# AIDynamicAction/rcognita

Measured on AMD Instinct MI355X. Metric: env-control-steps/sec (whole node), 3wrobot Nactor=10, higher is better.
Workload: dtype f64

## Files before the change

### include/rcg.h

```cpp
#ifndef RCG_H
#define RCG_H

#include <stdint.h>

#ifdef __cplusplus
extern "C" {
#endif

#define RCG_VERSION 122

#define RCG_MAX_DS 5
#define RCG_MAX_DU 2
#define RCG_MAX_CHI 7
#define RCG_MAX_PARS 5
#define RCG_MAX_DC 35
#define RCG_MAX_ROW 64
#define RCG_MAX_NACTOR 4096

typedef enum rcg_status {
  RCG_OK = 0,
  RCG_ERR_BAD_ARG = -1,
  RCG_ERR_HIP = -2,
  RCG_ERR_NO_DEVICE = -3,
  RCG_ERR_UNSUPPORTED = -4,
  RCG_ERR_NONFINITE = -5
} rcg_status;

typedef enum rcg_system { RCG_SYS_3WROBOT = 0, RCG_SYS_3WROBOT_NI = 1, RCG_SYS_2TANK = 2 } rcg_system;
#define RCG_SYS_USER_BASE 16
typedef enum rcg_mode { RCG_MODE_MPC = 0, RCG_MODE_RQL = 1, RCG_MODE_SQL = 2 } rcg_mode;
typedef enum rcg_stage { RCG_STAGE_QUADRATIC = 0, RCG_STAGE_BIQUADRATIC = 1 } rcg_stage;
typedef enum rcg_critic_struct {
  RCG_CRITIC_QUAD_LIN = 0,
  RCG_CRITIC_QUADRATIC = 1,
  RCG_CRITIC_QUAD_NOMIX = 2,
  RCG_CRITIC_QUAD_MIX = 3
} rcg_critic_struct;
typedef enum rcg_dtype { RCG_F32 = 0, RCG_F64 = 1 } rcg_dtype;
typedef enum rcg_where { RCG_HOST = 0, RCG_DEVICE = 1 } rcg_where;

#define RCG_FLAG_HAS_TARGET 0x1
#define RCG_FLAG_PER_ENV_PARS 0x2
#define RCG_FLAG_REF_LAG 0x4
#define RCG_FLAG_ACCUM_EVERY_SUBSTEP 0x8
#define RCG_FLAG_NO_CLIP 0x10
#define RCG_FLAG_DISTURB 0x20

typedef enum rcg_field {
  RCG_FIELD_STATE = 0,
  RCG_FIELD_ACTION = 1,
  RCG_FIELD_ACCUM = 2,
  RCG_FIELD_STEP_IDX = 3,
  RCG_FIELD_EPISODE_IDX = 4,
  RCG_FIELD_STATUS = 5,
  RCG_FIELD_PARS = 6,
  RCG_FIELD_STATE_INIT = 7,
  RCG_FIELD_STATE_PREV = 8,
  RCG_FIELD_BEST_J = 9,
  RCG_FIELD_BEST_IDX = 10,
  RCG_FIELD_W_CRITIC = 11,
  RCG_FIELD_W_PREV = 12,
  RCG_FIELD_OBS_BUF = 13,
  RCG_FIELD_ACT_BUF = 14,
  RCG_FIELD_RETURNS = 15,
  RCG_FIELD_ACTION_SQN = 16,
  RCG_FIELD_DISTURB = 17,
  RCG_FIELD_SUBSTEP_IDX = 18,
  RCG_FIELD_COUNT_ = 19
} rcg_field;

typedef struct rcg_cfg {
  int32_t struct_size;
  int32_t sys_id;
  int32_t batch;
  int32_t dtype;
  int32_t device;
  int32_t n_actor;
  int32_t mode;
  int32_t stage_obj_struct;
  int32_t critic_struct;
  int32_t n_critic;
  int32_t buffer_size;
  int32_t substeps_per_tick;
  int32_t flags;
  int32_t critic_every_ticks;
  double dt_sim;
  double sampling_time;
  double pred_step_size;
  double gamma;
  double pars[8];
  double ctrl_bnds[4];
  double R1[49];
  double R2[49];
  double target[8];
  double action_init[4];
  double w_init[40];
  double w_min[40];
  double w_max[40];
  double pars_disturb[6];
  double disturb_init[2];
  uint64_t seed;
  int64_t env_id_base;
} rcg_cfg;

typedef struct rcg_summary {
  double count;
  double sum;
  double sumsq;
  double min;
  double max;
  double n_failed;
} rcg_summary;

typedef struct rcg_handle rcg_handle;

int rcg_version(void);
const char* rcg_last_error(const rcg_handle* h);
int rcg_device_count(void);

int rcg_register_system(const char* name, const char* policy_src, int32_t ds, int32_t du, int32_t np, int32_t* sys_id);
int rcg_rtc_version(int32_t* major, int32_t* minor);
int rcg_system_info(int32_t sys_id, int32_t* ds, int32_t* du, int32_t* np, int32_t* has_jac);
int rcg_system_output_info(int32_t sys_id, int32_t* dy, int32_t* has_out, int32_t* has_out_jac);
int rcg_system_has_critic(int32_t sys_id, int32_t* has_critic);
int rcg_system_programs(int32_t sys_id, char* buf, int64_t cap, int64_t* need);

int rcg_create(const rcg_cfg* cfg, rcg_handle** out);
int rcg_destroy(rcg_handle* h);
int rcg_set_stream(rcg_handle* h, void* hip_stream);
int rcg_use_own_stream(rcg_handle* h);
int rcg_wait_stream(rcg_handle* h, void* producer_stream);
int rcg_release_stream(rcg_handle* h, void* consumer_stream);
int rcg_synchronize(rcg_handle* h);

int rcg_dev_alloc(rcg_handle* h, uint64_t bytes, void** dev_out);
int rcg_dev_free(rcg_handle* h, void* dev);
int rcg_memcpy_h2d(rcg_handle* h, void* dev_dst, const void* host_src, uint64_t bytes);
int rcg_memcpy_d2h(rcg_handle* h, void* host_dst, const void* dev_src, uint64_t bytes);

int rcg_set_field(rcg_handle* h, int field, const void* src, int where);
int rcg_get_field(rcg_handle* h, int field, void* dst, int where);
int64_t rcg_field_bytes(const rcg_handle* h, int field);
int rcg_field_ptr(rcg_handle* h, int field, void** dev_out);

int rcg_rhs(rcg_handle* h, const void* state, const void* action, void* dstate, void* clipped_action,
            int32_t n, int32_t clip);
int rcg_rhs_full(rcg_handle* h, const void* state, const void* disturb, const void* action, const void* xi,
                 void* dstate, void* ddisturb, void* clipped_action, int32_t n, int32_t clip);
int rcg_disturb_noise(rcg_handle* h, void* bits_out, void* xi_out);
int rcg_stage_obj(rcg_handle* h, const void* obs, const void* act, void* out, int32_t n);
int rcg_out(rcg_handle* h, const void* state, void* obs, int32_t n);
int rcg_critic(rcg_handle* h, const void* obs, const void* act, const void* w, void* out, int32_t n);
int rcg_actor_cost(rcg_handle* h, const void* cand, int32_t K, const void* obs, const void* state_sys,
                   const void* w, void* J);
int rcg_critic_cost(rcg_handle* h, const void* w, void* Jc);

int rcg_sim_step(rcg_handle* h, int32_t n_substeps);
int rcg_sim_step_h(rcg_handle* h, int32_t n_substeps, double step);
#define RCG_LOOP_DECIDE 1
#define RCG_LOOP_PUSH 2
#define RCG_LOOP_FIT 4
int rcg_loop_step(rcg_handle* h, const double* action_in, double step_h, int32_t n_substeps, int32_t flags, int32_t iters,
                  double* out);
int rcg_loop_step_begin(rcg_handle* h, const double* action_in, double step_h, int32_t n_substeps, int32_t flags, int32_t iters);
int rcg_loop_step_end(rcg_handle* h, double* out);
int rcg_actor_argmin(rcg_handle* h, const void* cand, int32_t K, const void* obs, const void* state_sys,
                     void* action, void* best_J, int32_t* best_idx);
int rcg_control_tick(rcg_handle* h, const void* cand, int32_t K);
int rcg_control_ticks(rcg_handle* h, int32_t T, int32_t K);
int rcg_control_tick_n(rcg_handle* h, const void* cand, int32_t K, int32_t T);
int rcg_set_tick_parts(rcg_handle* h, int32_t parts);
int rcg_join(rcg_handle* h);
int rcg_actor_optimize(rcg_handle* h, int32_t iters, const void* obs, const void* state_sys, const void* u_init,
                       void* u_opt, void* action, void* best_J, int32_t* n_iter);
int rcg_set_optimizer(rcg_handle* h, int32_t memory);
int rcg_set_optimizer_tol(rcg_handle* h, double ftol);
int rcg_control_tick_opt(rcg_handle* h, int32_t iters, int32_t warm_start);
int rcg_actor_search(rcg_handle* h, int32_t K, int32_t rounds, const void* obs, const void* state_sys, const void* centre,
                     void* u_best, void* action, void* best_J, int32_t* best_idx);
int rcg_control_tick_search(rcg_handle* h, int32_t K, int32_t rounds, int32_t warm_start);
int rcg_candidates_sample(rcg_handle* h, void* cand, int32_t K, int32_t round, const void* centre);
int rcg_nominal_action(rcg_handle* h, const void* obs, void* action, void* lyap, int32_t n, double ctrl_gain,
                       const double* ctrl_pars, int32_t clip);
int rcg_nominal_theta(rcg_handle* h, const void* obs, void* theta, int32_t n);
int rcg_control_tick_nominal(rcg_handle* h, double ctrl_gain, const double* ctrl_pars);
int rcg_critic_update(rcg_handle* h, int32_t do_fit);
int rcg_critic_fit(rcg_handle* h);
int rcg_episode_reset(rcg_handle* h);
int rcg_episode_stats(rcg_handle* h, int32_t from_accum, void* returns_out, rcg_summary* out);

int64_t rcg_tick_count(const rcg_handle* h);
int rcg_set_tick_count(rcg_handle* h, int64_t ticks);

typedef enum rcg_kernel { RCG_KERNEL_ACTOR = 0, RCG_KERNEL_SIM = 1, RCG_KERNEL_CRITIC = 2, RCG_KERNEL_COUNT_ = 3 } rcg_kernel;
#define RCG_PROFILE_PAUSE 0x80
int rcg_profile(rcg_handle* h, int32_t kernel_mask);
int rcg_profile_read(rcg_handle* h, int32_t kernel, double* total_ms, int64_t* launches);
int rcg_profile_samples(rcg_handle* h, int32_t kernel, double* ms_out, int64_t cap, int64_t* n_out);

typedef enum rcg_kernel_id {
  RCG_KID_NONE = 0,
  RCG_KID_ACTOR = 1,
  RCG_KID_ACTOR_DMA = 2,
  RCG_KID_TICKS = 3,
  RCG_KID_ACTOR_OPT = 4,
  RCG_KID_NOMINAL = 5,
  RCG_KID_SIM = 6,
  RCG_KID_SIM_V = 7,
  RCG_KID_SIM_DIST = 8,
  RCG_KID_CRITIC_FIT = 9,
  RCG_KID_ACTOR_DMA_PACKED = 10,
  RCG_KID_ACTOR_SEARCH = 11,
  RCG_KID_COUNT_ = 12
} rcg_kernel_id;
int rcg_last_launch(const rcg_handle* h, int32_t kind, int32_t* kernel_id, int32_t* variant, int32_t* envs_per_wave);
const char* rcg_kernel_name(int32_t kernel_id);

#ifdef __cplusplus
}
#endif
#endif
```

### rcognita_amd/_native.py

```python
from __future__ import annotations

import ctypes as C
import os
import sys

_HERE = os.path.dirname(os.path.abspath(__file__))
LIB_PATH = os.path.join(_HERE, "lib", "librcg.so")

RCG_VERSION = 122
OK, ERR_BAD_ARG, ERR_HIP, ERR_NO_DEVICE, ERR_UNSUPPORTED, ERR_NONFINITE = 0, -1, -2, -3, -4, -5
SYS_3WROBOT, SYS_3WROBOT_NI, SYS_2TANK = 0, 1, 2
MODE_MPC, MODE_RQL, MODE_SQL = 0, 1, 2
STAGE_QUADRATIC, STAGE_BIQUADRATIC = 0, 1
CRITIC_QUAD_LIN, CRITIC_QUADRATIC, CRITIC_QUAD_NOMIX, CRITIC_QUAD_MIX = 0, 1, 2, 3
F32, F64 = 0, 1
HOST, DEVICE = 0, 1
FLAG_HAS_TARGET, FLAG_PER_ENV_PARS, FLAG_REF_LAG, FLAG_ACCUM_EVERY_SUBSTEP, FLAG_NO_CLIP = 1, 2, 4, 8, 16
FLAG_DISTURB = 32
DIM_DISTURB = {0: 2, 1: 2, 2: 1}

(FIELD_STATE, FIELD_ACTION, FIELD_ACCUM, FIELD_STEP_IDX, FIELD_EPISODE_IDX, FIELD_STATUS, FIELD_PARS,
 FIELD_STATE_INIT, FIELD_STATE_PREV, FIELD_BEST_J, FIELD_BEST_IDX, FIELD_W_CRITIC, FIELD_W_PREV, FIELD_OBS_BUF,
 FIELD_ACT_BUF, FIELD_RETURNS, FIELD_ACTION_SQN, FIELD_DISTURB, FIELD_SUBSTEP_IDX) = range(19)
FIELD_COUNT = 19

MODE_IDS = {"MPC": MODE_MPC, "RQL": MODE_RQL, "SQL": MODE_SQL}
STAGE_IDS = {"quadratic": STAGE_QUADRATIC, "biquadratic": STAGE_BIQUADRATIC}
CRITIC_IDS = {"quad-lin": CRITIC_QUAD_LIN, "quadratic": CRITIC_QUADRATIC, "quad-nomix": CRITIC_QUAD_NOMIX,
              "quad-mix": CRITIC_QUAD_MIX}
SYS_IDS = {"3wrobot": SYS_3WROBOT, "3wrobotNI": SYS_3WROBOT_NI, "2tank": SYS_2TANK}
SYS_DIMS = {SYS_3WROBOT: (5, 2, 2), SYS_3WROBOT_NI: (3, 2, 0), SYS_2TANK: (2, 1, 5)}
SYS_DY = {}
SYS_USER_BASE = 16
MAX_DS, MAX_DU, MAX_PARS = 5, 2, 5

SYMBOLS = [
    "rcg_version", "rcg_last_error", "rcg_device_count", "rcg_create", "rcg_destroy", "rcg_set_stream", "rcg_use_own_stream",
    "rcg_synchronize", "rcg_dev_alloc", "rcg_dev_free", "rcg_memcpy_h2d", "rcg_memcpy_d2h", "rcg_set_field",
    "rcg_get_field", "rcg_field_bytes", "rcg_field_ptr", "rcg_rhs", "rcg_stage_obj", "rcg_critic",
    "rcg_actor_cost", "rcg_critic_cost", "rcg_sim_step", "rcg_sim_step_h", "rcg_actor_argmin", "rcg_control_tick",
    "rcg_critic_update", "rcg_control_ticks", "rcg_control_tick_n", "rcg_actor_optimize", "rcg_control_tick_opt", "rcg_nominal_action",
    "rcg_control_tick_nominal", "rcg_rhs_full", "rcg_disturb_noise", "rcg_episode_reset", "rcg_episode_stats", "rcg_tick_count", "rcg_set_tick_count", "rcg_profile", "rcg_profile_read",
    "rcg_profile_samples", "rcg_last_launch", "rcg_kernel_name", "rcg_wait_stream", "rcg_nominal_theta", "rcg_set_optimizer", "rcg_set_optimizer_tol", "rcg_set_tick_parts", "rcg_join", "rcg_loop_step", "rcg_loop_step_begin", "rcg_loop_step_end",
    "rcg_actor_search", "rcg_control_tick_search", "rcg_candidates_sample", "rcg_release_stream",
    "rcg_register_system", "rcg_rtc_version", "rcg_system_info", "rcg_system_output_info", "rcg_out",
    "rcg_system_has_critic", "rcg_system_programs", "rcg_critic_fit",
]
KERNEL_ACTOR, KERNEL_SIM, KERNEL_CRITIC = 0, 1, 2
(KID_NONE, KID_ACTOR, KID_ACTOR_DMA, KID_TICKS, KID_ACTOR_OPT, KID_NOMINAL, KID_SIM, KID_SIM_V, KID_SIM_DIST,
 KID_CRITIC_FIT, KID_ACTOR_DMA_PACKED, KID_ACTOR_SEARCH) = range(12)
DMA_MPC_G1, DMA_MPC, DMA_RQL_0, DMA_SQL_0 = 0, 1, 2, 6
LOOP_DECIDE, LOOP_PUSH, LOOP_FIT = 1, 2, 4
DMA_RQL_GEN_0 = 12
DMA_MPC_GEND, DMA_MPC_GENF = 10, 11


class RcgCfg(C.Structure):

    _fields_ = [
        ("struct_size", C.c_int32), ("sys_id", C.c_int32), ("batch", C.c_int32), ("dtype", C.c_int32),
        ("device", C.c_int32), ("n_actor", C.c_int32), ("mode", C.c_int32), ("stage_obj_struct", C.c_int32),
        ("critic_struct", C.c_int32), ("n_critic", C.c_int32), ("buffer_size", C.c_int32),
        ("substeps_per_tick", C.c_int32), ("flags", C.c_int32), ("critic_every_ticks", C.c_int32),
        ("dt_sim", C.c_double), ("sampling_time", C.c_double), ("pred_step_size", C.c_double), ("gamma", C.c_double),
        ("pars", C.c_double * 8), ("ctrl_bnds", C.c_double * 4), ("R1", C.c_double * 49), ("R2", C.c_double * 49),
        ("target", C.c_double * 8), ("action_init", C.c_double * 4), ("w_init", C.c_double * 40),
        ("w_min", C.c_double * 40), ("w_max", C.c_double * 40),
        ("pars_disturb", C.c_double * 6), ("disturb_init", C.c_double * 2), ("seed", C.c_uint64),
        ("env_id_base", C.c_int64),
    ]


class RcgSummary(C.Structure):
    _fields_ = [("count", C.c_double), ("sum", C.c_double), ("sumsq", C.c_double), ("min", C.c_double),
                ("max", C.c_double), ("n_failed", C.c_double)]


class NativeError(RuntimeError):
    def __init__(self, code, msg):
        super().__init__(f"librcg error {code}: {msg}")
        self.code = code


_lib = None


def use_library(path):
    global LIB_PATH
    if _lib is not None:
        raise RuntimeError("use_library: librcg is already loaded")
    LIB_PATH = os.path.abspath(path)


def lib():
    global _lib
    if _lib is not None:
        return _lib
    if not os.path.exists(LIB_PATH):
        raise ImportError(
            f"{LIB_PATH} not found: build the HIP library first (`make lib` at the repo root, or "
            "`python -c 'import __graft_entry__ as g; g.build()'`).  rcognita_amd has no CPU fallback."
        )
    torch = sys.modules.get("torch")
    if torch is not None and torch.cuda.is_available() and not torch.cuda.is_initialized():
        torch.cuda.init()
    L = C.CDLL(LIB_PATH)
    vp, i32, i64, u64 = C.c_void_p, C.c_int32, C.c_int64, C.c_uint64
    sig = {
        "rcg_version": (C.c_int, []),
        "rcg_last_error": (C.c_char_p, [vp]),
        "rcg_device_count": (C.c_int, []),
        "rcg_create": (C.c_int, [C.POINTER(RcgCfg), C.POINTER(vp)]),
        "rcg_destroy": (C.c_int, [vp]),
        "rcg_set_stream": (C.c_int, [vp, vp]),
        "rcg_use_own_stream": (C.c_int, [vp]),
        "rcg_synchronize": (C.c_int, [vp]),
        "rcg_dev_alloc": (C.c_int, [vp, u64, C.POINTER(vp)]),
        "rcg_dev_free": (C.c_int, [vp, vp]),
        "rcg_memcpy_h2d": (C.c_int, [vp, vp, vp, u64]),
        "rcg_memcpy_d2h": (C.c_int, [vp, vp, vp, u64]),
        "rcg_set_field": (C.c_int, [vp, C.c_int, vp, C.c_int]),
        "rcg_get_field": (C.c_int, [vp, C.c_int, vp, C.c_int]),
        "rcg_field_bytes": (i64, [vp, C.c_int]),
        "rcg_field_ptr": (C.c_int, [vp, C.c_int, C.POINTER(vp)]),
        "rcg_rhs": (C.c_int, [vp, vp, vp, vp, vp, i32, i32]),
        "rcg_stage_obj": (C.c_int, [vp, vp, vp, vp, i32]),
        "rcg_critic": (C.c_int, [vp, vp, vp, vp, vp, i32]),
        "rcg_actor_cost": (C.c_int, [vp, vp, i32, vp, vp, vp, vp]),
        "rcg_critic_cost": (C.c_int, [vp, vp, vp]),
        "rcg_sim_step": (C.c_int, [vp, i32]),
        "rcg_sim_step_h": (C.c_int, [vp, i32, C.c_double]),
        "rcg_actor_argmin": (C.c_int, [vp, vp, i32, vp, vp, vp, vp, vp]),
        "rcg_control_tick": (C.c_int, [vp, vp, i32]),
        "rcg_critic_update": (C.c_int, [vp, i32]),
        "rcg_control_ticks": (C.c_int, [vp, i32, i32]),
        "rcg_control_tick_n": (C.c_int, [vp, vp, i32, i32]),
        "rcg_actor_optimize": (C.c_int, [vp, i32, vp, vp, vp, vp, vp, vp, vp]),
        "rcg_control_tick_opt": (C.c_int, [vp, i32, i32]),
        "rcg_set_optimizer": (C.c_int, [vp, i32]),
        "rcg_set_tick_parts": (C.c_int, [vp, i32]),
        "rcg_set_optimizer_tol": (C.c_int, [vp, C.c_double]),
        "rcg_loop_step_begin": (C.c_int, [vp, vp, C.c_double, i32, i32, i32]),
        "rcg_loop_step_end": (C.c_int, [vp, vp]),
        "rcg_loop_step": (C.c_int, [vp, vp, C.c_double, i32, i32, i32, vp]),
        "rcg_join": (C.c_int, [vp]),
        "rcg_actor_search": (C.c_int, [vp, i32, i32, vp, vp, vp, vp, vp, vp, vp]),
        "rcg_control_tick_search": (C.c_int, [vp, i32, i32, i32]),
        "rcg_candidates_sample": (C.c_int, [vp, vp, i32, i32, vp]),
        "rcg_nominal_action": (C.c_int, [vp, vp, vp, vp, i32, C.c_double, C.POINTER(C.c_double), i32]),
        "rcg_control_tick_nominal": (C.c_int, [vp, C.c_double, C.POINTER(C.c_double)]),
        "rcg_nominal_theta": (C.c_int, [vp, vp, vp, i32]),
        "rcg_rhs_full": (C.c_int, [vp, vp, vp, vp, vp, vp, vp, vp, i32, i32]),
        "rcg_disturb_noise": (C.c_int, [vp, vp, vp]),
        "rcg_episode_reset": (C.c_int, [vp]),
        "rcg_episode_stats": (C.c_int, [vp, i32, vp, C.POINTER(RcgSummary)]),
        "rcg_tick_count": (i64, [vp]),
        "rcg_set_tick_count": (C.c_int, [vp, i64]),
        "rcg_profile": (C.c_int, [vp, i32]),
        "rcg_profile_read": (C.c_int, [vp, i32, C.POINTER(C.c_double), C.POINTER(i64)]),
        "rcg_profile_samples": (C.c_int, [vp, i32, C.POINTER(C.c_double), i64, C.POINTER(i64)]),
        "rcg_last_launch": (C.c_int, [vp, i32, C.POINTER(i32), C.POINTER(i32), C.POINTER(i32)]),
        "rcg_kernel_name": (C.c_char_p, [i32]),
        "rcg_wait_stream": (C.c_int, [vp, vp]),
        "rcg_release_stream": (C.c_int, [vp, vp]),
        "rcg_register_system": (C.c_int, [C.c_char_p, C.c_char_p, i32, i32, i32, C.POINTER(i32)]),
        "rcg_rtc_version": (C.c_int, [C.POINTER(i32), C.POINTER(i32)]),
        "rcg_system_info": (C.c_int, [i32, C.POINTER(i32), C.POINTER(i32), C.POINTER(i32), C.POINTER(i32)]),
        "rcg_system_output_info": (C.c_int, [i32, C.POINTER(i32), C.POINTER(i32), C.POINTER(i32)]),
        "rcg_out": (C.c_int, [vp, vp, vp, i32]),
        "rcg_system_has_critic": (C.c_int, [i32, C.POINTER(i32)]),
        "rcg_critic_fit": (C.c_int, [vp]),
        "rcg_system_programs": (C.c_int, [i32, C.c_char_p, i64, C.POINTER(i64)]),
    }
    for name, (res, args) in sig.items():
        fn = getattr(L, name)
        fn.restype = res
        fn.argtypes = args
    if L.rcg_version() != RCG_VERSION:
        raise ImportError(f"librcg.so version {L.rcg_version()} != binding version {RCG_VERSION}; rebuild")
    _lib = L
    return L


def last_error(handle=None) -> str:
    return lib().rcg_last_error(handle).decode("utf-8", "replace")


def check(rc, handle=None, allow=()):
    if rc != OK and rc not in allow:
        raise NativeError(rc, last_error(handle))
    return rc


def register_system(name: str, src: str, ds: int, du: int, np: int) -> dict:
    import time

    L = lib()
    sid = C.c_int32(-1)
    t0 = time.perf_counter()
    check(L.rcg_register_system(name.encode(), src.encode(), int(ds), int(du), int(np), C.byref(sid)))
    seconds = time.perf_counter() - t0
    SYS_DIMS[sid.value] = (int(ds), int(du), int(np))
    a, b = C.c_int32(0), C.c_int32(0)
    check(L.rcg_rtc_version(C.byref(a), C.byref(b)))
    jac = C.c_int32(0)
    check(L.rcg_system_info(sid.value, None, None, None, C.byref(jac)))
    dy, has_out, has_out_jac = C.c_int32(0), C.c_int32(0), C.c_int32(0)
    check(L.rcg_system_output_info(sid.value, C.byref(dy), C.byref(has_out), C.byref(has_out_jac)))
    SYS_DY[sid.value] = dy.value
    crit = C.c_int32(0)
    check(L.rcg_system_has_critic(sid.value, C.byref(crit)))
    return {"sys_id": sid.value, "name": name, "seconds": seconds, "hiprtc": (a.value, b.value), "has_jac": bool(jac.value),
            "dy": dy.value, "has_out": bool(has_out.value), "has_out_jac": bool(has_out_jac.value),
            "has_critic": bool(crit.value)}


def system_programs(sys_id: int) -> list:
    L = lib()
    need = C.c_int64(0)
    check(L.rcg_system_programs(int(sys_id), None, 0, C.byref(need)))
    buf = C.create_string_buffer(max(int(need.value), 1))
    check(L.rcg_system_programs(int(sys_id), buf, len(buf), None))
    return [tuple(line.split("\t", 1)) for line in buf.value.decode().splitlines() if line]


def sys_dy(sys_id: int) -> int:
    return SYS_DY.get(int(sys_id), SYS_DIMS[int(sys_id)][0])
```

### rcognita_amd/csrc/rcg_actor_dma.hpp

```cpp
#pragma once
#include <hip/hip_ext.h>
#include "rcg_kernels.hpp"

#ifndef RCG_DMA_AUX
#define RCG_DMA_AUX 2
#endif
#ifndef RCG_DMA_PRIO
#define RCG_DMA_PRIO 0
#endif

namespace rcg {

enum : int {
  DMA_MPC_G1 = 0,
  DMA_MPC = 1,
  DMA_RQL_0 = 2 ,
  DMA_SQL_0 = 6 ,
  DMA_MPC_GEND = 10,
  DMA_MPC_GENF = 11,
  DMA_RQL_GEN_0 = 12 ,
  DMA_VARIANTS = 16
};
__host__ __device__ constexpr bool dma_is_sql(int v) { return v >= DMA_SQL_0 && v < DMA_MPC_GEND; }
__host__ __device__ constexpr bool dma_is_rql(int v) { return (v >= DMA_RQL_0 && v < DMA_SQL_0) || v >= DMA_RQL_GEN_0; }
__host__ __device__ constexpr int dma_cs(int v) {
  return v >= DMA_RQL_GEN_0 ? v - DMA_RQL_GEN_0 : (dma_is_sql(v) ? v - DMA_SQL_0 : (dma_is_rql(v) ? v - DMA_RQL_0 : 0));
}

__host__ __device__ constexpr int dma_dc(int cs, int ds, int du) {
  return cs == RCG_CRITIC_QUAD_LIN ? (ds + du) * (ds + du + 1) / 2 + (ds + du)
                                   : (cs == RCG_CRITIC_QUADRATIC ? (ds + du) * (ds + du + 1) / 2
                                                                 : (cs == RCG_CRITIC_QUAD_NOMIX ? ds + du : ds + ds * du + du));
}

__host__ __device__ constexpr int dma_wslot(int esz, int variant, int ds, int du) {
  const int dcmax = (dma_is_sql(variant) || dma_is_rql(variant)) ? dma_dc(dma_cs(variant), ds, du) : 0;
  return dcmax > 9 ? ((dcmax * esz + 15) / 16) * 16 : 0;
}

__device__ __forceinline__ void wave_argmin(float& bestJ, int& bestI) {
  const unsigned long long wkey = wave_min_u64(((unsigned long long)float_order_key(bestJ) << 32) | (unsigned)bestI);
  bestJ = float_from_order_key((unsigned)(wkey >> 32));
  bestI = (int)(unsigned)wkey;
}
__device__ __forceinline__ void wave_argmin(double& bestJ, int& bestI) {
  for (int m = 1; m < 64; m <<= 1) {
    const double oJ = __shfl_xor(bestJ, m, 64);
    const int oI = __shfl_xor(bestI, m, 64);
    if ((oJ < bestJ) || (oJ == bestJ && oI < bestI)) {
      bestJ = oJ;
      bestI = oI;
    }
  }
}

template <typename S, typename = void>
struct HasPrefix {
  static constexpr bool value = false;
};
template <typename S>
struct HasPrefix<S, void_t_<decltype(S::PFX_FREE)>> {
  static constexpr bool value = true;
};
template <typename S>
constexpr unsigned pfx_free() {
  if constexpr (HasPrefix<S>::value)
    return S::PFX_FREE;
  else
    return 0u;
}
template <typename S>
constexpr int pfx_heading() {
  if constexpr (HasPrefix<S>::value)
    return S::PFX_HEADING;
  else
    return -1;
}

__device__ __forceinline__ float uniform_r(float v) {
  return __uint_as_float((unsigned)__builtin_amdgcn_readfirstlane((int)__float_as_uint(v)));
}
__device__ __forceinline__ double uniform_r(double v) {
  const unsigned long long b = (unsigned long long)__double_as_longlong(v);
  const unsigned lo = (unsigned)__builtin_amdgcn_readfirstlane((int)(unsigned)b);
  const unsigned hi = (unsigned)__builtin_amdgcn_readfirstlane((int)(unsigned)(b >> 32));
  return __longlong_as_double((long long)(((unsigned long long)hi << 32) | lo));
}

template <int J, int NP, int SZ, int PIECE>
__device__ __forceinline__ void dma_pieces(const unsigned char* g, unsigned off, unsigned char* l) {
  typedef __attribute__((address_space(3))) void lds_void;
  typedef const __attribute__((address_space(1))) void glb_void;
  if constexpr (J < NP) {
    constexpr int BASE = (J * PIECE / 4096) * 4096;
    const unsigned char* const gb = g + (off + (unsigned)BASE);
    if constexpr (SZ == 16)
      __builtin_amdgcn_global_load_lds((glb_void*)gb, (lds_void*)(l + BASE), 16, J * PIECE - BASE, RCG_DMA_AUX);
    else
      __builtin_amdgcn_global_load_lds((glb_void*)gb, (lds_void*)(l + BASE), 4, J * PIECE - BASE, RCG_DMA_AUX);
    dma_pieces<J + 1, NP, SZ, PIECE>(g, off, l);
  }
}

__host__ __device__ constexpr int dma_rpl(int r, int esz) { return r * esz <= 24 ? 4 : (r * esz <= 32 ? 2 : 1); }

template <typename Sys, typename real, int R, bool TGT, int V>
__global__ __launch_bounds__(256) void k_actor_dma(const ActorArgs<real> A, const KParams<real> P) {
  constexpr int DS = Sys::DS, DY = sys_dy<Sys>(), DU = Sys::DU, NCHI = DY + DU, NP = Sys::NP;
  constexpr bool OUT = HasOut<Sys>::value;
  constexpr bool G1 = V == DMA_MPC_G1, SQL = dma_is_sql(V), RQL = dma_is_rql(V), CRIT = RQL || SQL;
  constexpr bool GEND = V == DMA_MPC_GEND, GENF = V == DMA_MPC_GENF, GEN = GEND || GENF;
  constexpr bool GENR = V >= DMA_RQL_GEN_0;
  static_assert(!(GEN || GENR) || TGT, "the generic-cost instances subtract a target (zeros for a handle without one)");
  constexpr int CS = dma_cs(V);
  constexpr int DCMAX = CRIT ? dma_dc(CS, DY, DU) : 1;
  constexpr int ESZ = (int)sizeof(real);
  constexpr int WSLOT = dma_wslot(ESZ, V, DY, DU);
  constexpr bool WLDS = WSLOT > 0;
  constexpr int WREG = WLDS ? 1 : DCMAX;
  static_assert(R % DU == 0 && R >= DU && R <= 40, "row = N*du reals, at most 40 (f32: 160 bytes, f64: 320)");
  constexpr int N = R / DU;
  constexpr bool PFX = HasPrefix<Sys>::value && !OUT;
  constexpr unsigned FREE = PFX ? pfx_free<Sys>() : 0u;
  constexpr int HD = PFX ? pfx_heading<Sys>() : -1;
  constexpr bool TRIG0 = PFX && HD >= 0 && N >= 2;
  constexpr bool TRIG1 = TRIG0 && ((FREE >> (HD >= 0 ? HD : 0)) & 1u) && N >= 3;
  constexpr int RPL = dma_rpl(R, ESZ), TROWS = 64 * RPL;
  constexpr int TILE = TROWS * R * ESZ;
  constexpr int NFULL = TILE / 1024, NREM = (TILE % 1024) / 256;
  static_assert(NFULL * 1024 + NREM * 256 == TILE, "a tile is a whole number of 256-B segments");
  extern __shared__ __attribute__((aligned(16))) unsigned char smem_raw[];
  typedef __attribute__((address_space(3))) void lds_void;
  typedef const __attribute__((address_space(1))) void glb_void;

  const int lane = threadIdx.x & 63;
  const int wave_in_wg = __builtin_amdgcn_readfirstlane((int)(threadIdx.x >> 6));
  const long wave = (long)blockIdx.x * (blockDim.x >> 6) + wave_in_wg;
  const long B = P.B;
  const int K = A.K;
  const int T = (K + TROWS - 1) / TROWS;
  const int rem_rows = K % TROWS;
  const long env_hi = A.env_hi > 0 ? A.env_hi : B;
  const long env0 = A.env_lo + wave * A.gpw;
  if (env0 >= env_hi) return;
  const long env1 = env0 + A.gpw < env_hi ? env0 + A.gpw : env_hi;
  const int n_tiles = (int)(env1 - env0) * T;

  unsigned char* const tile = smem_raw + (size_t)wave_in_wg * TILE;
  const size_t env_stride = (size_t)K * (R * ESZ);
  const unsigned char* envb;
  {
    const unsigned long long p = (unsigned long long)(reinterpret_cast<const unsigned char*>(A.cand) + (size_t)env0 * env_stride);
    const unsigned lo = (unsigned)__builtin_amdgcn_readfirstlane((int)(unsigned)p);
    const unsigned hi = (unsigned)__builtin_amdgcn_readfirstlane((int)(unsigned)(p >> 32));
    envb = reinterpret_cast<const unsigned char*>(((unsigned long long)hi << 32) | lo);
  }
  const unsigned lane16 = (unsigned)lane * 16u, lane4 = (unsigned)lane * 4u;
  const int jspan = A.jwave ? A.gpw * K : K;
  real* const jstage = reinterpret_cast<real*>(smem_raw + (size_t)4 * TILE + (size_t)4 * WSLOT) + (size_t)wave_in_wg * jspan;
  real* const wl = reinterpret_cast<real*>(smem_raw + (size_t)4 * TILE + (size_t)wave_in_wg * WSLOT);

  auto issue_tile = [&](const unsigned char* g, int rows) {
    unsigned o16 = lane16, o4 = lane4;
    if (NFULL) asm volatile("" : "+v"(o16));
    if (NREM) asm volatile("" : "+v"(o4));
    asm volatile("" : "+s"(rows));
    if (rows == TROWS) {
      dma_pieces<0, NFULL, 16, 1024>(g, o16, tile);
      dma_pieces<0, NREM, 4, 256>(g + NFULL * 1024, o4, tile + NFULL * 1024);
    } else {
      const int vb = rows * (R * ESZ);
#pragma unroll
      for (int j = 0; j < NFULL; ++j)
        if ((int)o16 < vb - j * 1024)
          __builtin_amdgcn_global_load_lds((glb_void*)(g + (o16 + (unsigned)(j * 1024))), (lds_void*)(tile + j * 1024), 16, 0,
                                           RCG_DMA_AUX);
#pragma unroll
      for (int j = 0; j < NREM; ++j)
        if ((int)o4 < vb - (NFULL * 1024 + j * 256))
          __builtin_amdgcn_global_load_lds((glb_void*)(g + (o4 + (unsigned)(NFULL * 1024 + j * 256))),
                                           (lds_void*)(tile + NFULL * 1024 + j * 256), 4, 0, RCG_DMA_AUX);
    }
  };
  const int last_rows = rem_rows ? rem_rows : TROWS;
  auto rows_of = [&](int tt) -> int { return tt == T - 1 ? last_rows : TROWS; };

  real y0[DY], yn[sys_dxy<Sys>()], x0[DS], xn[DS], pv[NP > 0 ? NP : 1], pn[NP > 0 ? NP : 1], wc[WREG], wn[WREG];
  real wnl = 0;
  const bool lag = A.state_sys != A.obs;
#pragma unroll
  for (int i = 0; i < NP; ++i) pn[i] = P.pars[i];
#pragma unroll
  for (int i = 0; i < WREG; ++i) wn[i] = wc[i] = 0;
  constexpr int dc_rt = CRIT ? DCMAX : 0;
  auto fetch_env = [&](long b) {
    if (RCG_DBG(A, 4)) {
#pragma unroll
      for (int c = 0; c < sys_dxy<Sys>(); ++c) yn[c] = (real)0.5;
#pragma unroll
      for (int c = 0; c < DS; ++c) xn[c] = (real)0.5;
      return;
    }
    if constexpr (OUT) {
      load_obs_raw<Sys, real>(A.obs, A.obs_x, B, b, yn);
    } else {
#pragma unroll
      for (int c = 0; c < DS; ++c) yn[c] = A.obs[(long)c * B + b];
    }
    if (lag) {
#pragma unroll
      for (int c = 0; c < DS; ++c) xn[c] = A.state_sys[(long)c * B + b];
    }
    if (A.pars_env) {
#pragma unroll
      for (int i = 0; i < NP; ++i) pn[i] = A.pars_env[(long)i * B + b];
    }
    if (CRIT && WLDS) {
      if (lane < dc_rt) wnl = A.w[(long)lane * B + b];
    } else if (CRIT) {
#pragma unroll
      for (int i = 0; i < WREG; ++i) wn[i] = A.w[(long)i * B + b];
    }
  };

  constexpr bool TRI = GENF || GENR;
  constexpr int NSYM = TRI ? sym_len<NCHI>() : 1;
  real S1[NSYM], S2[NSYM];
  const bool biq = (GEN || GENR) && (P.stage_kind & STAGE_BIQUAD);
  const bool full_rt = GENF || (GENR && (P.stage_kind & STAGE_FULL));
  if constexpr (TRI) {
    if (full_rt) {
      load_sym<NCHI, real>(P.Rfull, S1);
    } else {
#pragma unroll
      for (int i = 0; i < NSYM; ++i) S1[i] = 0;
    }
    if (full_rt && biq) {
      load_sym<NCHI, real>(P.Rfull + 49, S2);
    } else {
#pragma unroll
      for (int i = 0; i < NSYM; ++i) S2[i] = 0;
    }
  }
  auto gen_stage = [&](const real* chi) -> real {
    real q;
    if (TRI && full_rt)
      q = quad_sym<NCHI, real>(S1, chi);
    else
      q = stage_diag<NCHI, real>(P, chi);
    if (biq) {
      real c2[NCHI];
#pragma unroll
      for (int i = 0; i < NCHI; ++i) c2[i] = chi[i] * chi[i];
      real q4;
      if (TRI && full_rt) {
        q4 = quad_sym<NCHI, real>(S2, c2);
      } else {
        q4 = 0;
#pragma unroll
        for (int i = 0; i < NCHI; ++i) q4 = fma_r(P.R2d[i] * c2[i], c2[i], q4);
      }
      q = q4 + q;
    }
    return q;
  };

  fetch_env(env0);
  issue_tile(envb, rows_of(0));

  const real h = P.h_pred;
  long b = env0;
  int t = 0;
  const bool env_pars = A.pars_env != nullptr;
  auto pre_env = Sys::template prepare<real>(pn);
  real x1s[DS], trig0[2] = {0, 0}, trig1[2] = {0, 0}, Sini[DY];
#pragma unroll
  for (int c = 0; c < DS; ++c) x1s[c] = 0;
#pragma unroll
  for (int c = 0; c < DY; ++c) Sini[c] = 0;
  real bestJ = inf_r<real>();
  int bestI = 0x7fffffff;
  real bu[DU];
#pragma unroll
  for (int c = 0; c < DU; ++c) bu[c] = 0;
  real resJ = 0, resAcc = 0, resU[DU];
  int resI = 0;
#pragma unroll
  for (int c = 0; c < DU; ++c) resU[c] = 0;

  auto adopt_regs = [&]() {
    if constexpr (OUT) {
#pragma unroll
      for (int c = 0; c < DS; ++c) x0[c] = lag ? xn[c] : yn[c];
#pragma unroll
      for (int i = 0; i < NP; ++i) pv[i] = pn[i];
      pre_env = Sys::template prepare<real>(pv);
      obs_of_raw<Sys, real>(pre_env, A.obs_x, yn, y0);
    } else {
#pragma unroll
      for (int c = 0; c < DS; ++c) {
        y0[c] = yn[c];
        x0[c] = lag ? xn[c] : yn[c];
      }
    }
    if (CRIT && WLDS) {
      if (lane < dc_rt) wl[lane] = wnl;
      asm volatile("s_waitcnt lgkmcnt(0)" ::: "memory");
      __builtin_amdgcn_wave_barrier();
    } else if (CRIT) {
#pragma unroll
      for (int i = 0; i < WREG; ++i) wc[i] = wn[i];
    }
  };
  auto adopt_rest = [&]() {
    if constexpr (PFX) {
#pragma unroll
      for (int c = 0; c < DS; ++c) x0[c] = uniform_r(x0[c]);
      if constexpr (TRIG0) {
        sincos_sel<real, true>(x0[HD], &trig0[0], &trig0[1]);
        if constexpr (FREE != 0) {
          real uz[DU], d[DS];
#pragma unroll
          for (int c = 0; c < DU; ++c) uz[c] = 0;
          Sys::template rhs_trig<real>(pre_env, x0, uz, trig0[0], trig0[1], d);
#pragma unroll
          for (int c = 0; c < DS; ++c)
            if ((FREE >> c) & 1u) x1s[c] = uniform_r(fma_r(h, d[c], x0[c]));
        }
        if constexpr (TRIG1) {
          sincos_sel<real, true>(x1s[HD], &trig1[0], &trig1[1]);
          trig1[0] = uniform_r(trig1[0]);
          trig1[1] = uniform_r(trig1[1]);
        }
        if constexpr (FREE == 0) {
          trig0[0] = uniform_r(trig0[0]);
          trig0[1] = uniform_r(trig0[1]);
        }
      }
      if constexpr (G1) {
#pragma unroll
        for (int c = 0; c < DY; ++c) {
          const real chi0 = TGT ? y0[c] - P.target[c] : y0[c];
          real a = fma_r(chi0, chi0, (real)0);
          if (N >= 2 && ((FREE >> c) & 1u)) {
            const real chi1 = TGT ? x1s[c] - P.target[c] : x1s[c];
            a = fma_r(chi1, chi1, a);
          }
          Sini[c] = uniform_r(a);
        }
      }
    }
    bestJ = inf_r<real>();
    bestI = 0x7fffffff;
  };
  const bool adopt_early = OUT || T == 1;

  for (int g = 0; g < n_tiles; ++g) {
    if (t == 0) {
      if constexpr (!OUT) {
        if (env_pars) pre_env = Sys::template prepare<real>(pn);
      }
      if (adopt_early) adopt_regs();
    }
    if constexpr (RCG_DMA_PRIO > 0 && ESZ == 8) __builtin_amdgcn_s_setprio(RCG_DMA_PRIO);
    asm volatile("s_waitcnt vmcnt(0)" ::: "memory");
    real rows[RPL][R];
#pragma unroll
    for (int j = 0; j < RPL; ++j) {
      const real* const myrow = reinterpret_cast<const real*>(tile) + (j * 64 + lane) * R;
#pragma unroll
      for (int i = 0; i < R; ++i) rows[j][i] = myrow[i];
    }
    asm volatile("s_waitcnt lgkmcnt(0)" ::: "memory");
    __builtin_amdgcn_wave_barrier();
    if (g + 1 < n_tiles) {
      if (t == T - 1) {
        fetch_env(b + 1);
        envb += env_stride;
        issue_tile(envb, rows_of(0));
      } else {
        issue_tile(envb + (size_t)(t + 1) * TILE, rows_of(t + 1));
      }
    }
    if constexpr (RCG_DMA_PRIO > 0 && ESZ == 8) __builtin_amdgcn_s_setprio(0);
    if (t == 0) {
      if (!adopt_early) adopt_regs();
      adopt_rest();
    }

#pragma unroll
    for (int j = 0; j < RPL; ++j) {
      const real* const cur = rows[j];
      real x[DS], y[DY];
      if constexpr (OUT) {
#pragma unroll
        for (int c = 0; c < DS; ++c) x[c] = x0[c];
#pragma unroll
        for (int c = 0; c < DY; ++c) y[c] = y0[c];
      } else {
#pragma unroll
        for (int c = 0; c < DS; ++c) {
          x[c] = x0[c];
          y[c] = y0[c];
        }
      }
      real J = 0, gk = 1;
      real S[NCHI];
#pragma unroll
      for (int i = 0; i < NCHI; ++i) S[i] = (PFX && G1 && i < DY) ? Sini[i < DY ? i : 0] : (real)0;
      real Phi[SQL ? DCMAX : 1];
#pragma unroll
      for (int i = 0; i < (SQL ? DCMAX : 1); ++i) Phi[i] = 0;
      auto wget = [&](int i) -> real { return WLDS ? wl[i] : wc[WLDS ? 0 : i]; };
      if (RCG_DBG(A, 1)) {
#pragma unroll
        for (int i = 0; i < R; ++i) J += cur[i];
      } else {
#pragma unroll
        for (int kk = 0; kk < N; ++kk) {
          if (kk > 0) {
            real d[DS];
            if constexpr (TRIG0 || TRIG1) {
              if (kk == 1 && TRIG0)
                Sys::template rhs_trig<real>(pre_env, x, &cur[(kk - 1) * DU], trig0[0], trig0[1], d);
              else if (kk == 2 && TRIG1)
                Sys::template rhs_trig<real>(pre_env, x, &cur[(kk - 1) * DU], trig1[0], trig1[1], d);
              else
                Sys::template rhs<real, true>(pre_env, x, &cur[(kk - 1) * DU], d);
            } else {
              Sys::template rhs<real, true>(pre_env, x, &cur[(kk - 1) * DU], d);
            }
#pragma unroll
            for (int c = 0; c < DS; ++c) {
              if (PFX && kk == 1 && ((FREE >> c) & 1u))
                x[c] = x1s[c];
              else
                x[c] = fma_r(h, d[c], x[c]);
              if constexpr (!OUT) y[c] = x[c];
            }
            if constexpr (OUT) sys_out<Sys, real, true>(pre_env, x, y);
          }
          real chi[NCHI];
#pragma unroll
          for (int c = 0; c < DY; ++c) chi[c] = TGT ? y[c] - P.target[c] : y[c];
#pragma unroll
          for (int c = 0; c < DU; ++c) chi[DY + c] = cur[kk * DU + c];
          if (G1) {
#pragma unroll
            for (int i = 0; i < NCHI; ++i) {
              if (PFX && i < DY && (kk == 0 || (kk == 1 && ((FREE >> i) & 1u)))) continue;
              S[i] = fma_r(chi[i], chi[i], S[i]);
            }
          } else if (SQL) {
            critic_phi_accum<DY, DU, real>(chi, y, &cur[kk * DU], Phi, CS);
          } else if (RQL && kk == N - 1) {
            J += critic_with<DY, DU, real>(chi, y, &cur[kk * DU], wget, CS);
          } else if (GEN || GENR) {
            J = fma_r(gk, gen_stage(chi), J);
            gk *= P.gamma;
          } else {
            J = fma_r(gk, stage_diag<NCHI, real>(P, chi), J);
            gk *= P.gamma;
          }
        }
        if (G1) {
#pragma unroll
          for (int i = 0; i < NCHI; ++i) J = fma_r(P.R1d[i], S[i], J);
        }
        if (SQL) {
#pragma unroll
          for (int i = 0; i < DCMAX; ++i) J = fma_r(wget(i), Phi[i], J);
        }
      }

      const int k = t * TROWS + j * 64 + lane;
      const bool has_row = k < K;
      if (A.J && has_row) jstage[(A.jwave ? (int)(b - env0) * K : 0) + k] = J;
      const real Jc = (J != J) ? inf_r<real>() : J;
      if (has_row && (Jc < bestJ || bestI == 0x7fffffff)) {
        bestJ = Jc;
        bestI = k;
#pragma unroll
        for (int c = 0; c < DU; ++c) bu[c] = cur[c];
      }
    }

    if (A.J && (A.jwave ? g == n_tiles - 1 : t == T - 1)) {
      asm volatile("s_waitcnt lgkmcnt(0)" ::: "memory");
      __builtin_amdgcn_wave_barrier();
      real* const Jout = A.J + (A.jwave ? env0 : b) * K;
      const int n = A.jwave ? (int)(env1 - env0) * K : K;
      const int nbytes = n * ESZ;
      if ((nbytes & 1023) == 0) {
        const unsigned char* const src = reinterpret_cast<const unsigned char*>(jstage);
        unsigned char* const dst = reinterpret_cast<unsigned char*>(Jout);
        for (int i = lane * 16; i < nbytes; i += 1024)
          __builtin_nontemporal_store(*reinterpret_cast<const v4f*>(src + i), reinterpret_cast<v4f*>(dst + i));
      } else {
        for (int i = lane; i < n; i += 64) Jout[i] = jstage[i];
      }
    }
    if (++t == T) {
      if (RCG_DBG(A, 2)) {
        if (bestJ == (real)-12345.678f) A.best_J[b] = bestJ;
        if (lane == 0 && A.step_idx) atomicAdd(&A.step_idx[b], 1);
        t = 0;
        ++b;
        continue;
      }
      wave_argmin(bestJ, bestI);
      const int wl = __builtin_amdgcn_readfirstlane(bestI & 63);
#pragma unroll
      for (int c = 0; c < DU; ++c) bu[c] = readlane_r(bu[c], wl);
      real acc_inc = 0;
      if (A.accum) {
        real chi[NCHI];
#pragma unroll
        for (int c = 0; c < DY; ++c) chi[c] = TGT ? y0[c] - P.target[c] : y0[c];
#pragma unroll
        for (int c = 0; c < DU; ++c) chi[DY + c] = bu[c];
        acc_inc = ((GEN || GENR || SQL) ? stage_any<NCHI, real>(P, chi) : stage_diag<NCHI, real>(P, chi)) * P.sampling_time;
      }
      if (lane == (int)(b - env0)) {
        resJ = bestJ;
        resI = bestI;
        resAcc = acc_inc;
#pragma unroll
        for (int c = 0; c < DU; ++c) resU[c] = bu[c];
      }
      t = 0;
      ++b;
    }
  }

  if (lane < (int)(env1 - env0) && !RCG_DBG(A, 2)) {
    const long bb = env0 + lane;
#pragma unroll
    for (int c = 0; c < DU; ++c)
      if (A.action_out) A.action_out[(long)c * B + bb] = resU[c];
    if (A.best_J) A.best_J[bb] = resJ;
    if (A.best_idx) A.best_idx[bb] = resI;
    if (A.accum) atomicAdd(&A.accum[bb], resAcc);
    if (A.step_idx) atomicAdd(&A.step_idx[bb], 1);
  }
}

#if !defined(__HIPCC_RTC__)
template <typename Sys, typename real, int GROUP>
bool launch_dma(int r, int variant, dim3 grid, dim3 block, size_t lds, hipStream_t s, const ActorArgs<real>& A,
                const KParams<real>& P, hipEvent_t ev_a, hipEvent_t ev_b);
#endif

template <typename real>
constexpr int dma_max_row() {
  return 40;
}

}
```

### rcognita_amd/csrc/rcg_api.hip

```cpp
#include <cstdarg>
#include <cstdio>
#include <cstdlib>
#include <cstring>

#include "rcg_disturb.hpp"
#include "rcg_handle.hpp"
#include "rcg_search.hpp"

using namespace rcg;

static thread_local std::string g_err = "";

int rcg_fail(rcg_handle* h, int code, const char* fmt, ...) {
  char buf[512];
  va_list ap;
  va_start(ap, fmt);
  vsnprintf(buf, sizeof buf, fmt, ap);
  va_end(ap);
  if (h)
    h->err = buf;
  else
    g_err = buf;
  return code;
}
// ... 937 lines not shown
  if (action_in) memcpy(p_act, action_in, in_bytes);
  const double* const act_dev = action_in ? p_act : nullptr;
  const float d32 = h->p32.dt_sim;
  const double d64 = h->p64.dt_sim;
  h->p64.dt_sim = step_h / (double)n_substeps;
  h->p32.dt_sim = (float)h->p64.dt_sim;
  int rc;
  const bool one_launch = decide && !push && h->cfg.mode == RCG_MODE_MPC && h->p64.stage_kind == 0 && opt_memory_of(h) == 0;
  if (one_launch) {
    h->loop_io.on = true;
    h->loop_io.act_in = act_dev;
    h->loop_io.n_substeps = n_substeps, h->loop_io.dc = dc;
    h->loop_io.out = p_out, h->loop_io.flag = p_flag, h->loop_io.seq = seq;
    rc = h->sys->optimize(h, iters, nullptr, h->f[RCG_FIELD_STATE_PREV], nullptr, 0, h->sqn_alt,
                          h->f[RCG_FIELD_ACTION], h->f[RCG_FIELD_BEST_J], (int32_t*)h->f[RCG_FIELD_BEST_IDX], false, false);
    h->loop_io.on = false;
  } else if (!decide && !push) {
    rc = h->sys->loop(h, act_dev, n_substeps, 1, 1, 0, dc, p_out, p_flag, seq);
  } else {
    rc = h->sys->loop(h, act_dev, n_substeps, push ? 0 : 1, 0, 0, dc, p_out, p_flag, seq);
    if (rc == RCG_OK && push) rc = h->sys->critic_update(h, n_substeps, 1, fit ? 1 : 0);
    if (rc == RCG_OK && decide)
      rc = h->sys->optimize(h, iters, nullptr, h->f[RCG_FIELD_STATE_PREV], nullptr, 0, h->sqn_alt,
                            h->f[RCG_FIELD_ACTION], h->f[RCG_FIELD_BEST_J], (int32_t*)h->f[RCG_FIELD_BEST_IDX], false, false);
    if (rc == RCG_OK) rc = h->sys->loop(h, nullptr, n_substeps, 0, 1, decide ? 1 : 0, dc, p_out, p_flag, seq);
  }
  h->p32.dt_sim = d32;
  h->p64.dt_sim = d64;
  if (rc) return rc;
  HIPCHK(h, hipGetLastError());
  h->loop_pending = true;
  h->loop_pending_decided = decide;
  h->loop_pending_row = row;
  return RCG_OK;
}

int rcg_loop_step_end(rcg_handle* h, double* out) {
  DeviceGuard dev_guard(h);
  if (!h) return RCG_ERR_BAD_ARG;
  if (!h->loop_pending) return rcg_fail(h, RCG_ERR_BAD_ARG, "rcg_loop_step_end: no step is pending (rcg_loop_step_begin)");
  h->loop_pending = false;
  const int B = h->cfg.batch, row = h->loop_pending_row;
  double* const p_out = (double*)h->loop_pin;
  volatile double* const f = p_out + (size_t)B * row + (size_t)B * h->du;
  const double seq = (double)h->loop_seq;
  bool done = false;
  for (long spin = 0; spin < 20000000L && !done; ++spin) {
    done = true;
    for (int b = 0; b < B; ++b)
      if (f[b] != seq) {
        done = false;
        break;
      }
    if (!done) __builtin_ia32_pause();
  }
  if (!done) {
    HIPCHK(h, hipStreamSynchronize(h->stream));
    for (int b = 0; b < B; ++b)
      if (f[b] != seq) return rcg_fail(h, RCG_ERR_HIP, "rcg_loop_step: the glue kernel did not report env %d", b);
  }
  __atomic_thread_fence(__ATOMIC_ACQUIRE);
  if (out) {
    memcpy(out, p_out, (size_t)B * row * sizeof(double));
    if (h->loop_pending_decided) std::swap(h->f[RCG_FIELD_ACTION_SQN], h->sqn_alt);
  }
  return RCG_OK;
}

int rcg_loop_step(rcg_handle* h, const double* action_in, double step_h, int32_t n_substeps, int32_t flags, int32_t iters,
                  double* out) {
  if (!h || !out) return rcg_fail(h, RCG_ERR_BAD_ARG, "rcg_loop_step: bad argument");
  const int rc = rcg_loop_step_begin(h, action_in, step_h, n_substeps, flags, iters);
  return rc ? rc : rcg_loop_step_end(h, out);
}

static int check_search(rcg_handle* h, const char* who, int32_t K, int32_t rounds) {
  if (K < 64) return rcg_fail(h, RCG_ERR_BAD_ARG, "%s: K must be >= 64 (a wave evaluates 64 candidates at a time)", who);
  if (rounds < 1 || rounds > 64) return rcg_fail(h, RCG_ERR_BAD_ARG, "%s: rounds must be in [1, 64]", who);
  if (h->cfg.mode != RCG_MODE_MPC && !h->f[RCG_FIELD_W_CRITIC])
    return rcg_fail(h, RCG_ERR_BAD_ARG, "%s: RQL/SQL need critic weights (buffer_size > 0)", who);
  return RCG_OK;
}

int rcg_actor_search(rcg_handle* h, int32_t K, int32_t rounds, const void* obs, const void* state_sys, const void* centre,
                     void* u_best, void* action, void* best_J, int32_t* best_idx) {
  DeviceGuard dev_guard(h);
  if (!h) return RCG_ERR_BAD_ARG;
  const int rc = check_search(h, "rcg_actor_search", K, rounds);
  if (rc) return rc;
  return h->sys->search(h, K, rounds, 0, obs, state_sys, centre, 0, u_best, action, best_J, best_idx, false, false);
}

int rcg_control_tick_search(rcg_handle* h, int32_t K, int32_t rounds, int32_t warm_start) {
  DeviceGuard dev_guard(h);
  if (!h) return RCG_ERR_BAD_ARG;
  int rc = check_search(h, "rcg_control_tick_search", K, rounds);
  if (rc) return rc;
  if (h->rtc)
    return rcg_fail(h, RCG_ERR_UNSUPPORTED, "rcg_control_tick_search: not available for a system registered at run time");
  bool sim_first = true;
  if (h->cfg.mode != RCG_MODE_MPC) {
    rc = tick_critic_phase(h, "rcg_control_tick_search");
    if (rc) return rc;
    sim_first = false;
  }
  const bool warm = warm_start && h->tick_count > 0;
  void* sqn = h->f[RCG_FIELD_ACTION_SQN];
  rc = h->sys->search(h, K, rounds, 0, nullptr, nullptr, warm ? sqn : nullptr, warm ? 1 : 0, sqn, h->f[RCG_FIELD_ACTION],
                      h->f[RCG_FIELD_BEST_J], (int32_t*)h->f[RCG_FIELD_BEST_IDX], true, sim_first);
  if (rc == RCG_OK) h->tick_count += 1;
  return rc;
}

int rcg_candidates_sample(rcg_handle* h, void* cand, int32_t K, int32_t round, const void* centre) {
  DeviceGuard dev_guard(h);
  if (!h || !cand) return rcg_fail(h, RCG_ERR_BAD_ARG, "rcg_candidates_sample: cand is required");
  if (K < 1 || round < 0 || round > 63) return rcg_fail(h, RCG_ERR_BAD_ARG, "rcg_candidates_sample: need K >= 1 and 0 <= round <= 63");
  const int R = h->cfg.n_actor * h->du;
  const int32_t* ep = (const int32_t*)h->f[RCG_FIELD_EPISODE_IDX];
  const int32_t* st = (const int32_t*)h->f[RCG_FIELD_STEP_IDX];
  const int n_draws = (R + 7) / 8;
  int KB = 256;
  while (KB > 64 && (size_t)rcg::cand_block_draws(KB, n_draws, h->du) * 32 > (size_t)48 * 1024) KB >>= 1;
  const size_t lds = (size_t)rcg::cand_block_draws(KB, n_draws, h->du) * 32;
  if (lds > (size_t)160 * 1024)
    return rcg_fail(h, RCG_ERR_UNSUPPORTED, "rcg_candidates_sample: rows of %d reals need %zu B of LDS per 64 candidates", R, lds);
  if ((K + KB - 1) / KB > 65535) return rcg_fail(h, RCG_ERR_BAD_ARG, "rcg_candidates_sample: K too large");
  const dim3 grid((unsigned)h->cfg.batch, (unsigned)((K + KB - 1) / KB)), block(256);
#define RCG_SAMPLE(DU, real, P)                                                                                          \
  do {                                                                                                                   \
    auto fn = k_cand_sample<DU, real>;                                                                                   \
    if (lds > (size_t)64 * 1024)                     \
      HIPCHK(h, hipFuncSetAttribute(reinterpret_cast<const void*>(fn), hipFuncAttributeMaxDynamicSharedMemorySize,      \
                                    (int)lds));                                                                          \
    hipLaunchKernelGGL(fn, grid, block, lds, h->stream, (real*)cand, (const real*)centre, ep, st, (int)K, (int)round, R, \
                       (uint64_t)h->cfg.seed, (int64_t)h->cfg.env_id_base, (real)h->cfg.action_init[0],                  \
                       (real)h->cfg.action_init[1], KB, P);                                                              \
  } while (0)
  if (h->cfg.dtype == RCG_F64) {
    if (h->du == 1)
      RCG_SAMPLE(1, double, h->p64);
    else
      RCG_SAMPLE(2, double, h->p64);
  } else {
    if (h->du == 1)
      RCG_SAMPLE(1, float, h->p32);
    else
      RCG_SAMPLE(2, float, h->p32);
  }
#undef RCG_SAMPLE
  HIPCHK(h, hipGetLastError());
  return RCG_OK;
}

int rcg_nominal_action(rcg_handle* h, const void* obs, void* action, void* lyap, int32_t n, double ctrl_gain,
                       const double* ctrl_pars, int32_t clip) {
  DeviceGuard dev_guard(h);
  if (!h || !obs || (!action && !lyap) || n < 1)
    return rcg_fail(h, RCG_ERR_BAD_ARG, "rcg_nominal_action: obs and one of action/lyap are required, n >= 1");
  return h->sys->nominal(h, obs, action, lyap, nullptr, n, ctrl_gain, ctrl_pars, clip, false);
}

int rcg_nominal_theta(rcg_handle* h, const void* obs, void* theta, int32_t n) {
  DeviceGuard dev_guard(h);
  if (!h || !obs || !theta || n < 1) return rcg_fail(h, RCG_ERR_BAD_ARG, "rcg_nominal_theta: obs, theta and n >= 1 are required");
  if (h->cfg.sys_id != RCG_SYS_3WROBOT)
    return rcg_fail(h, RCG_ERR_UNSUPPORTED, "rcg_nominal_theta: only CtrlNominal3WRobot has a theta search");
  return h->sys->nominal(h, obs, nullptr, nullptr, theta, n, 1.0, nullptr, 0, false);
}

int rcg_control_tick_nominal(rcg_handle* h, double ctrl_gain, const double* ctrl_pars) {
  DeviceGuard dev_guard(h);
  if (!h) return RCG_ERR_BAD_ARG;
  if (h->cfg.sys_id == RCG_SYS_2TANK)
    return rcg_fail(h, RCG_ERR_UNSUPPORTED, "rcg_control_tick_nominal: the reference defines no nominal controller for 2tank");
  if (h->rtc)
    return rcg_fail(h, RCG_ERR_UNSUPPORTED, "rcg_control_tick_nominal: not available for a system registered at run time");
  int rc = h->sys->sim_step(h, h->cfg.substeps_per_tick);
  if (rc) return rc;
  rc = h->sys->nominal(h, h->f[RCG_FIELD_STATE], h->f[RCG_FIELD_ACTION], nullptr, nullptr, h->cfg.batch, ctrl_gain,
                       ctrl_pars, 1, true);
  if (rc == RCG_OK) h->tick_count += 1;
  return rc;
}

int rcg_episode_reset(rcg_handle* h) {
  DeviceGuard dev_guard(h);
  if (!h) return RCG_ERR_BAD_ARG;
  const long B = h->cfg.batch;
  h->tick_count = 0;
  if (h->cfg.dtype == RCG_F64)
    hipLaunchKernelGGL((k_episode_reset<double>), dim3(blocks_for(B)), dim3(256), 0, h->stream,
                       (double*)h->f[RCG_FIELD_STATE], (double*)h->f[RCG_FIELD_STATE_PREV],
                       (const double*)h->f[RCG_FIELD_STATE_INIT], (double*)h->f[RCG_FIELD_ACTION],
                       (double*)h->f[RCG_FIELD_ACCUM], (double*)h->f[RCG_FIELD_RETURNS],
                       (int32_t*)h->f[RCG_FIELD_STEP_IDX], (int32_t*)h->f[RCG_FIELD_EPISODE_IDX],
                       (uint32_t*)h->f[RCG_FIELD_STATUS], h->ds, h->du, h->cfg.action_init[0], h->cfg.action_init[1], B);
  else
    hipLaunchKernelGGL((k_episode_reset<float>), dim3(blocks_for(B)), dim3(256), 0, h->stream,
                       (float*)h->f[RCG_FIELD_STATE], (float*)h->f[RCG_FIELD_STATE_PREV],
                       (const float*)h->f[RCG_FIELD_STATE_INIT], (float*)h->f[RCG_FIELD_ACTION],
                       (float*)h->f[RCG_FIELD_ACCUM], (float*)h->f[RCG_FIELD_RETURNS],
                       (int32_t*)h->f[RCG_FIELD_STEP_IDX], (int32_t*)h->f[RCG_FIELD_EPISODE_IDX],
                       (uint32_t*)h->f[RCG_FIELD_STATUS], h->ds, h->du, (float)h->cfg.action_init[0],
                       (float)h->cfg.action_init[1], B);
  HIPCHK(h, hipGetLastError());
  if (h->cfg.flags & RCG_FLAG_DISTURB) {
    const int dd = h->cfg.sys_id == RCG_SYS_2TANK ? 1 : 2;
    const int rc = h->cfg.dtype == RCG_F64 ? fill_rows<double>(h, h->f[RCG_FIELD_DISTURB], dd, h->cfg.disturb_init)
                                           : fill_rows<float>(h, h->f[RCG_FIELD_DISTURB], dd, h->cfg.disturb_init);
    if (rc) return rc;
    HIPCHK(h, hipMemsetAsync(h->f[RCG_FIELD_SUBSTEP_IDX], 0, h->fbytes[RCG_FIELD_SUBSTEP_IDX], h->stream));
  }
  return RCG_OK;
}

int rcg_episode_stats(rcg_handle* h, int32_t from_accum, void* returns_out, rcg_summary* out) {
  DeviceGuard dev_guard(h);
  if (!h || !out) return rcg_fail(h, RCG_ERR_BAD_ARG, "rcg_episode_stats: out is required");
  const int field = from_accum ? RCG_FIELD_ACCUM : RCG_FIELD_RETURNS;
  const long B = h->cfg.batch;
  if (h->cfg.dtype == RCG_F64)
    hipLaunchKernelGGL((k_stats<double>), dim3(1), dim3(1024), 0, h->stream, (const double*)h->f[field],
                       (const uint32_t*)h->f[RCG_FIELD_STATUS], B, h->d_summary);
  else
    hipLaunchKernelGGL((k_stats<float>), dim3(1), dim3(1024), 0, h->stream, (const float*)h->f[field],
                       (const uint32_t*)h->f[RCG_FIELD_STATUS], B, h->d_summary);
  HIPCHK(h, hipGetLastError());
  double s[6];
  HIPCHK(h, hipMemcpyAsync(s, h->d_summary, sizeof s, hipMemcpyDeviceToHost, h->stream));
  if (returns_out)
    HIPCHK(h, hipMemcpyAsync(returns_out, h->f[field], h->fbytes[field], hipMemcpyDeviceToHost, h->stream));
  HIPCHK(h, hipStreamSynchronize(h->stream));
  out->count = s[0];
  out->sum = s[1];
  out->sumsq = s[2];
  out->min = s[3];
  out->max = s[4];
  out->n_failed = s[5];
  return s[5] > 0 ? rcg_fail(h, RCG_ERR_NONFINITE, "rcg_episode_stats: %.0f env(s) hit a non-finite state", s[5])
                  : RCG_OK;
}

int64_t rcg_tick_count(const rcg_handle* h) { return h ? (int64_t)h->tick_count : -1; }

int rcg_set_tick_count(rcg_handle* h, int64_t ticks) {
  if (!h) return RCG_ERR_BAD_ARG;
  if (ticks < 0) return rcg_fail(h, RCG_ERR_BAD_ARG, "rcg_set_tick_count: ticks must be >= 0");
  h->tick_count = (long)ticks;
  return RCG_OK;
}

int rcg_profile(rcg_handle* h, int32_t enable) {
  DeviceGuard dev_guard(h);
  if (!h) return RCG_ERR_BAD_ARG;
  if (((unsigned)enable & 0xffu) == RCG_PROFILE_PAUSE) {
    h->prof_mask = 0;
    return RCG_OK;
  }
  const int drain_rc = prof_drain(h);
  h->prof_mask = (unsigned)enable & 0x7fu;
  h->prof_stride = (((unsigned)enable >> 8) & 0xfffu) ? (((unsigned)enable >> 8) & 0xfffu) : 1u;
  const unsigned skip = (unsigned)enable >> 20;
  for (int k = 0; k < RCG_KERNEL_COUNT_; ++k)
    h->prof_seen[k] = skip ? (uint64_t)h->prof_stride - (uint64_t)(skip % h->prof_stride) : 0;
  if (enable) {
    memset(h->prof_ms, 0, sizeof h->prof_ms);
    memset(h->prof_n, 0, sizeof h->prof_n);
    for (auto& v : h->prof_samples) v.clear();
  }
  return drain_rc;
}

int rcg_profile_read(rcg_handle* h, int32_t kernel, double* total_ms, int64_t* launches) {
  DeviceGuard dev_guard(h);
  if (!h || kernel < 0 || kernel >= RCG_KERNEL_COUNT_)
    return rcg_fail(h, RCG_ERR_BAD_ARG, "rcg_profile_read: bad kernel id");
  const int drain_rc = prof_drain(h);
  if (total_ms) *total_ms = h->prof_ms[kernel];
  if (launches) *launches = h->prof_n[kernel];
  return drain_rc;
}

int rcg_profile_samples(rcg_handle* h, int32_t kernel, double* ms_out, int64_t cap, int64_t* n_out) {
  DeviceGuard dev_guard(h);
  if (!h || kernel < 0 || kernel >= RCG_KERNEL_COUNT_ || cap < 0 || (cap > 0 && !ms_out))
    return rcg_fail(h, RCG_ERR_BAD_ARG, "rcg_profile_samples: bad argument");
  const int drain_rc = prof_drain(h);
  const std::vector<float>& v = h->prof_samples[kernel];
  const int64_t n = (int64_t)v.size();
  for (int64_t i = 0; i < n && i < cap; ++i) ms_out[i] = (double)v[(size_t)i];
  if (n_out) *n_out = n;
  return drain_rc;
}

int rcg_last_launch(const rcg_handle* h, int32_t kind, int32_t* kernel_id, int32_t* variant, int32_t* envs_per_wave) {
  if (!h || kind < 0 || kind >= RCG_KERNEL_COUNT_) return RCG_ERR_BAD_ARG;
  if (kernel_id) *kernel_id = h->last[kind].kernel_id;
  if (variant) *variant = h->last[kind].variant;
  if (envs_per_wave) *envs_per_wave = h->last[kind].envs_per_wave;
  return RCG_OK;
}

const char* rcg_kernel_name(int32_t kernel_id) {
  static const char* const names[RCG_KID_COUNT_] = {"none",        "k_actor",   "k_actor_dma", "k_ticks",    "k_actor_opt",
                                                    "k_nominal",   "k_sim",     "k_sim_v",     "k_sim_dist", "k_critic_fit",
                                                    "k_actor_dma_packed", "k_actor_search"};
  return (kernel_id >= 0 && kernel_id < RCG_KID_COUNT_) ? names[kernel_id] : "?";
}

}
```

### rcognita_amd/csrc/rcg_dma_launch.hpp

```cpp
#pragma once

#include "rcg_actor_dma.hpp"
#include "rcg_actor_dma_packed.hpp"

namespace rcg {

template <typename Sys, typename real, int GROUP, int R>
static bool launch_dma_r(int r, int variant, dim3 grid, dim3 block, size_t lds, hipStream_t s, const ActorArgs<real>& A,
                         const KParams<real>& P, hipEvent_t ev_a, hipEvent_t ev_b) {
  if constexpr (R > dma_max_row<real>()) {
    return false;
  } else {
    if (r != R) return launch_dma_r<Sys, real, GROUP, R + 1>(r, variant, grid, block, lds, s, A, P, ev_a, ev_b);
    if constexpr (R % Sys::DU != 0) {
      return false;
    } else {
#define RCG_DMA_CASE(V)                                                                                              \
  case V: {                                                                                                          \
    auto fn = k_actor_dma<Sys, real, R, ((V) >= DMA_MPC_GEND ? true : Sys::TGT), V>;                                 \
    if (lds > 64 * 1024)      \
      (void)hipFuncSetAttribute(reinterpret_cast<const void*>(fn), hipFuncAttributeMaxDynamicSharedMemorySize,       \
                                (int)lds);                                                                           \
    if (ev_a)                                                                                                        \
      hipExtLaunchKernelGGL(fn, grid, block, (std::uint32_t)lds, s, ev_a, ev_b, 0, A, P);                            \
    else                                                                                                             \
      hipLaunchKernelGGL(fn, grid, block, lds, s, A, P);                                                             \
    return true;                                                                                                     \
  }
      if constexpr (GROUP == 0) {
        switch (variant) {
          RCG_DMA_CASE(DMA_MPC_G1)
          RCG_DMA_CASE(DMA_MPC)
        }
      } else if constexpr (GROUP == 6) {
        switch (variant) {
          RCG_DMA_CASE(DMA_MPC_GEND)
          RCG_DMA_CASE(DMA_MPC_GENF)
        }
      } else if constexpr (GROUP == 7) {
        switch (variant) {
          RCG_DMA_CASE(DMA_RQL_GEN_0 + RCG_CRITIC_QUAD_LIN)
          RCG_DMA_CASE(DMA_RQL_GEN_0 + RCG_CRITIC_QUADRATIC)
          RCG_DMA_CASE(DMA_RQL_GEN_0 + RCG_CRITIC_QUAD_NOMIX)
          RCG_DMA_CASE(DMA_RQL_GEN_0 + RCG_CRITIC_QUAD_MIX)
        }
      } else if constexpr (GROUP == 1) {
        switch (variant) {
          RCG_DMA_CASE(DMA_SQL_0 + RCG_CRITIC_QUAD_LIN)
          RCG_DMA_CASE(DMA_SQL_0 + RCG_CRITIC_QUADRATIC)
          RCG_DMA_CASE(DMA_SQL_0 + RCG_CRITIC_QUAD_NOMIX)
          RCG_DMA_CASE(DMA_SQL_0 + RCG_CRITIC_QUAD_MIX)
        }
      } else {
        switch (variant) {
          RCG_DMA_CASE(DMA_RQL_0 + RCG_CRITIC_QUAD_LIN)
          RCG_DMA_CASE(DMA_RQL_0 + RCG_CRITIC_QUADRATIC)
          RCG_DMA_CASE(DMA_RQL_0 + RCG_CRITIC_QUAD_NOMIX)
          RCG_DMA_CASE(DMA_RQL_0 + RCG_CRITIC_QUAD_MIX)
        }
      }
#undef RCG_DMA_CASE
      return false;
    }
  }
}

template <typename Sys, typename real, int GROUP>
bool launch_dma(int r, int variant, dim3 grid, dim3 block, size_t lds, hipStream_t s, const ActorArgs<real>& A,
                const KParams<real>& P, hipEvent_t ev_a, hipEvent_t ev_b) {
  return launch_dma_r<Sys, real, GROUP, 1>(r, variant, grid, block, lds, s, A, P, ev_a, ev_b);
}

template <typename Sys, typename real, int GROUP, int R>
static bool launch_dma_packed_r(int r, int variant, dim3 grid, dim3 block, size_t lds, hipStream_t s,
                                const ActorArgs<real>& A, const KParams<real>& P, hipEvent_t ev_a, hipEvent_t ev_b) {
  if constexpr (R > dma_max_row<real>()) {
    return false;
  } else {
    if (r != R) return launch_dma_packed_r<Sys, real, GROUP, R + 1>(r, variant, grid, block, lds, s, A, P, ev_a, ev_b);
    if constexpr (R % Sys::DU != 0) {
      return false;
    } else {
#define RCG_DMAP_CASE(V)                                                                                             \
  case V: {                                                                                                          \
    if constexpr ((V) >= DMA_RQL_0 &&                                                                                \
                  !packed_critic_ok(dma_dc(((V) >= DMA_SQL_0 ? (V)-DMA_SQL_0 : (V)-DMA_RQL_0), sys_dy<Sys>(), Sys::DU), \
                                    (int)sizeof(real))) {                                                            \
      return false;       \
    } else {                                                                                                         \
      auto fn = k_actor_dma_packed<Sys, real, R, Sys::TGT, V>;                                                       \
      if (lds > 64 * 1024)                                                                                           \
        (void)hipFuncSetAttribute(reinterpret_cast<const void*>(fn), hipFuncAttributeMaxDynamicSharedMemorySize,     \
                                  (int)lds);                                                                         \
      if (ev_a)                                                                                                      \
        hipExtLaunchKernelGGL(fn, grid, block, (std::uint32_t)lds, s, ev_a, ev_b, 0, A, P);                          \
      else                                                                                                           \
        hipLaunchKernelGGL(fn, grid, block, lds, s, A, P);                                                           \
      return true;                                                                                                   \
    }                                                                                                                \
  }
      if constexpr (GROUP == 3) {
        switch (variant) {
          RCG_DMAP_CASE(DMA_MPC_G1)
          RCG_DMAP_CASE(DMA_MPC)
        }
      } else if constexpr (GROUP == 4) {
        switch (variant) {
          RCG_DMAP_CASE(DMA_SQL_0 + RCG_CRITIC_QUAD_LIN)
          RCG_DMAP_CASE(DMA_SQL_0 + RCG_CRITIC_QUADRATIC)
          RCG_DMAP_CASE(DMA_SQL_0 + RCG_CRITIC_QUAD_NOMIX)
          RCG_DMAP_CASE(DMA_SQL_0 + RCG_CRITIC_QUAD_MIX)
        }
      } else {
        switch (variant) {
          RCG_DMAP_CASE(DMA_RQL_0 + RCG_CRITIC_QUAD_LIN)
          RCG_DMAP_CASE(DMA_RQL_0 + RCG_CRITIC_QUADRATIC)
          RCG_DMAP_CASE(DMA_RQL_0 + RCG_CRITIC_QUAD_NOMIX)
          RCG_DMAP_CASE(DMA_RQL_0 + RCG_CRITIC_QUAD_MIX)
        }
      }
#undef RCG_DMAP_CASE
      return false;
    }
  }
}

template <typename Sys, typename real, int GROUP>
bool launch_dma_packed(int r, int variant, dim3 grid, dim3 block, size_t lds, hipStream_t s, const ActorArgs<real>& A,
                       const KParams<real>& P, hipEvent_t ev_a, hipEvent_t ev_b) {
  return launch_dma_packed_r<Sys, real, GROUP, 1>(r, variant, grid, block, lds, s, A, P, ev_a, ev_b);
}

}
```

### rcognita_amd/csrc/rcg_handle.hpp

```cpp
#pragma once
#include <hip/hip_ext.h>
#include <hip/hip_runtime.h>

#include <cstdint>
#include <cstdio>
#include <cstdlib>
#include <map>
#include <string>
#include <vector>

#include "rcg_actor_opt.hpp"
#include "rcg_kernels.hpp"

struct rcg_handle {
  rcg_cfg cfg;
  int ds, du, np, dc, nchi;
  int dy;
  bool rtc_has_out;
  size_t esz;
  hipStream_t stream;
  hipStream_t own_stream;
  void* f[RCG_FIELD_COUNT_];
  size_t fbytes[RCG_FIELD_COUNT_];
  double* d_summary;
  long tick_count;
  int opt_memory;
  double opt_ftol;
  void* d_const;
  struct {
    bool on;
    const double* act_in;
    int n_substeps, dc;
    double *out, *flag, seq;
  } loop_io;
  bool loop_pending;
  int loop_pending_row;
  bool loop_pending_decided;
  void* sqn_alt;
  void* loop_pin;
  uint64_t loop_seq;
  void* fit_scratch;
  size_t fit_scratch_bytes;
  rcg::KParams<float> p32;
  rcg::KParams<double> p64;
  const struct SysVTable* sys;
  const struct RtcSystem* rtc;
  std::map<std::string, hipFunction_t> rtc_fn;
  std::string err;
  unsigned prof_mask;
  unsigned prof_stride;
  uint64_t prof_seen[RCG_KERNEL_COUNT_];
  std::vector<hipEvent_t> ev_free;
  struct Pending {
    hipEvent_t a, b;
    int kernel;
  };
  std::vector<Pending> ev_pending;
  double prof_ms[RCG_KERNEL_COUNT_];
  int64_t prof_n[RCG_KERNEL_COUNT_];
  std::vector<float> prof_samples[RCG_KERNEL_COUNT_];
  hipEvent_t cur_a, cur_b;
  bool scope_due;
  hipEvent_t order_ev;
  hipEvent_t release_ev;
  void* bounce;
  int tick_parts;
  hipStream_t split_stream[2];
  hipEvent_t split_fork, split_join[2];
  bool split_pending;
  int sub_lo, sub_hi;
  int probe;
  struct LastLaunch {
    int32_t kernel_id, variant, envs_per_wave;
  } last[RCG_KERNEL_COUNT_];
};
static constexpr size_t kProfMaxSamples = 65536;

static constexpr size_t kBounceBytes = 16384;
static constexpr int kSplitMinBatch = 65536;
static constexpr int kVariantSplitBit = 4096;
static inline void note_launch(rcg_handle* h, int kind, int kernel_id, int variant, int envs_per_wave) {
  h->last[kind].kernel_id = kernel_id;
  h->last[kind].variant = variant | (h->sub_hi > 0 ? kVariantSplitBit : 0);
  h->last[kind].envs_per_wave = envs_per_wave;
}

static constexpr size_t kConstR64 = 512, kConstW = 1296, kConstBytes = 2256;
static constexpr int kFitMaxRows = 8;

int rcg_fail(rcg_handle* h, int code, const char* fmt, ...);

#define HIPCHK(h, call)                                                                                 \
  do {                                                                                                  \
    hipError_t e_ = (call);                                                                             \
    if (e_ != hipSuccess)                                                                               \
      return rcg_fail((h), RCG_ERR_HIP, "%s failed: %s (%s:%d)", #call, hipGetErrorString(e_), __FILE__, \
                      __LINE__);                                                                        \
  } while (0)

struct ProfScope {
  rcg_handle* h;
  hipEvent_t a, b;
  int kernel;
  bool on;
  ProfScope(rcg_handle* h_, int kernel_)
      : h(h_), a(nullptr), b(nullptr), kernel(kernel_), on((h_->prof_mask >> kernel_) & 1u) {
    if (!on) return;
    if ((h->prof_seen[kernel]++ % h->prof_stride) != 0) {
      on = false;
      return;
    }
    for (hipEvent_t* e : {&a, &b}) {
      if (!h->ev_free.empty()) {
        *e = h->ev_free.back();
        h->ev_free.pop_back();
      } else if (hipEventCreate(e) != hipSuccess) {
        if (a) h->ev_free.push_back(a);
        a = b = nullptr;
        on = false;
        return;
      }
    }
    h->cur_a = a;
    h->cur_b = b;
    h->scope_due = true;
  }
  ~ProfScope() {
    if (!on) return;
    h->scope_due = false;
    if (h->cur_a == nullptr) {
      h->ev_pending.push_back({a, b, kernel});
    } else {
      h->cur_a = h->cur_b = nullptr;
      h->ev_free.push_back(a);
      h->ev_free.push_back(b);
    }
  }
  ProfScope(const ProfScope&) = delete;
  ProfScope& operator=(const ProfScope&) = delete;
};

struct ProfPair {
  hipEvent_t a, b;
};
static inline ProfPair prof_take(rcg_handle* h) {
  const ProfPair p{h->cur_a, h->cur_b};
  h->cur_a = h->cur_b = nullptr;
#ifdef RCG_DEV
  if (h->scope_due) {
    if (!p.a) {
      fprintf(stderr, "librcg (dev): a second launch inside one due ProfScope would go untimed\n");
      abort();
    }
  }
#endif
  return p;
}
static inline void prof_give_back(rcg_handle* h, const ProfPair& p) {
  h->cur_a = p.a;
  h->cur_b = p.b;
}

#define RCG_LAUNCH(h, kern, grid, block, lds, ...)                                                                 \
  do {                                                                                                             \
    rcg_handle* h__ = (h);                                                                                         \
    const ProfPair pp__ = prof_take(h__);                                                                          \
    if (pp__.a) {                                                                                                  \
      hipExtLaunchKernelGGL(kern, grid, block, (std::uint32_t)(lds), h__->stream, pp__.a, pp__.b, 0, __VA_ARGS__); \
    } else {                                                                                                       \
      hipLaunchKernelGGL(kern, grid, block, lds, h__->stream, __VA_ARGS__);                                        \
    }                                                                                                              \
  } while (0)

template <typename real>
inline const rcg::KParams<real>& params(const rcg_handle* h);
template <>
inline const rcg::KParams<float>& params<float>(const rcg_handle* h) {
  return h->p32;
}
template <>
inline const rcg::KParams<double>& params<double>(const rcg_handle* h) {
  return h->p64;
}

static inline int opt_memory_of(const rcg_handle* h) {
  if (h->opt_memory >= 0) return h->opt_memory;
  const bool generic = !(h->cfg.mode == RCG_MODE_MPC && h->p32.stage_kind == 0);
  const int dcw = h->cfg.mode != RCG_MODE_MPC ? h->dc : 0;
  int mem = generic ? 4 : 0;
  while (mem > 0 && (size_t)rcg::opt_lds_reals(h->cfg.n_actor, h->ds, h->du, h->np, dcw, mem, h->dy) * h->esz > (size_t)160 * 1024) --mem;
  return mem;
}
static inline size_t opt_wave_lds_bytes(const rcg_handle* h) {
  const int dcw = h->cfg.mode != RCG_MODE_MPC ? h->dc : 0;
  return (size_t)rcg::opt_lds_reals(h->cfg.n_actor, h->ds, h->du, h->np, dcw, opt_memory_of(h), h->dy) * h->esz;
}

static inline unsigned blocks_for(long n, int bs = 256) { return (unsigned)((n + bs - 1) / bs); }

struct SysVTable {
  int (*rhs)(rcg_handle*, const void* state, const void* action, void* dstate, void* clipped, int32_t n, int32_t clip);
  int (*stage_obj)(rcg_handle*, const void* obs, const void* act, void* out, int32_t n);
  int (*critic)(rcg_handle*, const void* obs, const void* act, const void* w, void* out, int32_t n);
  int (*critic_cost)(rcg_handle*, const void* w, void* Jc);
  int (*actor)(rcg_handle*, const char* who, const void* cand, int K, const void* obs, const void* state_sys,
               const void* w, void* J, void* action, void* best_J, int32_t* best_idx, bool tick, bool sim_first);
  int (*sim_step)(rcg_handle*, int32_t n_substeps);
  int (*critic_update)(rcg_handle*, int32_t n_substeps , int32_t do_push, int32_t do_fit);
  int (*optimize)(rcg_handle*, int32_t iters, const void* obs, const void* state_sys, const void* u_init, int shift,
                  void* u_opt, void* action, void* best_J, int32_t* n_iter, bool tick, bool sim_first);
  int (*nominal)(rcg_handle*, const void* obs, void* action, void* lyap, void* theta, int32_t n, double gain,
                 const double* ctrl_pars, int32_t clip, bool tick);
  int (*ticks)(rcg_handle*, int32_t T, int32_t K, const void* cand);
  int (*rhs_full)(rcg_handle*, const void* state, const void* disturb, const void* action, const void* xi, void* dstate,
                  void* ddisturb, void* clipped, int32_t n, int32_t clip);
  int (*search)(rcg_handle*, int32_t K, int32_t rounds, int32_t round0, const void* obs, const void* state_sys,
                const void* centre, int shift, void* u_best, void* action, void* best_J, int32_t* best_idx, bool tick,
                bool sim_first);
  int (*ticks_mem)(rcg_handle*, int32_t T, int32_t K, const void* cand);
  int (*loop)(rcg_handle*, const double* act_in, int32_t n_substeps, int32_t do_sim, int32_t do_tail, int32_t decided, int32_t dc,
              double* out, double* flag, double seq);
};
extern const SysVTable kVt3WRobot, kVt3WRobotNI, kVt2Tank;

struct RtcDims {
  int ds, du, np;
  bool has_jac;
  int dy;
  bool has_out;
  bool has_out_jac;
  bool has_critic;
};
const RtcSystem* rtc_lookup(int sys_id, RtcDims* dims);
int rtc_out(rcg_handle* h, const void* state, void* obs, int32_t n);
int rtc_prepare_tick(rcg_handle* h, const void* cand, int32_t K);
int rtc_prepare_tick_opt(rcg_handle* h);
extern const SysVTable kVtRtc;
void rcg_set_thread_error(const std::string& text);
```

### rcognita_amd/csrc/rcg_math.hpp

```cpp
#pragma once
#include <hip/hip_runtime.h>

namespace rcg {

template <typename real>
__device__ __forceinline__ void sincos_r(real x, real* s, real* c);

template <>
__device__ __forceinline__ void sincos_r<float>(float x, float* s, float* c) {
  const float kf = __builtin_rintf(x * 0.63661977236758134308f);
  float r = __builtin_fmaf(kf, -1.57079637050628662109375f, x);
  r = __builtin_fmaf(kf, 4.37113882867379288655e-8f, r);
  r = __builtin_fmaf(kf, 1.71512451000588187280e-15f, r);
  const float r2 = r * r;
  float ps = __builtin_fmaf(r2, -1.9515295891e-4f, 8.3321608736e-3f);
  ps = __builtin_fmaf(ps, r2, -1.6666654611e-1f);
  const float sr = __builtin_fmaf(ps * r2, r, r);
  float pc = __builtin_fmaf(r2, 2.443315711809948e-5f, -1.388731625493765e-3f);
  pc = __builtin_fmaf(pc, r2, 4.166664568298827e-2f);
  const float cr = __builtin_fmaf(pc * r2, r2, __builtin_fmaf(r2, -0.5f, 1.0f));
  const int k = (int)kf;
  const float ss = (k & 1) ? cr : sr;
  const float cc = (k & 1) ? sr : cr;
  *s = (k & 2) ? -ss : ss;
  *c = ((k + 1) & 2) ? -cc : cc;
}

template <>
__device__ __forceinline__ void sincos_r<double>(double x, double* s, double* c) {
  ::sincos(x, s, c);
}

__device__ __forceinline__ void sincos_hw(float x, float* s, float* c) {
  const float kf = __builtin_rintf(x * 0.15915494309189533577f);
  float r = __builtin_fmaf(kf, -6.28318548202514648438f, x);
  r = __builtin_fmaf(kf, 1.74845553146951715e-7f, r);
  const float t = r * 0.15915494309189533577f;
  *s = __builtin_amdgcn_sinf(t);
  *c = __builtin_amdgcn_cosf(t);
}

__device__ __forceinline__ void sincos_fast(double x, double* s, double* c) {
  const double kf = __builtin_rint(x * 0.63661977236758134308);
  double r = __builtin_fma(kf, -1.57079632679489655800e+00, x);
  r = __builtin_fma(kf, -6.12323399573676603587e-17, r);
  const double z = r * r;
  double ps = __builtin_fma(z, 1.58969099521155010221e-10, -2.50507602534068634195e-08);
  ps = __builtin_fma(ps, z, 2.75573137070700676789e-06);
  ps = __builtin_fma(ps, z, -1.98412698298579493134e-04);
  ps = __builtin_fma(ps, z, 8.33333333332248946124e-03);
  ps = __builtin_fma(ps, z, -1.66666666666666324348e-01);
  const double sr = __builtin_fma(ps * z, r, r);
  double pc = __builtin_fma(z, -1.13596475577881948265e-11, 2.08757232129817482790e-09);
  pc = __builtin_fma(pc, z, -2.75573143513906633035e-07);
  pc = __builtin_fma(pc, z, 2.48015872894767294178e-05);
  pc = __builtin_fma(pc, z, -1.38888888888741095749e-03);
  pc = __builtin_fma(pc, z, 4.16666666666666019037e-02);
  const double cr = __builtin_fma(pc * z, z, __builtin_fma(z, -0.5, 1.0));
  const int k = (int)kf;
  const double ss = (k & 1) ? cr : sr;
  const double cc = (k & 1) ? sr : cr;
  *s = (k & 2) ? -ss : ss;
  *c = ((k + 1) & 2) ? -cc : cc;
}

template <typename real, bool HW>
__device__ __forceinline__ void sincos_sel(real x, real* s, real* c) {
  sincos_r<real>(x, s, c);
}
template <>
__device__ __forceinline__ void sincos_sel<double, true>(double x, double* s, double* c) {
  sincos_fast(x, s, c);
}
template <>
__device__ __forceinline__ void sincos_sel<float, true>(float x, float* s, float* c) {
  sincos_hw(x, s, c);
}

typedef float v2f __attribute__((ext_vector_type(2)));
__device__ __forceinline__ v2f pk_fma(v2f a, v2f b, v2f c) { return __builtin_elementwise_fma(a, b, c); }
__device__ __forceinline__ v2f pk_splat(float s) { return v2f{s, s}; }

__device__ __forceinline__ float fma_r(float a, float b, float c) { return __builtin_fmaf(a, b, c); }
__device__ __forceinline__ double fma_r(double a, double b, double c) { return __builtin_fma(a, b, c); }

template <typename real>
__device__ __forceinline__ real clamp_r(real v, real lo, real hi) {
  return v < lo ? lo : (v > hi ? hi : v);
}

__device__ __forceinline__ float clamp_fin(float v, float lo, float hi) { return __builtin_amdgcn_fmed3f(v, lo, hi); }
__device__ __forceinline__ double clamp_fin(double v, double lo, double hi) { return __builtin_fmin(__builtin_fmax(v, lo), hi); }

template <typename real>
__device__ __forceinline__ bool finite_r(real v) {
  return __builtin_isfinite(v);
}

template <typename real>
__device__ __forceinline__ real inf_r() {
  return (real)__builtin_huge_val();
}

__device__ __forceinline__ unsigned float_order_key(float v) {
  const unsigned b = __float_as_uint(v + 0.0f);
  return (b & 0x80000000u) ? ~b : (b | 0x80000000u);
}
__device__ __forceinline__ float float_from_order_key(unsigned k) {
  return __uint_as_float((k & 0x80000000u) ? (k ^ 0x80000000u) : ~k);
}
__device__ __forceinline__ unsigned long long wave_min_u64(unsigned long long k) {
#define RCG_DPP_MIN(CTRL)                                                                                      \
  {                                                                                                            \
    const unsigned lo = (unsigned)__builtin_amdgcn_update_dpp(0, (int)(unsigned)k, CTRL, 0xF, 0xF, false);         \
    const unsigned hi = (unsigned)__builtin_amdgcn_update_dpp(0, (int)(unsigned)(k >> 32), CTRL, 0xF, 0xF, false); \
    const unsigned long long o = ((unsigned long long)hi << 32) | lo;                                          \
    k = o < k ? o : k;                                                                                         \
  }
  RCG_DPP_MIN(0xB1)
  RCG_DPP_MIN(0x4E)
  RCG_DPP_MIN(0x141)
  RCG_DPP_MIN(0x140)
#undef RCG_DPP_MIN
  unsigned long long r[4];
#pragma unroll
  for (int i = 0; i < 4; ++i) {
    const unsigned lo = (unsigned)__builtin_amdgcn_readlane((int)(unsigned)k, 16 * i);
    const unsigned hi = (unsigned)__builtin_amdgcn_readlane((int)(unsigned)(k >> 32), 16 * i);
    r[i] = ((unsigned long long)hi << 32) | lo;
  }
  const unsigned long long a = r[1] < r[0] ? r[1] : r[0], b = r[3] < r[2] ? r[3] : r[2];
  return b < a ? b : a;
}

__device__ __forceinline__ float readlane_r(float v, int l) {
  return __uint_as_float((unsigned)__builtin_amdgcn_readlane((int)__float_as_uint(v), l));
}
__device__ __forceinline__ double readlane_r(double v, int l) {
  const unsigned long long b = (unsigned long long)__double_as_longlong(v);
  const unsigned lo = (unsigned)__builtin_amdgcn_readlane((int)(unsigned)b, l);
  const unsigned hi = (unsigned)__builtin_amdgcn_readlane((int)(unsigned)(b >> 32), l);
  return __longlong_as_double((long long)(((unsigned long long)hi << 32) | lo));
}


}
```

### rcognita_amd/csrc/rcg_rtc.hip

```cpp
#include <hip/hiprtc.h>

#include <cctype>
#include <map>
#include <memory>
#include <mutex>
#include <tuple>

#include "rcg_rtc_headers.inc"
#include "rcg_sysops.hpp"

using namespace rcg;

namespace {

struct RtcProgram {
  std::string code;
  std::map<std::string, std::string> lowered;
  std::map<int, hipModule_t> module;
  std::map<std::pair<int, std::string>, hipFunction_t> fn;
};

}

struct RtcSystem {
  int id;
  std::string name, src;
  RtcDims dims;
  bool tgt;
  RtcProgram core[2];
  std::map<std::tuple<int, int, int, int>, std::unique_ptr<RtcProgram>> dma;
  std::map<std::tuple<int, int, int>, std::unique_ptr<RtcProgram>> critic;
  std::vector<std::string> compiled;
};

namespace {

std::mutex g_mu;
std::vector<std::unique_ptr<RtcSystem>> g_sys;

const char* const kSysExpr = "rcg::RcgRtcSys";
const char* const kOpts[] = {"--offload-arch=gfx950", "-O3", "-std=c++17", "-ffp-contract=fast"};

template <typename real>
const char* real_name() {
  return sizeof(real) == 8 ? "double" : "float";
}

bool is_identifier(const char* s) {
  if (!s || !(isalpha((unsigned char)s[0]) || s[0] == '_')) return false;
  for (const char* p = s; *p; ++p)
    if (!(isalnum((unsigned char)*p) || *p == '_')) return false;
  return strlen(s) < 128;
}

std::string unit_source(const RtcSystem& S, bool critic = false) {
  char dims[1536];
  snprintf(dims, sizeof dims,
           "static_assert(RcgRtcSys::DS == %d, \"rcg_register_system: %s::DS differs from the declared ds\");\n"
           "static_assert(RcgRtcSys::DU == %d, \"rcg_register_system: %s::DU differs from the declared du\");\n"
           "static_assert(RcgRtcSys::NP == %d, \"rcg_register_system: %s::NP differs from the declared np\");\n"
           "static_assert(RcgRtcSys::HAS_OUT || RcgRtcSys::DY == RcgRtcSys::DS, \"rcg_register_system: %s::DY differs from DS "
           "but %s defines no out (without an output map the observation is the state)\");\n",
           S.dims.ds, S.name.c_str(), S.dims.du, S.name.c_str(), S.dims.np, S.name.c_str(), S.name.c_str(), S.name.c_str());
  const std::string& N = S.name;
  return std::string(critic ? "#include \"rcg_critic_fit_ml.hpp\"\n#include \"rcg_critic_fit_gen.hpp\"\n" : "") +
         "#include \"rcg_actor_dma_packed.hpp\"\n#include \"rcg_actor_opt.hpp\"\nnamespace rcg {\n#line 1 \"" + N + ".policy\"\n" +
         S.src +
         "\n#line 1 \"rcg_rtc_adapter\"\n"
         "namespace rtc {\n"
         "template <class...> using void_t = void;\n"
         "template <class S, class = void> struct tgt { static constexpr bool v = false; };\n"
         "template <class S> struct tgt<S, void_t<decltype(S::TGT)>> { static constexpr bool v = S::TGT; };\n"
         "template <class S, class = void> struct zw { static constexpr unsigned v = 0u; };\n"
         "template <class S> struct zw<S, void_t<decltype(S::ZW_PRESET)>> { static constexpr unsigned v = S::ZW_PRESET; };\n"
         "template <class S, class = void> struct su1 { static constexpr unsigned v = 0u; };\n"
         "template <class S> struct su1<S, void_t<decltype(S::SHARED_U1)>> { static constexpr unsigned v = S::SHARED_U1; };\n"
         "template <class S, class = void> struct jac { static constexpr bool v = false; };\n"
         "template <class S> struct jac<S, void_t<decltype(&S::template jac_T<float, true>)>> { static constexpr bool v = true; };\n"
         "template <class S, class = void> struct out { static constexpr bool v = false; };\n"
         "template <class S> struct out<S, void_t<decltype(&S::template out<float, true>)>> { static constexpr bool v = true; };\n"
         "template <class S, class = void> struct ojac { static constexpr bool v = false; };\n"
         "template <class S> struct ojac<S, void_t<decltype(&S::template out_jac_T<float, true>)>> { static constexpr bool v = true; };\n"
         "template <class S, class = void> struct dy { static constexpr int v = S::DS; };\n"
         "template <class S> struct dy<S, void_t<decltype(S::DY)>> { static constexpr int v = S::DY; };\n"
         "template <class S, class = void> struct crit { static constexpr bool v = false; };\n"
         "template <class S> struct crit<S, void_t<decltype(S::CRITIC)>> { static constexpr bool v = S::CRITIC; };\n"
         "template <bool TGT, bool JAC, int DY, bool OUT, bool OJAC, bool CRIT> __global__ void k_rtc_probe() {}\n"
         "}  // namespace rtc\n"
         "struct RcgRtcSys : " + N + " {\n"
         "  static constexpr bool TGT = rtc::tgt<" + N + ">::v;\n"
         "  static constexpr unsigned ZW_PRESET = rtc::zw<" + N + ">::v;\n"
         "  static constexpr unsigned SHARED_U1 = rtc::su1<" + N + ">::v;\n"
         "  static constexpr bool HAS_OUT = rtc::out<" + N + ">::v;\n"
         "  static constexpr int DY = rtc::dy<" + N + ">::v;\n"
         "};\n" +
         dims + "}  // namespace rcg\n";
}

int compile(const std::string& src, const std::string& file, const std::vector<std::string>& exprs, RtcProgram* out,
            std::string* log) {
  std::vector<const char*> names, texts;
  for (int i = 0; i < kRtcHeaderCount; ++i) {
    names.push_back(kRtcHeaderNames[i]);
    texts.push_back(kRtcHeaderTexts[i]);
  }
  for (const char* stub : {"hip/hip_runtime.h", "hip/hip_ext.h"}) {
    names.push_back(stub);
    texts.push_back("\n");
  }
  hiprtcProgram prog;
  if (hiprtcCreateProgram(&prog, src.c_str(), file.c_str(), (int)names.size(), texts.data(), names.data()) != HIPRTC_SUCCESS) {
    *log = "hiprtcCreateProgram failed";
    return RCG_ERR_HIP;
  }
  for (const auto& e : exprs) hiprtcAddNameExpression(prog, e.c_str());
  const hiprtcResult rc = hiprtcCompileProgram(prog, (int)(sizeof kOpts / sizeof kOpts[0]), kOpts);
  size_t n = 0;
  hiprtcGetProgramLogSize(prog, &n);
  std::string text(n, '\0');
  if (n) hiprtcGetProgramLog(prog, &text[0]);
  while (!text.empty() && text.back() == '\0') text.pop_back();
  if (rc != HIPRTC_SUCCESS) {
    *log = std::string(hiprtcGetErrorString(rc)) + ":\n" + text;
    hiprtcDestroyProgram(&prog);
    return RCG_ERR_BAD_ARG;
  }
  n = 0;
  hiprtcGetCodeSize(prog, &n);
  out->code.assign(n, '\0');
  if (n) hiprtcGetCode(prog, &out->code[0]);
  for (const auto& e : exprs) {
    const char* low = nullptr;
    if (hiprtcGetLoweredName(prog, e.c_str(), &low) != HIPRTC_SUCCESS || !low) {
      *log = "hiprtcGetLoweredName: no instance " + e;
      hiprtcDestroyProgram(&prog);
      return RCG_ERR_HIP;
    }
    out->lowered[e] = low;
  }
  hiprtcDestroyProgram(&prog);
  return n ? RCG_OK : RCG_ERR_HIP;
}

std::string tf(bool b) { return b ? "true" : "false"; }

template <typename real>
std::string expr_rhs() {
  return std::string("rcg::k_rhs<") + kSysExpr + ", " + real_name<real>() + ">";
}
template <typename real>
std::string expr_stage_obj() {
  return std::string("rcg::k_stage_obj<") + kSysExpr + ", " + real_name<real>() + ">";
}
template <typename real>
std::string expr_out() {
  return std::string("rcg::k_out<") + kSysExpr + ", " + real_name<real>() + ">";
}
template <typename real>
std::string expr_sim(bool tgt) {
  return std::string("rcg::k_sim<") + kSysExpr + ", " + real_name<real>() + ", " + tf(tgt) + ">";
}
template <typename real>
std::string expr_actor(bool gen, bool tgt, bool str, bool direct) {
  return std::string("rcg::k_actor<") + kSysExpr + ", " + real_name<real>() + ", " + tf(gen) + ", " + tf(tgt) + ", " + tf(str) +
         (direct ? ", false, true>" : ">");
}
template <typename real>
std::string expr_opt(bool tgt, bool gen, bool pairs) {
  return std::string("rcg::k_actor_opt<") + kSysExpr + ", " + real_name<real>() + ", " + tf(tgt) + ", " + tf(gen) + ", " + tf(pairs) +
         ">";
}
template <typename real>
std::string expr_dma(bool packed, int R, int variant, bool sys_tgt) {
  const bool tgt = (!packed && variant >= DMA_MPC_GEND) ? true : sys_tgt;
  return std::string(packed ? "rcg::k_actor_dma_packed<" : "rcg::k_actor_dma<") + kSysExpr + ", " + real_name<real>() + ", " +
         std::to_string(R) + ", " + tf(tgt) + ", " + std::to_string(variant) + ">";
}

template <typename real>
std::string expr_critic() {
  return std::string("rcg::k_critic<") + kSysExpr + ", " + real_name<real>() + ">";
}
template <typename real>
std::string expr_critic_cost() {
  return std::string("rcg::k_critic_cost<") + kSysExpr + ", " + real_name<real>() + ">";
}
template <typename real>
std::string expr_fit(int cs, int form) {
  const std::string head = std::string("<") + kSysExpr + ", " + real_name<real>() + ", " + std::to_string(cs);
  if (form == FIT_FORM_GEN) return "rcg::k_critic_fit_gen" + head + ">";
  if (form == FIT_FORM_3ML) return "rcg::k_critic_fit_ml" + head + ", 3>";
  return "rcg::k_critic_fit" + head + ", " + std::to_string(form == FIT_FORM_3 ? 3 : kFitMaxRows) + ">";
}

template <typename real>
std::vector<std::string> core_exprs(const RtcDims& d) {
  const bool has_jac = d.has_jac && (!d.has_out || d.has_out_jac);
  std::vector<std::string> e{expr_rhs<real>(), expr_stage_obj<real>(), expr_sim<real>(false), expr_sim<real>(true)};
  if (d.has_out) e.push_back(expr_out<real>());
  for (int g = 0; g < 2; ++g)
    for (int t = 0; t < 2; ++t) {
      for (int s = 0; s < 2; ++s) e.push_back(expr_actor<real>(g, t, s, false));
      if (g) e.push_back(expr_actor<real>(true, t, true, true));
    }
  if (has_jac)
    for (int sel = 0; sel < 8; ++sel) e.push_back(expr_opt<real>(sel & 2, sel & 4, sel & 1));
  return e;
}

int function(rcg_handle* h, RtcProgram& P, const std::string& expr, hipFunction_t* fn) {
  const int dev = h->cfg.device;
  auto it = P.fn.find({dev, expr});
  if (it != P.fn.end()) {
    *fn = it->second;
    return RCG_OK;
  }
  auto low = P.lowered.find(expr);
  if (low == P.lowered.end()) return rcg_fail(h, RCG_ERR_HIP, "runtime system: no compiled instance %s", expr.c_str());
  if (!P.module.count(dev)) {
    hipModule_t m = nullptr;
    HIPCHK(h, hipModuleLoadData(&m, P.code.data()));
    P.module[dev] = m;
  }
  hipFunction_t f = nullptr;
  HIPCHK(h, hipModuleGetFunction(&f, P.module[dev], low->second.c_str()));
  P.fn[{dev, expr}] = f;
  *fn = f;
  return RCG_OK;
}

template <typename real>
int core_function(rcg_handle* h, const std::string& expr, hipFunction_t* fn) {
  auto hit = h->rtc_fn.find(expr);
  if (hit != h->rtc_fn.end()) {
    *fn = hit->second;
    return RCG_OK;
  }
  std::lock_guard<std::mutex> lock(g_mu);
  RtcSystem& S = *const_cast<RtcSystem*>(h->rtc);
  const int rc = function(h, S.core[sizeof(real) == 8 ? 1 : 0], expr, fn);
  if (rc == RCG_OK) h->rtc_fn[expr] = *fn;
  return rc;
}

template <typename real>
int dma_function(rcg_handle* h, bool packed, int R, int variant, hipFunction_t* fn) {
  RtcSystem& S = *const_cast<RtcSystem*>(h->rtc);
  const std::string expr = expr_dma<real>(packed, R, variant, S.tgt);
  auto hit = h->rtc_fn.find(expr);
  if (hit != h->rtc_fn.end()) {
    *fn = hit->second;
    return RCG_OK;
  }
  const auto key = std::make_tuple(sizeof(real) == 8 ? 1 : 0, packed ? 1 : 0, R, variant);
  bool have;
  {
    std::lock_guard<std::mutex> lock(g_mu);
    have = S.dma.count(key) != 0;
  }
  std::unique_ptr<RtcProgram> P;
  if (!have) {
    P.reset(new RtcProgram);
    std::string log;
    const int rc = compile(unit_source(S), S.name + "_dma.hip", {expr}, P.get(), &log);
    if (rc) {
      h->err = "runtime system " + S.name + ": compiling " + expr + ": " + log;
      return RCG_ERR_HIP;
    }
  }
  std::lock_guard<std::mutex> lock(g_mu);
  auto it = S.dma.find(key);
  if (it == S.dma.end()) {
    it = S.dma.emplace(key, std::move(P)).first;
    S.compiled.push_back(S.name + "_dma.hip\t" + expr);
  }
  const int rc = function(h, *it->second, expr, fn);
  if (rc == RCG_OK) h->rtc_fn[expr] = *fn;
  return rc;
}

template <typename real>
int critic_functions(rcg_handle* h, int form, hipFunction_t* f_critic, hipFunction_t* f_cost, hipFunction_t* f_fit) {
  RtcSystem& S = *const_cast<RtcSystem*>(h->rtc);
  if (!S.dims.has_critic) return RCG_ERR_UNSUPPORTED;
  const int cs = h->cfg.critic_struct;
  const std::string e[3] = {expr_critic<real>(), expr_critic_cost<real>(), expr_fit<real>(cs, form)};
  hipFunction_t* const out[3] = {f_critic, f_cost, f_fit};
  bool all = true;
  for (int i = 0; i < 3; ++i) {
    if (!out[i]) continue;
    auto hit = h->rtc_fn.find(e[i]);
    if (hit != h->rtc_fn.end())
      *out[i] = hit->second;
    else
      all = false;
  }
  if (all) return RCG_OK;
  const auto key = std::make_tuple(sizeof(real) == 8 ? 1 : 0, cs, form);
  bool have;
  {
    std::lock_guard<std::mutex> lock(g_mu);
    have = S.critic.count(key) != 0;
  }
  const std::string file = S.name + "_critic.hip";
  std::unique_ptr<RtcProgram> P;
  if (!have) {
    P.reset(new RtcProgram);
    std::string log;
    const int rc = compile(unit_source(S, true), file, {e[0], e[1], e[2]}, P.get(), &log);
    if (rc) {
      h->err = "runtime system " + S.name + ": compiling the critic program (" + e[2] + "): " + log;
      return RCG_ERR_HIP;
    }
  }
  std::lock_guard<std::mutex> lock(g_mu);
  auto it = S.critic.find(key);
  if (it == S.critic.end()) {
    it = S.critic.emplace(key, std::move(P)).first;
    for (const auto& x : e) S.compiled.push_back(file + "\t" + x);
  }
  for (int i = 0; i < 3; ++i) {
    if (!out[i]) continue;
    const int rc = function(h, *it->second, e[i], out[i]);
    if (rc) return rc;
    h->rtc_fn[e[i]] = *out[i];
  }
  return RCG_OK;
}

int refuse_critic(rcg_handle* h, const char* who) {
  return rcg_fail(h, RCG_ERR_UNSUPPORTED,
                  "%s: not available for a system registered at run time whose policy does not opt in with CRITIC (%s)", who,
                  h->rtc ? h->rtc->name.c_str() : "?");
}

int launch(rcg_handle* h, hipFunction_t f, dim3 grid, dim3 block, size_t lds, void** args) {
  const ProfPair pp = prof_take(h);
  hipError_t e;
  if (pp.a)
    e = hipExtModuleLaunchKernel(f, grid.x * block.x, grid.y * block.y, grid.z * block.z, block.x, block.y, block.z, lds,
                                 h->stream, args, nullptr, pp.a, pp.b, 0);
  else
    e = hipModuleLaunchKernel(f, grid.x, grid.y, grid.z, block.x, block.y, block.z, (unsigned)lds, h->stream, args, nullptr);
  if (e != hipSuccess) return rcg_fail(h, RCG_ERR_HIP, "runtime system: kernel launch failed: %s", hipGetErrorString(e));
  return RCG_OK;
}

int refuse(rcg_handle* h, const char* who) {
  return rcg_fail(h, RCG_ERR_UNSUPPORTED, "%s: not available for a system registered at run time (%s)", who,
                  h->rtc ? h->rtc->name.c_str() : "?");
}

int rtc_rhs(rcg_handle* h, const void* state, const void* action, void* dstate, void* clipped, int32_t n, int32_t clip) {
  return by_dtype(h, [&](auto r) {
    using real = decltype(r);
    hipFunction_t f;
    int rc = core_function<real>(h, expr_rhs<real>(), &f);
    if (rc) return rc;
    const real* st = (const real*)state;
    const real* ac = (const real*)action;
    real* ds = (real*)dstate;
    real* cl = (real*)clipped;
    const real* pe = (h->f[RCG_FIELD_PARS] && n == h->cfg.batch) ? (const real*)h->f[RCG_FIELD_PARS] : nullptr;
    long nn = n;
    int ci = clip;
    KParams<real> P = params<real>(h);
    void* args[] = {&st, &ac, &ds, &cl, &pe, &nn, &ci, &P};
    return launch(h, f, dim3(blocks_for(n)), dim3(256), 0, args);
  });
}

int rtc_stage_obj(rcg_handle* h, const void* obs, const void* act, void* out, int32_t n) {
  return by_dtype(h, [&](auto r) {
    using real = decltype(r);
    hipFunction_t f;
    int rc = core_function<real>(h, expr_stage_obj<real>(), &f);
    if (rc) return rc;
    const real* o = (const real*)obs;
    const real* a = (const real*)act;
    real* y = (real*)out;
    long nn = n;
    KParams<real> P = params<real>(h);
    void* args[] = {&o, &a, &y, &nn, &P};
    return launch(h, f, dim3(blocks_for(n)), dim3(256), 0, args);
  });
}

template <typename real>
int sim_step(rcg_handle* h, int32_t n_substeps) {
  hipFunction_t f;
  int rc = core_function<real>(h, expr_sim<real>((h->cfg.flags & RCG_FLAG_HAS_TARGET) != 0), &f);
  if (rc) return rc;
  SimArgs<real> A = sim_args<real>(h, n_substeps);
  KParams<real> P = params<real>(h);
  void* args[] = {&A, &P};
  ProfScope prof_scope(h, RCG_KERNEL_SIM);
  note_launch(h, RCG_KERNEL_SIM, RCG_KID_SIM, 0, 64);
  return launch(h, f, dim3(blocks_for(h->cfg.batch)), dim3(256), 0, args);
}

int rtc_sim_step(rcg_handle* h, int32_t n_substeps) {
  return by_dtype(h, [&](auto r) { return sim_step<decltype(r)>(h, n_substeps); });
}

struct ActorPick {
  bool packed, dma;
  hipFunction_t f;
};
template <typename real>
int resolve_actor_instance(rcg_handle* h, const ActorPlan& L, bool streamed, ActorPick* p) {
  p->packed = L.pack_ok && !(L.variant >= DMA_RQL_0 && !packed_critic_ok(h->dc, (int)sizeof(real)));
  p->dma = !p->packed && L.dma_ok;
  if (p->packed || p->dma) return dma_function<real>(h, p->packed, L.R, L.variant, &p->f);
  return core_function<real>(h, expr_actor<real>(L.long_row || L.generic, L.tgt, streamed, L.long_row), &p->f);
}

template <typename real>
int actor(rcg_handle* h, const char* who, const void* cand, int K, const void* obs, const void* state_sys, const void* w, void* J,
          void* action, void* best_J, int32_t* best_idx, bool tick, bool sim_first) {
  const RtcSystem& S = *h->rtc;
  ActorArgs<real> A;
  ActorPlan L;
  int rc = actor_plan<real>(h, who, S.dims.ds, S.dims.du, S.tgt, cand, K, obs, state_sys, w, J, action, best_J, best_idx, tick,
                            sim_first, A, L);
  if (rc) return rc;
  if (h->probe == 1) {
    h->probe = (L.dma_ok && !L.pack_ok) ? 3 : 2;
    return RCG_OK;
  }
  if (h->sub_hi > 0 && !(L.dma_ok && !L.pack_ok))
    return rcg_fail(h, RCG_ERR_UNSUPPORTED, "%s: a split tick needs the k_actor_dma shape", who);
  ActorPick pick;
  rc = resolve_actor_instance<real>(h, L, cand != nullptr, &pick);
  if (rc) return rc;
  const bool packed = pick.packed, dma = pick.dma;
  hipFunction_t const f = pick.f;
  const bool fuse_sim = packed && L.fuse_sim;
  if (sim_first && !fuse_sim) {
    rc = sim_step<real>(h, h->cfg.substeps_per_tick);
    if (rc) return rc;
  }
  KParams<real> P = params<real>(h);
  ProfScope prof_scope(h, RCG_KERNEL_ACTOR);
  if (packed) {
    ActorArgs<real> Ap = packed_args(h, A, L);
    void* args[] = {&Ap, &P};
    rc = launch(h, f, L.pack_grid, dim3(256), L.pack_lds, args);
    if (rc == RCG_OK) note_launch(h, RCG_KERNEL_ACTOR, RCG_KID_ACTOR_DMA_PACKED, L.variant | (fuse_sim ? 16 : 0), (int)L.pack_gpw);
    return rc;
  }
  if (dma) {
    ActorArgs<real> Ad = dma_args(h, A, L);
    void* args[] = {&Ad, &P};
    rc = launch(h, f, L.dma_grid, dim3(256), L.dma_lds, args);
    if (rc == RCG_OK) note_launch(h, RCG_KERNEL_ACTOR, RCG_KID_ACTOR_DMA, L.variant, (int)L.dma_gpw);
    return rc;
  }
  void* args[] = {&A, &P};
  rc = launch(h, f, dim3(L.blocks), dim3(64 * L.wpb), L.long_row ? 0 : L.lds, args);
  if (rc == RCG_OK)
    note_launch(h, RCG_KERNEL_ACTOR, RCG_KID_ACTOR,
                L.long_row ? (1 | (L.tgt ? 2 : 0) | 4 | 16) : ((L.generic ? 1 : 0) | (L.tgt ? 2 : 0) | (cand ? 4 : 0)), A.G);
  return rc;
}

int rtc_actor(rcg_handle* h, const char* who, const void* cand, int K, const void* obs, const void* state_sys, const void* w,
              void* J, void* action, void* best_J, int32_t* best_idx, bool tick, bool sim_first) {
  return by_dtype(h, [&](auto r) {
    return actor<decltype(r)>(h, who, cand, K, obs, state_sys, w, J, action, best_J, best_idx, tick, sim_first);
  });
}

int rtc_optimize(rcg_handle* h, int32_t iters, const void* obs, const void* state_sys, const void* u_init, int shift, void* u_opt,
                 void* action, void* best_J, int32_t* n_iter, bool tick, bool sim_first) {
  if (!h->rtc->dims.has_jac)
    return rcg_fail(h, RCG_ERR_UNSUPPORTED, "rcg_actor_optimize: the policy %s defines no jac_T (the optimiser's adjoint sweep)",
                    h->rtc->name.c_str());
  if (h->rtc->dims.has_out && !h->rtc->dims.has_out_jac)
    return rcg_fail(h, RCG_ERR_UNSUPPORTED,
                    "rcg_actor_optimize: the policy %s defines out but no out_jac_T (the adjoint of its output map)",
                    h->rtc->name.c_str());
  if (h->loop_io.on) return refuse(h, "rcg_loop_step");
  return by_dtype(h, [&](auto r) {
    using real = decltype(r);
    const rcg_cfg& c = h->cfg;
    OptArgs<real> A;
    int wpb;
    size_t lds;
    int rc = opt_plan<real>(h, h->du, iters, obs, state_sys, u_init, shift, u_opt, action, best_J, n_iter, tick, A, wpb, lds);
    if (rc) return rc;
    KParams<real> P = params<real>(h);
    const bool generic = !(c.mode == RCG_MODE_MPC && P.stage_kind == 0);
    const bool tgt = c.flags & RCG_FLAG_HAS_TARGET;
    const bool pairs = A.memory > 0;
    hipFunction_t f;
    rc = core_function<real>(h, expr_opt<real>(tgt, generic, pairs), &f);
    if (rc) return rc;
    if (tick && sim_first) {
      rc = sim_step<real>(h, c.substeps_per_tick);
      if (rc) return rc;
    }
    ProfScope prof_scope(h, RCG_KERNEL_ACTOR);
    void* args[] = {&A, &P};
    rc = launch(h, f, dim3(blocks_for(c.batch, wpb * OPT_G)), dim3(64 * wpb), lds, args);
    if (rc == RCG_OK)
      note_launch(h, RCG_KERNEL_ACTOR, RCG_KID_ACTOR_OPT, (generic ? 1 : 0) | (tgt ? 2 : 0) | (pairs ? 4 : 0), OPT_G);
    return rc;
  });
}

int rtc_critic(rcg_handle* h, const void* obs, const void* act, const void* w, void* out, int32_t n) {
  if (!h->rtc->dims.has_critic) return refuse(h, "rcg_critic");
  return by_dtype(h, [&](auto r) {
    using real = decltype(r);
    hipFunction_t f;
    int rc = critic_functions<real>(h, fit_form_of(h->cfg.n_critic - 1, h->dc, false), &f, nullptr, nullptr);
    if (rc) return rc;
    const real* o = (const real*)obs;
    const real* a = (const real*)act;
    const real* ww = (const real*)w;
    real* y = (real*)out;
    long nn = n;
    KParams<real> P = params<real>(h);
    void* args[] = {&o, &a, &ww, &y, &nn, &P};
    return launch(h, f, dim3(blocks_for(n)), dim3(256), 0, args);
  });
}

int rtc_critic_cost(rcg_handle* h, const void* w, void* Jc) {
  if (!h->rtc->dims.has_critic) return refuse(h, "rcg_critic_cost");
  return by_dtype(h, [&](auto r) {
    using real = decltype(r);
    hipFunction_t f;
    int rc = critic_functions<real>(h, fit_form_of(h->cfg.n_critic - 1, h->dc, false), nullptr, &f, nullptr);
    if (rc) return rc;
    const real* ww = w ? (const real*)w : (const real*)h->f[RCG_FIELD_W_CRITIC];
    const real* wp = (const real*)h->f[RCG_FIELD_W_PREV];
    const real* ob = (const real*)h->f[RCG_FIELD_OBS_BUF];
    const real* ab = (const real*)h->f[RCG_FIELD_ACT_BUF];
    real* jc = (real*)Jc;
    KParams<real> P = params<real>(h);
    void* args[] = {&ww, &wp, &ob, &ab, &jc, &P};
    return launch(h, f, dim3(blocks_for(h->cfg.batch)), dim3(256), 0, args);
  });
}

int rtc_critic_update(rcg_handle* h, int32_t n_substeps, int32_t do_push, int32_t do_fit) {
  if (!h->rtc->dims.has_critic) return refuse(h, "the critic update");
  return by_dtype(h, [&](auto r) {
    using real = decltype(r);
    hipFunction_t f;
    int rc = critic_functions<real>(h, fit_form_of(h->cfg.n_critic - 1, h->dc, false), nullptr, nullptr, &f);
    if (rc) return rc;
    ProfScope prof_scope(h, RCG_KERNEL_CRITIC);
    FitArgs<real> F;
    FitPlan L;
    rc = fit_plan<real>(h, n_substeps, do_push, do_fit, false, F, L);
    if (rc) return rc;
    KParams<double> P64 = h->p64;
    KParams<real> P = params<real>(h);
    double* scratch = (double*)h->fit_scratch;
    void* args[] = {&F, &P64, &P, &scratch};
    rc = launch(h, f, L.grid, L.block, 0, args);
    if (rc == RCG_OK) note_launch(h, RCG_KERNEL_CRITIC, RCG_KID_CRITIC_FIT, L.variant, L.epw);
    return rc;
  });
}
int rtc_nominal(rcg_handle* h, const void*, void*, void*, void*, int32_t, double, const double*, int32_t, bool) {
  return refuse(h, "the nominal controller");
}
int rtc_ticks(rcg_handle* h, int32_t, int32_t, const void*) { return refuse(h, "rcg_control_ticks"); }
int rtc_rhs_full(rcg_handle* h, const void*, const void*, const void*, const void*, void*, void*, void*, int32_t, int32_t) {
  return refuse(h, "rcg_rhs_full");
}
int rtc_search(rcg_handle* h, int32_t, int32_t, int32_t, const void*, const void*, const void*, int, void*, void*, void*, int32_t*,
               bool, bool) {
  return refuse(h, "rcg_actor_search");
}
int rtc_loop(rcg_handle* h, const double*, int32_t, int32_t, int32_t, int32_t, int32_t, double*, double*, double) {
  return refuse(h, "rcg_loop_step");
}

int probe(RtcSystem& S, std::string* log) {
  const std::string pol = "rcg::" + S.name;
  const std::string e = std::string("rcg::rtc::k_rtc_probe<") + kSysExpr + "::TGT, rcg::rtc::jac<" + pol + ">::v, " + kSysExpr +
                        "::DY, " + kSysExpr + "::HAS_OUT, rcg::rtc::ojac<" + pol + ">::v, rcg::rtc::crit<" + pol + ">::v>";
  RtcProgram P;
  const int rc = compile(unit_source(S), S.name + "_probe.hip", {e}, &P, log);
  if (rc) return rc;
  const std::string& low = P.lowered[e];
  long v[6];
  size_t p = low.find("IL");
  int n = 0;
  for (p = p == std::string::npos ? p : p + 1; p != std::string::npos && n < 6 && p + 2 < low.size() && low[p] == 'L'; ++n) {
    const char t = low[p + 1];
    size_t q = p + 2;
    const bool neg = t == 'i' && low[q] == 'n';
    if (neg) ++q;
    long x = 0;
    while (q < low.size() && isdigit((unsigned char)low[q])) x = 10 * x + (low[q++] - '0');
    if ((t != 'b' && t != 'i') || q >= low.size() || low[q] != 'E') break;
    v[n] = neg ? -x : x;
    p = q + 1;
  }
  if (n != 6) {
    *log = "cannot read the probe instance " + low;
    return RCG_ERR_HIP;
  }
  S.tgt = v[0] != 0;
  S.dims.has_jac = v[1] != 0;
  S.dims.dy = (int)v[2];
  S.dims.has_out = v[3] != 0;
  S.dims.has_out_jac = S.dims.has_out && v[4] != 0;
  S.dims.has_critic = v[5] != 0;
  return RCG_OK;
}

}

#if !defined(__HIP_DEVICE_COMPILE__)
const SysVTable kVtRtc = {&rtc_rhs,     &rtc_stage_obj, &rtc_critic,   &rtc_critic_cost, &rtc_actor,
                          &rtc_sim_step, &rtc_critic_update, &rtc_optimize, &rtc_nominal, &rtc_ticks,
                          &rtc_rhs_full, &rtc_search,    &rtc_ticks,    &rtc_loop};
#endif

int rtc_out(rcg_handle* h, const void* state, void* obs, int32_t n) {
  return by_dtype(h, [&](auto r) {
    using real = decltype(r);
    hipFunction_t f;
    int rc = core_function<real>(h, expr_out<real>(), &f);
    if (rc) return rc;
    const real* st = (const real*)state;
    real* y = (real*)obs;
    const real* pe = (h->f[RCG_FIELD_PARS] && n == h->cfg.batch) ? (const real*)h->f[RCG_FIELD_PARS] : nullptr;
    long nn = n;
    KParams<real> P = params<real>(h);
    void* args[] = {&st, &y, &pe, &nn, &P};
    return launch(h, f, dim3(blocks_for(n)), dim3(256), 0, args);
  });
}

int rtc_prepare_tick(rcg_handle* h, const void* cand, int32_t K) {
  if (!h->rtc->dims.has_critic) return refuse_critic(h, "rcg_control_tick");
  int rc = by_dtype(h, [&](auto r) {
    hipFunction_t f;
    return critic_functions<decltype(r)>(h, fit_form_of(h->cfg.n_critic - 1, h->dc, false), nullptr, nullptr, &f);
  });
  if (rc) return rc;
  return by_dtype(h, [&](auto r) {
    using real = decltype(r);
    const RtcSystem& S = *h->rtc;
    ActorArgs<real> A;
    ActorPlan L;
    int rc2 = actor_plan<real>(h, "rcg_control_tick", S.dims.ds, S.dims.du, S.tgt, cand, K, nullptr, nullptr, nullptr, nullptr,
                               h->f[RCG_FIELD_ACTION], h->f[RCG_FIELD_BEST_J], (int32_t*)h->f[RCG_FIELD_BEST_IDX], true, false, A, L);
    if (rc2) return rc2;
    ActorPick pick;
    return resolve_actor_instance<real>(h, L, cand != nullptr, &pick);
  });
}

int rtc_prepare_tick_opt(rcg_handle* h) {
  const RtcDims& d = h->rtc->dims;
  if (!d.has_critic) return refuse_critic(h, "rcg_control_tick_opt");
  if (!d.has_jac || (d.has_out && !d.has_out_jac))
    return rcg_fail(h, RCG_ERR_UNSUPPORTED, "rcg_control_tick_opt: the policy %s defines no jac_T%s (the optimiser's adjoint sweep)",
                    h->rtc->name.c_str(), d.has_out ? " / out_jac_T" : "");
  return by_dtype(h, [&](auto r) {
    hipFunction_t f;
    return critic_functions<decltype(r)>(h, fit_form_of(h->cfg.n_critic - 1, h->dc, false), nullptr, nullptr, &f);
  });
}

const RtcSystem* rtc_lookup(int sys_id, RtcDims* dims) {
  std::lock_guard<std::mutex> lock(g_mu);
  const int i = sys_id - RCG_SYS_USER_BASE;
  if (i < 0 || i >= (int)g_sys.size()) return nullptr;
  if (dims) *dims = g_sys[i]->dims;
  return g_sys[i].get();
}

extern "C" {

int rcg_register_system(const char* name, const char* policy_src, int32_t ds, int32_t du, int32_t np, int32_t* sys_id) {
  if (!name || !policy_src || !sys_id) return rcg_fail(nullptr, RCG_ERR_BAD_ARG, "rcg_register_system: null argument");
  if (!is_identifier(name))
    return rcg_fail(nullptr, RCG_ERR_BAD_ARG, "rcg_register_system: the name must be the policy struct's C++ identifier");
  if (ds < 1 || du < 1 || np < 0) return rcg_fail(nullptr, RCG_ERR_BAD_ARG, "rcg_register_system: need ds >= 1, du >= 1, np >= 0");
  if (ds > RCG_MAX_DS || du > RCG_MAX_DU || np > RCG_MAX_PARS)
    return rcg_fail(nullptr, RCG_ERR_UNSUPPORTED, "rcg_register_system: ds %d, du %d, np %d beyond the limits %d, %d, %d", ds, du, np,
                    RCG_MAX_DS, RCG_MAX_DU, RCG_MAX_PARS);
  auto known = [&](int* rc) -> bool {
    for (const auto& s : g_sys) {
      if (s->name != name) continue;
      if (s->src != policy_src || s->dims.ds != ds || s->dims.du != du || s->dims.np != np) {
        *rc = rcg_fail(nullptr, RCG_ERR_BAD_ARG, "rcg_register_system: %s is registered already, with another source or dimensions",
                       name);
      } else {
        *sys_id = s->id;
        *rc = RCG_OK;
      }
      return true;
    }
    return false;
  };
  int rc = RCG_OK;
  {
    std::lock_guard<std::mutex> lock(g_mu);
    if (known(&rc)) return rc;
  }
  std::unique_ptr<RtcSystem> S(new RtcSystem);
  S->name = name;
  S->src = policy_src;
  S->dims = RtcDims{ds, du, np, false, ds, false, false, false};
  S->tgt = false;
  std::string log;
  rc = probe(*S, &log);
  if (rc == RCG_OK && (S->dims.dy < 1 || S->dims.dy > RCG_MAX_DS))
    return rcg_fail(nullptr, RCG_ERR_UNSUPPORTED, "rcg_register_system: %s::DY = %d beyond 1 .. %d", name, S->dims.dy, RCG_MAX_DS);
  if (rc == RCG_OK) rc = compile(unit_source(*S), S->name + "_f32.hip", core_exprs<float>(S->dims), &S->core[0], &log);
  if (rc == RCG_OK) rc = compile(unit_source(*S), S->name + "_f64.hip", core_exprs<double>(S->dims), &S->core[1], &log);
  if (rc) {
    rcg_set_thread_error(std::string("rcg_register_system: ") + name + ": " + log);
    return rc;
  }
  for (const auto& e : core_exprs<float>(S->dims)) S->compiled.push_back(S->name + "_f32.hip\t" + e);
  for (const auto& e : core_exprs<double>(S->dims)) S->compiled.push_back(S->name + "_f64.hip\t" + e);
  std::lock_guard<std::mutex> lock(g_mu);
  if (known(&rc)) return rc;
  S->id = RCG_SYS_USER_BASE + (int)g_sys.size();
  *sys_id = S->id;
  g_sys.push_back(std::move(S));
  return RCG_OK;
}

int rcg_system_has_critic(int32_t sys_id, int32_t* has_critic) {
  RtcDims d{0, 0, 0, false, 0, false, false, true};
  if (!(sys_id >= 0 && sys_id <= 2) && !(sys_id >= RCG_SYS_USER_BASE && rtc_lookup(sys_id, &d)))
    return rcg_fail(nullptr, RCG_ERR_BAD_ARG, "rcg_system_has_critic: bad sys_id %d", sys_id);
  if (has_critic) *has_critic = d.has_critic ? 1 : 0;
  return RCG_OK;
}

int rcg_system_programs(int32_t sys_id, char* buf, int64_t cap, int64_t* need) {
  std::lock_guard<std::mutex> lock(g_mu);
  const int i = sys_id - RCG_SYS_USER_BASE;
  if (i < 0 || i >= (int)g_sys.size()) return rcg_fail(nullptr, RCG_ERR_BAD_ARG, "rcg_system_programs: bad sys_id %d", sys_id);
  std::string text;
  for (const auto& line : g_sys[i]->compiled) text += line + "\n";
  if (need) *need = (int64_t)text.size() + 1;
  if (buf && cap > 0) {
    const size_t n = text.size() < (size_t)cap - 1 ? text.size() : (size_t)cap - 1;
    memcpy(buf, text.data(), n);
    buf[n] = '\0';
  }
  return RCG_OK;
}

int rcg_rtc_version(int32_t* major, int32_t* minor) {
  int a = 0, b = 0;
  if (hiprtcVersion(&a, &b) != HIPRTC_SUCCESS) return rcg_fail(nullptr, RCG_ERR_HIP, "rcg_rtc_version: hiprtcVersion failed");
  if (major) *major = a;
  if (minor) *minor = b;
  return RCG_OK;
}

}
```

### rcognita_amd/csrc/rcg_sysops.hpp

```cpp
#pragma once
#include <cmath>
#include <cstdlib>
#include <cstring>
#include <type_traits>

#include "rcg_actor_dma.hpp"
#include "rcg_actor_dma_packed.hpp"
#include "rcg_critic_fit_ml.hpp"
#include "rcg_actor_opt.hpp"
#include "rcg_critic_fit.hpp"
#include "rcg_critic_fit_gen.hpp"
#include "rcg_disturb.hpp"
#include "rcg_handle.hpp"
#include "rcg_loop.hpp"
#include "rcg_nominal.hpp"
#include "rcg_search.hpp"
#include "rcg_ticks.hpp"

namespace rcg {

template <typename F>
static int by_dtype(rcg_handle* h, F&& f) {
  return h->cfg.dtype == RCG_F64 ? f(double{}) : f(float{});
}
// ... 299 lines not shown
  bool no_pack = false;
  int fit_lanes = 0;
  int dma_min_k = 33;
  bool no_tick_fuse = false;
  bool no_pk = false;
};
static inline const DevKnobs& dev_knobs() {
  static const DevKnobs k = [] {
    DevKnobs v;
#ifdef RCG_DEV
    if (const char* e = getenv("RCG_DBG")) v.dbg = atoi(e);
    if (const char* e = getenv("RCG_ACTOR_KERNEL")) v.force_plain = !strcmp(e, "plain");
    if (const char* e = getenv("RCG_GPW")) v.gpw = atol(e);
    if (const char* e = getenv("RCG_LDS_PAD")) v.lds_pad = atol(e);
    if (const char* e = getenv("RCG_PER_CU")) v.per_cu = atoi(e);
    if (const char* e = getenv("RCG_PLAIN_LDS")) v.plain_lds = atol(e);
    v.mpc_only = getenv("RCG_DMA_MPC_ONLY") != nullptr;
    v.no_gen_multi = getenv("RCG_NO_GEN_MULTI") != nullptr;
    v.no_g1 = getenv("RCG_NO_G1") != nullptr;
    v.no_pack = getenv("RCG_NO_PACK") != nullptr;
    v.no_pk = getenv("RCG_NO_PK") != nullptr;
    v.no_tick_fuse = getenv("RCG_NO_TICK_FUSE") != nullptr;
    if (const char* e = getenv("RCG_DMA_MINK")) v.dma_min_k = atoi(e);
    if (const char* e = getenv("RCG_FIT_LANES")) v.fit_lanes = atoi(e);
#endif
    return v;
  }();
  return k;
}
#ifdef RCG_DEV
static int fit_lanes_knob() { return dev_knobs().fit_lanes; }
#endif

template <typename Sys>
int op_ticks(rcg_handle* h, int32_t T, int32_t K, const void* cand);

struct ActorPlan {
  int R;
  size_t row_bytes;
  bool long_row;
  bool generic, tgt;
  int wpb;
  size_t lds;
  unsigned blocks;
  int variant;
  bool dma_ok, pack_ok;
  bool fuse_sim;
  long pack_gpw;
  dim3 pack_grid;
  size_t pack_lds;
  long dma_gpw;
  dim3 dma_grid;
  size_t dma_lds;
  int dma_jwave;
};

template <typename real>
static int actor_plan(rcg_handle* h, const char* who, int DS, int DU, bool sys_tgt, const void* cand, int K, const void* obs,
                      const void* state_sys, const void* w, void* J, void* action, void* best_J, int32_t* best_idx, bool tick,
                      bool sim_first, ActorArgs<real>& A, ActorPlan& L) {
  const rcg_cfg& c = h->cfg;
  if (K < 1) return rcg_fail(h, RCG_ERR_BAD_ARG, "%s: K must be >= 1", who);
  memset(&A, 0, sizeof A);
  A.cand = (const real*)cand;
  A.obs = obs ? (const real*)obs : (const real*)h->f[RCG_FIELD_STATE];
  if (state_sys)
    A.state_sys = (const real*)state_sys;
  else if (obs)
    A.state_sys = (const real*)obs;
  else
    A.state_sys = (const real*)h->f[(tick && (c.flags & RCG_FLAG_REF_LAG)) ? RCG_FIELD_STATE_PREV : RCG_FIELD_STATE];
  A.obs_x = obs ? 0 : 1;
  if (obs && !state_sys && h->dy != h->ds)
    return rcg_fail(h, RCG_ERR_BAD_ARG, "%s: an observation of dim_output %d != dim_state %d needs state_sys", who, h->dy, h->ds);
  A.pars_env = (const real*)h->f[RCG_FIELD_PARS];
  A.w = w ? (const real*)w : (const real*)h->f[RCG_FIELD_W_CRITIC];
  if (c.mode != RCG_MODE_MPC && !A.w)
    return rcg_fail(h, RCG_ERR_BAD_ARG, "%s: RQL/SQL need critic weights (buffer_size > 0 or an explicit w)", who);
  A.J = (real*)J;
  A.action_out = (real*)action;
  A.best_J = (real*)best_J;
  A.best_idx = best_idx;
  A.accum = (tick && !(c.flags & RCG_FLAG_ACCUM_EVERY_SUBSTEP)) ? (real*)h->f[RCG_FIELD_ACCUM] : nullptr;
  A.step_idx = tick ? (int32_t*)h->f[RCG_FIELD_STEP_IDX] : nullptr;
  A.K = K;
  if (K >= 64) {
    A.Kp = 64;
    A.G = 1;
    A.n_tiles = (K + 63) / 64;
  } else {
    int kp = 1;
    while (kp < K) kp <<= 1;
    A.Kp = kp;
    A.G = 64 / kp;
    A.n_tiles = 1;
  }
  A.grid_g = 0;
  A.no_multi = dev_knobs().no_gen_multi ? 1 : 0;
  if (!cand) {
    if (DU == 1) {
      A.grid_g = K;
    } else {
      int g = (int)std::floor(std::sqrt((double)K) + 1e-9);
      if (g * g != K)
        return rcg_fail(h, RCG_ERR_BAD_ARG, "%s: generated grid for du = 2 needs a square K (got %d)", who, K);
      A.grid_g = g;
    }
  }
  const int R = c.n_actor * DU;
  const size_t row_bytes = (size_t)R * sizeof(real);
  L.R = R;
  L.row_bytes = row_bytes;
  A.vec_ok = (cand && row_bytes % 16 == 0 && ((uintptr_t)cand % 16) == 0) ? 1 : 0;
  const long B = c.batch;
  const long n_waves = (B + A.G - 1) / A.G;
  int wpb = 4;
  const bool long_row = cand && R > RCG_MAX_ROW;
  size_t lds_per_wave = (cand && !long_row) ? 64 * row_bytes : 0;
  while (wpb > 1 && lds_per_wave * wpb > 64 * 1024) wpb >>= 1;
  size_t lds = lds_per_wave * wpb;
  if (cand && (size_t)dev_knobs().plain_lds > lds) lds = (size_t)dev_knobs().plain_lds;
  L.long_row = long_row;
  L.wpb = wpb;
  L.lds = lds;
  L.blocks = (unsigned)((n_waves + wpb - 1) / wpb);
  const KParams<real>& P = params<real>(h);
  const bool generic = !(c.mode == RCG_MODE_MPC && P.stage_kind == 0);
  const bool tgt = (c.flags & RCG_FLAG_HAS_TARGET) != 0;
  L.generic = generic;
  L.tgt = tgt;

  const DevKnobs& knobs = dev_knobs();
  A.dbg = knobs.dbg;
  constexpr size_t esz = sizeof(real);
  const size_t tile = (size_t)64 * dma_rpl(R, (int)esz) * R * esz;
  const bool mode_ok = c.mode == RCG_MODE_MPC || !knobs.mpc_only;
  const bool std_cost = P.stage_kind == 0 && (tgt == sys_tgt || !tgt);
  const bool gen_cost = c.mode == RCG_MODE_MPC && P.stage_kind != 0 && !knobs.force_plain;
  const bool gen_rql = c.mode == RCG_MODE_RQL && !std_cost && !knobs.force_plain;
  const bool sql_any = c.mode == RCG_MODE_SQL && (tgt == sys_tgt || !tgt);
  int variant;
  if (gen_cost)
    variant = (P.stage_kind & STAGE_FULL) ? DMA_MPC_GENF : DMA_MPC_GEND;
  else if (c.mode == RCG_MODE_MPC)
    variant = (c.gamma == 1.0 && !knobs.no_g1) ? DMA_MPC_G1 : DMA_MPC;
  else if (c.mode == RCG_MODE_RQL)
    variant = (gen_rql ? DMA_RQL_GEN_0 : DMA_RQL_0) + c.critic_struct;
  else
    variant = DMA_SQL_0 + c.critic_struct;
  L.variant = variant;
  const size_t wslot = (size_t)4 * dma_wslot((int)esz, variant, h->dy, DU);
  const bool slab16 = ((size_t)K * row_bytes) % 16 == 0;
  const int dma_min_k = (c.mode != RCG_MODE_MPC && knobs.dma_min_k > 20) ? 20 : knobs.dma_min_k;
  L.dma_ok = cand && ((uintptr_t)cand % 16) == 0 && K >= dma_min_k && slab16 && R <= dma_max_row<real>() &&
             (std_cost || gen_cost || gen_rql || sql_any) && mode_ok && !knobs.force_plain &&
             !(A.J && 4 * tile + wslot + 4 * esz * K > (size_t)160 * 1024);
  const int pack_g = (K >= 4 && K <= 32) ? 64 / K : 0;
  L.pack_ok = cand && ((uintptr_t)cand % 16) == 0 && pack_g >= 2 && slab16 && R <= dma_max_row<real>() && P.stage_kind == 0 &&
              mode_ok && (tgt == sys_tgt || !tgt) && !knobs.force_plain && !knobs.no_pack;
  L.fuse_sim = L.pack_ok && tick && sim_first && !obs && !state_sys && !A.J &&
               !(c.flags & (RCG_FLAG_DISTURB | RCG_FLAG_ACCUM_EVERY_SUBSTEP)) && !knobs.no_tick_fuse;
  {
    long gpw = pack_g;
    while (pack_g > 0 && gpw * 2 <= 64 && B / (gpw * 2) >= 4096) gpw *= 2;
    if (pack_g > 0 && knobs.gpw > 0 && knobs.gpw % pack_g == 0 && knobs.gpw <= 64) gpw = knobs.gpw;
    const long pw = gpw > 0 ? (B + gpw - 1) / gpw : 0;
    const size_t full_tile = (size_t)64 * R * esz;
    size_t lds_req = 4 * full_tile + (A.J ? 4 * esz * (size_t)gpw * K : 0) + (L.fuse_sim ? 4 * esz * 2 * DS * 64 : 0);
    const size_t cap = knobs.per_cu == 2 ? (size_t)56 * 1024 : (knobs.per_cu == 8 ? 0 : (size_t)36 * 1024);
    if (lds_req < cap) lds_req = cap;
    L.pack_gpw = gpw;
    L.pack_grid = dim3((unsigned)((pw + 3) / 4));
    L.pack_lds = lds_req;
  }
  {
    const long Bn = h->sub_hi > 0 ? h->sub_hi - h->sub_lo : B;
    long gpw = 1;
    while (gpw < 16 && Bn / (gpw * 2) >= 8192) gpw *= 2;
    if (knobs.gpw > 0) gpw = knobs.gpw;
    gpw = gpw < 1 ? 1 : (gpw > 64 ? 64 : gpw);
    const long pw = (Bn + gpw - 1) / gpw;
    const bool long_slab = (size_t)gpw * K * row_bytes >= (size_t)16 * 1024 * esz;
    const bool valu_heavy = variant == DMA_MPC_GENF ||
                            variant >= DMA_RQL_GEN_0 ||
                            ((dma_is_rql(variant) || dma_is_sql(variant)) && (size_t)dma_dc(dma_cs(variant), h->dy, DU) * esz >= 68);
    const int per_cu = knobs.per_cu > 0 ? knobs.per_cu : ((row_bytes >= 20 * esz && long_slab && !valu_heavy) ? 2 : 4);
    const int jwave = (A.J && 4 * tile + wslot + 4 * esz * gpw * K <= (size_t)64 * 1024) ? 1 : 0;
    size_t lds_req = 4 * tile + wslot + (A.J ? 4 * esz * K * (jwave ? gpw : 1) : 0);
    if (knobs.lds_pad > 0) {
      lds_req += (size_t)knobs.lds_pad;
    } else if (knobs.lds_pad == 0) {
      const size_t want = per_cu <= 2 ? (size_t)56 * 1024 : (per_cu <= 4 ? (size_t)36 * 1024 : 0);
      if (lds_req < want) lds_req = want;
    }
    L.dma_gpw = gpw;
    L.dma_grid = dim3((unsigned)((pw + 3) / 4));
    L.dma_lds = lds_req;
    L.dma_jwave = jwave;
  }
  return RCG_OK;
}

template <typename real>
static ActorArgs<real> packed_args(const rcg_handle* h, const ActorArgs<real>& A, const ActorPlan& L) {
  ActorArgs<real> Ap = A;
  Ap.G = 64 / A.K;
  Ap.gpw = (int)L.pack_gpw;
  Ap.jwave = 1;
  if (L.fuse_sim) {
    Ap.sim_state = (real*)h->f[RCG_FIELD_STATE];
    Ap.sim_state_prev = (real*)h->f[RCG_FIELD_STATE_PREV];
    Ap.sim_action = (const real*)h->f[RCG_FIELD_ACTION];
    Ap.sim_status = (uint32_t*)h->f[RCG_FIELD_STATUS];
    Ap.sim_n_sub = h->cfg.substeps_per_tick;
  }
  return Ap;
}
template <typename real>
static ActorArgs<real> dma_args(const rcg_handle* h, const ActorArgs<real>& A, const ActorPlan& L) {
  ActorArgs<real> Ad = A;
  Ad.gpw = (int)L.dma_gpw;
  Ad.env_lo = h->sub_lo;
  Ad.env_hi = h->sub_hi;
  Ad.jwave = L.dma_jwave;
  return Ad;
}

template <typename Sys, typename real>
static int launch_actor(rcg_handle* h, const char* who, const void* cand, int K, const void* obs,
                        const void* state_sys, const void* w, void* J, void* action, void* best_J, int32_t* best_idx,
                        bool tick, bool sim_first) {
  const rcg_cfg& c = h->cfg;
  ActorArgs<real> A;
  ActorPlan L;
  {
    const int rc = actor_plan<real>(h, who, Sys::DS, Sys::DU, Sys::TGT, cand, K, obs, state_sys, w, J, action, best_J, best_idx,
                                    tick, sim_first, A, L);
    if (rc) return rc;
  }
  const KParams<real>& P = params<real>(h);
  const DevKnobs& knobs = dev_knobs();
  const int R = L.R, wpb = L.wpb, variant = L.variant;
  const size_t lds = L.lds;
  const unsigned blocks = L.blocks;
  const bool generic = L.generic, tgt = L.tgt, dma_ok = L.dma_ok, pack_ok = L.pack_ok, fuse_sim = L.fuse_sim;
  if (h->probe == 1) {
    h->probe = (dma_ok && !pack_ok) ? 3 : 2;
    return RCG_OK;
  }
  if (h->sub_hi > 0 && !(dma_ok && !pack_ok))
    return rcg_fail(h, RCG_ERR_UNSUPPORTED, "%s: a split tick needs the k_actor_dma shape", who);
  if constexpr (std::is_same<real, float>::value && GenPk<Sys>::supported && GenPk<Sys>::fuse_tick) {
    if (tick && sim_first && !cand && !generic && !tgt && c.gamma == 1.0 && Sys::ZW_PRESET != 0u &&
        (P.zero_w & Sys::ZW_PRESET) == Sys::ZW_PRESET && K >= 256 && A.n_tiles % 4 == 0 && A.grid_g > 0 &&
        (64 % A.grid_g) == 0 && !A.no_multi && !knobs.no_pk && !knobs.no_tick_fuse && !(c.flags & RCG_FLAG_DISTURB) && !obs &&
        !state_sys &&
        action == h->f[RCG_FIELD_ACTION] && best_J == h->f[RCG_FIELD_BEST_J] && (void*)best_idx == h->f[RCG_FIELD_BEST_IDX])
      return op_ticks<Sys>(h, 1, K, nullptr);
  }
  if (sim_first && !fuse_sim) {
    int rc = op_sim_step<Sys>(h, c.substeps_per_tick);
    if (rc) return rc;
  }
  ProfScope prof_scope(h, RCG_KERNEL_ACTOR);
  if (pack_ok) {
    const ProfPair pp = prof_take(h);
    const ActorArgs<real> Ap = packed_args(h, A, L);
    const dim3 grid = L.pack_grid, block(256);
    const size_t lds_req = L.pack_lds;
    const bool launched =
        variant < DMA_RQL_0    ? launch_dma_packed<Sys, real, 3>(R, variant, grid, block, lds_req, h->stream, Ap, P, pp.a, pp.b)
        : variant >= DMA_SQL_0 ? launch_dma_packed<Sys, real, 4>(R, variant, grid, block, lds_req, h->stream, Ap, P, pp.a, pp.b)
                               : launch_dma_packed<Sys, real, 5>(R, variant, grid, block, lds_req, h->stream, Ap, P, pp.a, pp.b);
    if (launched) {
      note_launch(h, RCG_KERNEL_ACTOR, RCG_KID_ACTOR_DMA_PACKED, variant | (fuse_sim ? 16 : 0), (int)L.pack_gpw);
      HIPCHK(h, hipGetLastError());
      return RCG_OK;
    }
    prof_give_back(h, pp);
    if (fuse_sim) {
      int rc = op_sim_step<Sys>(h, c.substeps_per_tick);
      if (rc) return rc;
    }
  }
  if (dma_ok) {
    const ActorArgs<real> Ad = dma_args(h, A, L);
    const dim3 grid = L.dma_grid, block(256);
    const size_t lds_req = L.dma_lds;
    bool ok = false;
    const ProfPair pp = prof_take(h);
    if (variant >= DMA_RQL_GEN_0)
      ok = launch_dma<Sys, real, 7>(R, variant, grid, block, lds_req, h->stream, Ad, P, pp.a, pp.b);
    else if (variant >= DMA_MPC_GEND)
      ok = launch_dma<Sys, real, 6>(R, variant, grid, block, lds_req, h->stream, Ad, P, pp.a, pp.b);
    else if (variant < DMA_RQL_0)
      ok = launch_dma<Sys, real, 0>(R, variant, grid, block, lds_req, h->stream, Ad, P, pp.a, pp.b);
    else if (variant >= DMA_SQL_0)
      ok = launch_dma<Sys, real, 1>(R, variant, grid, block, lds_req, h->stream, Ad, P, pp.a, pp.b);
    else
      ok = launch_dma<Sys, real, 2>(R, variant, grid, block, lds_req, h->stream, Ad, P, pp.a, pp.b);
    if (!ok) prof_give_back(h, pp);
    if (ok) {
      note_launch(h, RCG_KERNEL_ACTOR, RCG_KID_ACTOR_DMA, variant, (int)L.dma_gpw);
      HIPCHK(h, hipGetLastError());
      return RCG_OK;
    }
  }
  if constexpr (std::is_same<real, float>::value && GenPk<Sys>::supported) {
    const bool pk_ok = !cand && !generic && !tgt && c.gamma == 1.0 && Sys::ZW_PRESET != 0u &&
                       (P.zero_w & Sys::ZW_PRESET) == Sys::ZW_PRESET && K >= 256 && A.n_tiles % 4 == 0 && A.grid_g > 0 &&
                       (64 % A.grid_g) == 0 && !A.no_multi && !knobs.no_pk;
    if (pk_ok) {
      RCG_LAUNCH(h, (k_actor<Sys, real, false, false, false, true>), dim3(blocks), dim3(64 * wpb), lds, A, P);
      note_launch(h, RCG_KERNEL_ACTOR, RCG_KID_ACTOR, 8, A.G);
      HIPCHK(h, hipGetLastError());
      return RCG_OK;
    }
  }
  if (L.long_row) {
    if (tgt)
      RCG_LAUNCH(h, (k_actor<Sys, real, true, true, true, false, true>), dim3(blocks), dim3(64 * wpb), 0, A, P);
    else
      RCG_LAUNCH(h, (k_actor<Sys, real, true, false, true, false, true>), dim3(blocks), dim3(64 * wpb), 0, A, P);
    note_launch(h, RCG_KERNEL_ACTOR, RCG_KID_ACTOR, 1 | (tgt ? 2 : 0) | 4 | 16, A.G);
    HIPCHK(h, hipGetLastError());
    return RCG_OK;
  }
#define RCG_LAUNCH_ACTOR(GEN, TGT, STR) \
  RCG_LAUNCH(h, (k_actor<Sys, real, GEN, TGT, STR>), dim3(blocks), dim3(64 * wpb), lds, A, P)
#define RCG_LAUNCH_ACTOR2(GEN, TGT)      \
  do {                                   \
    if (cand)                            \
      RCG_LAUNCH_ACTOR(GEN, TGT, true);  \
    else                                 \
      RCG_LAUNCH_ACTOR(GEN, TGT, false); \
  } while (0)
  if (generic) {
    if (tgt)
      RCG_LAUNCH_ACTOR2(true, true);
    else
      RCG_LAUNCH_ACTOR2(true, false);
  } else {
    if (tgt)
      RCG_LAUNCH_ACTOR2(false, true);
    else
      RCG_LAUNCH_ACTOR2(false, false);
  }
#undef RCG_LAUNCH_ACTOR2
#undef RCG_LAUNCH_ACTOR
  note_launch(h, RCG_KERNEL_ACTOR, RCG_KID_ACTOR, (generic ? 1 : 0) | (tgt ? 2 : 0) | (cand ? 4 : 0), A.G);
  HIPCHK(h, hipGetLastError());
  return RCG_OK;
}

template <typename Sys>
int op_actor(rcg_handle* h, const char* who, const void* cand, int K, const void* obs, const void* state_sys,
                    const void* w, void* J, void* action, void* best_J, int32_t* best_idx, bool tick, bool sim_first) {
  return by_dtype(h, [&](auto r) {
    return launch_actor<Sys, decltype(r)>(h, who, cand, K, obs, state_sys, w, J, action, best_J, best_idx, tick,
                                          sim_first);
  });
}

template <typename real>
static int opt_plan(rcg_handle* h, int du, int32_t iters, const void* obs, const void* state_sys, const void* u_init, int shift,
                    void* u_opt, void* action, void* best_J, int32_t* n_iter, bool tick, OptArgs<real>& A, int& wpb, size_t& lds) {
  const rcg_cfg& c = h->cfg;
  memset(&A, 0, sizeof A);
  A.obs = obs ? (const real*)obs : (const real*)h->f[RCG_FIELD_STATE];
  if (state_sys)
    A.state_sys = (const real*)state_sys;
  else if (obs)
    A.state_sys = (const real*)obs;
  else
    A.state_sys = (const real*)h->f[(tick && (c.flags & RCG_FLAG_REF_LAG)) ? RCG_FIELD_STATE_PREV : RCG_FIELD_STATE];
  A.obs_x = obs ? 0 : 1;
  if (obs && !state_sys && h->dy != h->ds)
    return rcg_fail(h, RCG_ERR_BAD_ARG, "rcg_actor_optimize: an observation of dim_output %d != dim_state %d needs state_sys", h->dy,
                    h->ds);
  A.pars_env = (const real*)h->f[RCG_FIELD_PARS];
  A.w = (const real*)h->f[RCG_FIELD_W_CRITIC];
  if (c.mode != RCG_MODE_MPC && !A.w)
    return rcg_fail(h, RCG_ERR_BAD_ARG, "rcg_actor_optimize: RQL/SQL need critic weights (buffer_size > 0)");
  A.u_init = (const real*)u_init;
  A.u_opt = (real*)u_opt;
  A.action_out = (real*)action;
  A.best_J = (real*)best_J;
  A.n_iter = n_iter;
  A.accum = (tick && !(c.flags & RCG_FLAG_ACCUM_EVERY_SUBSTEP)) ? (real*)h->f[RCG_FIELD_ACCUM] : nullptr;
  A.step_idx = tick ? (int32_t*)h->f[RCG_FIELD_STEP_IDX] : nullptr;
  for (int i = 0; i < du; ++i) A.u0[i] = (real)c.action_init[i];
  A.iters = iters;
  A.shift = shift;
  A.memory = opt_memory_of(h);
  A.ftol = (real)h->opt_ftol;
  A.dcw = c.mode != RCG_MODE_MPC ? h->dc : 0;
  const size_t lds_wave = opt_wave_lds_bytes(h);
  wpb = 4;
  size_t on_cu = 0;
  for (int cand_wpb = 4; cand_wpb >= 1; cand_wpb >>= 1) {
    const size_t fit = lds_wave * cand_wpb ? ((size_t)160 * 1024 / (lds_wave * cand_wpb)) * cand_wpb : 0;
    if (fit * 4 > on_cu * 5) {
      on_cu = fit;
      wpb = cand_wpb;
    }
  }
  lds = lds_wave * wpb;
  if (lds > (size_t)160 * 1024)
    return rcg_fail(h, RCG_ERR_UNSUPPORTED,
                    "rcg_actor_optimize: horizon %d with %d curvature pairs needs %zu B of LDS per wave (rcg_set_optimizer)",
                    c.n_actor, opt_memory_of(h), lds_wave);
  return RCG_OK;
}

template <typename Sys>
int op_optimize(rcg_handle* h, int32_t iters, const void* obs, const void* state_sys, const void* u_init,
                       int shift, void* u_opt, void* action, void* best_J, int32_t* n_iter, bool tick, bool sim_first) {
  const rcg_cfg& c = h->cfg;
  return by_dtype(h, [&](auto r) {
    using real = decltype(r);
    const KParams<real>& P = params<real>(h);
    OptArgs<real> A;
    int wpb;
    size_t lds;
    {
      const int rc = opt_plan<real>(h, Sys::DU, iters, obs, state_sys, u_init, shift, u_opt, action, best_J, n_iter, tick, A, wpb, lds);
      if (rc) return rc;
    }
    const bool loop = h->loop_io.on;
    if (loop)
      fill_loop_args<real>(h, A.loop, h->loop_io.act_in, h->loop_io.n_substeps, 1, 1, 1, h->loop_io.dc, h->loop_io.out,
                           h->loop_io.flag, h->loop_io.seq);
    const bool generic = !(c.mode == RCG_MODE_MPC && P.stage_kind == 0);
    const dim3 grid(blocks_for(c.batch, wpb * OPT_G)), block(64 * wpb);
    const bool tgt = c.flags & RCG_FLAG_HAS_TARGET;
    if (tick && sim_first) {
      const int rc = op_sim_step<Sys>(h, c.substeps_per_tick);
      if (rc) return rc;
    }
    const bool pairs = A.memory > 0;
    ProfScope prof_scope(h, RCG_KERNEL_ACTOR);
#define RCG_OPT_LAUNCH(T, GEN, PR)                                                                                  \
  do {                                                                                                              \
    auto fn = k_actor_opt<Sys, real, T, GEN, PR>;                                                                   \
    if (lds > 64 * 1024)                              \
      HIPCHK(h, hipFuncSetAttribute(reinterpret_cast<const void*>(fn), hipFuncAttributeMaxDynamicSharedMemorySize, \
                                    (int)lds));                                                                     \
    RCG_LAUNCH(h, fn, grid, block, lds, A, P);                                                                      \
  } while (0)
    const int sel = (generic ? 4 : 0) | (tgt ? 2 : 0) | (pairs ? 1 : 0);
    if (loop) {
      if (generic || pairs || obs || state_sys != h->f[RCG_FIELD_STATE_PREV] || u_init || tick)
        return rcg_fail(h, RCG_ERR_UNSUPPORTED, "rcg_loop_step: the one-launch sample is the plain MPC instance on the handle's own fields");
      auto fn = tgt ? k_actor_opt<Sys, real, true, false, false, true> : k_actor_opt<Sys, real, false, false, false, true>;
      if (lds > 64 * 1024)
        HIPCHK(h, hipFuncSetAttribute(reinterpret_cast<const void*>(fn), hipFuncAttributeMaxDynamicSharedMemorySize, (int)lds));
      RCG_LAUNCH(h, fn, grid, block, lds, A, P);
    } else
    switch (sel) {
      case 0: RCG_OPT_LAUNCH(false, false, false); break;
      case 1: RCG_OPT_LAUNCH(false, false, true); break;
      case 2: RCG_OPT_LAUNCH(true, false, false); break;
      case 3: RCG_OPT_LAUNCH(true, false, true); break;
      case 4: RCG_OPT_LAUNCH(false, true, false); break;
      case 5: RCG_OPT_LAUNCH(false, true, true); break;
      case 6: RCG_OPT_LAUNCH(true, true, false); break;
      default: RCG_OPT_LAUNCH(true, true, true); break;
    }
#undef RCG_OPT_LAUNCH
    note_launch(h, RCG_KERNEL_ACTOR, RCG_KID_ACTOR_OPT, (generic ? 1 : 0) | (tgt ? 2 : 0) | (pairs ? 4 : 0) | (loop ? 8 : 0), OPT_G);
    HIPCHK(h, hipGetLastError());
    return (int)RCG_OK;
  });
}

template <typename Sys>
int op_search(rcg_handle* h, int32_t K, int32_t rounds, int32_t round0, const void* obs, const void* state_sys,
                     const void* centre, int shift, void* u_best, void* action, void* best_J, int32_t* best_idx, bool tick,
                     bool sim_first) {
  const rcg_cfg& c = h->cfg;
  return by_dtype(h, [&](auto r) {
    using real = decltype(r);
    const KParams<real>& P = params<real>(h);
    SearchArgs<real> A;
    memset(&A, 0, sizeof A);
    A.obs = obs ? (const real*)obs : (const real*)h->f[RCG_FIELD_STATE];
    if (state_sys)
      A.state_sys = (const real*)state_sys;
    else if (obs)
      A.state_sys = (const real*)obs;
    else
      A.state_sys = (const real*)h->f[(tick && (c.flags & RCG_FLAG_REF_LAG)) ? RCG_FIELD_STATE_PREV : RCG_FIELD_STATE];
    A.pars_env = (const real*)h->f[RCG_FIELD_PARS];
    A.w = (const real*)h->f[RCG_FIELD_W_CRITIC];
    A.centre_in = (const real*)centre;
    A.u_best = (real*)u_best;
    A.action_out = (real*)action;
    A.best_J = (real*)best_J;
    A.best_idx = best_idx;
    A.accum = (tick && !(c.flags & RCG_FLAG_ACCUM_EVERY_SUBSTEP)) ? (real*)h->f[RCG_FIELD_ACCUM] : nullptr;
    A.step_rw = tick ? (int32_t*)h->f[RCG_FIELD_STEP_IDX] : nullptr;
    A.episode_idx = (const int32_t*)h->f[RCG_FIELD_EPISODE_IDX];
    A.step_idx = (const int32_t*)h->f[RCG_FIELD_STEP_IDX];
    for (int i = 0; i < Sys::DU; ++i) A.u0[i] = (real)c.action_init[i];
    A.K = K;
    A.rounds = rounds;
    A.round0 = round0;
    A.shift = shift;
    A.seed = c.seed;
    A.env_id_base = c.env_id_base;
    const int R = c.n_actor * Sys::DU;
    const bool generic = !(c.mode == RCG_MODE_MPC && P.stage_kind == 0);
    const bool tgt = (c.flags & RCG_FLAG_HAS_TARGET) != 0;
#ifndef RCG_SEARCH_F64_REG_ROWS
#define RCG_SEARCH_F64_REG_ROWS 5
#endif
    int nc = (!generic && tgt == Sys::TGT && (c.n_actor == 3 || c.n_actor == 5 || c.n_actor == 10)) ? c.n_actor : 0;
    if (sizeof(real) == 8 && nc > RCG_SEARCH_F64_REG_ROWS) nc = 0;
    int wpb = 4;
    const size_t lds_wave = (size_t)search_lds_reals(R, nc > 0) * sizeof(real);
    while (wpb > 1 && lds_wave * wpb > (size_t)64 * 1024) wpb >>= 1;
    const size_t lds = lds_wave * wpb;
    if (lds > (size_t)64 * 1024)
      return rcg_fail(h, RCG_ERR_UNSUPPORTED, "rcg_actor_search: rows of %d reals need %zu B of LDS per wave (at most 65536)", R,
                      lds_wave);
    const dim3 grid(blocks_for(c.batch, wpb)), block(64 * wpb);
    if (tick && sim_first) {
      const int rc = op_sim_step<Sys>(h, c.substeps_per_tick);
      if (rc) return rc;
    }
    ProfScope prof_scope(h, RCG_KERNEL_ACTOR);
    if (nc == 3)
      RCG_LAUNCH(h, (k_actor_search<Sys, real, false, Sys::TGT, 3>), grid, block, lds, A, P);
    else if (nc == 5)
      RCG_LAUNCH(h, (k_actor_search<Sys, real, false, Sys::TGT, 5>), grid, block, lds, A, P);
    else if (nc == 10)
      RCG_LAUNCH(h, (k_actor_search<Sys, real, false, Sys::TGT, 10>), grid, block, lds, A, P);
    else if (generic && tgt)
      RCG_LAUNCH(h, (k_actor_search<Sys, real, true, true, 0>), grid, block, lds, A, P);
    else if (generic)
      RCG_LAUNCH(h, (k_actor_search<Sys, real, true, false, 0>), grid, block, lds, A, P);
    else if (tgt)
      RCG_LAUNCH(h, (k_actor_search<Sys, real, false, true, 0>), grid, block, lds, A, P);
    else
      RCG_LAUNCH(h, (k_actor_search<Sys, real, false, false, 0>), grid, block, lds, A, P);
    note_launch(h, RCG_KERNEL_ACTOR, RCG_KID_ACTOR_SEARCH, (generic ? 1 : 0) | (tgt ? 2 : 0) | (nc > 0 ? 4 : 0), 1);
    HIPCHK(h, hipGetLastError());
    return (int)RCG_OK;
  });
}

template <typename Sys>
int op_ticks(rcg_handle* h, int32_t T, int32_t K, const void* cand) {
  constexpr int DU = Sys::DU;
  const rcg_cfg& c = h->cfg;
  return by_dtype(h, [&](auto r) {
    using real = decltype(r);
    const KParams<real>& P = params<real>(h);
    TicksArgs<real> A;
    memset(&A, 0, sizeof A);
    A.state = (real*)h->f[RCG_FIELD_STATE];
    A.state_prev = (real*)h->f[RCG_FIELD_STATE_PREV];
    A.action = (real*)h->f[RCG_FIELD_ACTION];
    A.pars_env = (const real*)h->f[RCG_FIELD_PARS];
    A.accum = (real*)h->f[RCG_FIELD_ACCUM];
    A.step_idx = (int32_t*)h->f[RCG_FIELD_STEP_IDX];
    A.status = (uint32_t*)h->f[RCG_FIELD_STATUS];
    A.best_J = (real*)h->f[RCG_FIELD_BEST_J];
    A.best_idx = (int32_t*)h->f[RCG_FIELD_BEST_IDX];
    A.cand = (const real*)cand;
    A.dist = (c.flags & RCG_FLAG_DISTURB) ? 1 : 0;
    if (A.dist) {
      A.disturb = (real*)h->f[RCG_FIELD_DISTURB];
      A.substep_idx = (int32_t*)h->f[RCG_FIELD_SUBSTEP_IDX];
      A.episode_idx = (const int32_t*)h->f[RCG_FIELD_EPISODE_IDX];
      A.D = disturb_pars(h);
    }
    A.T = T;
    A.n_sub = c.substeps_per_tick;
    A.K = K;
    if (K >= 64) {
      A.Kp = 64;
      A.G = 1;
      A.n_tiles = (K + 63) / 64;
    } else {
      int kp = 1;
      while (kp < K) kp <<= 1;
      A.Kp = kp;
      A.G = 64 / kp;
      A.n_tiles = 1;
    }
    A.grid_g = cand ? 0 : (DU == 1 ? K : (int)std::floor(std::sqrt((double)K) + 1e-9));
    A.no_multi = dev_knobs().no_gen_multi ? 1 : 0;
    const long n_waves = (c.batch + A.G - 1) / A.G;
    const bool generic = P.stage_kind != 0;
    const bool tgt = (c.flags & RCG_FLAG_HAS_TARGET) != 0;
    const int R = c.n_actor * DU;
    const size_t row_bytes = (size_t)R * sizeof(real);
    size_t lds = 0;
    if (cand) {
      const size_t rows_wave = K >= 64 ? (size_t)K : (size_t)A.G * K;
      A.vec_ok = (row_bytes % 16 == 0 && ((uintptr_t)cand % 16) == 0) ? 1 : 0;
      A.stage_once = rows_wave * row_bytes <= (size_t)32 * 1024 ? 1 : 0;
      const size_t per_wave = (A.stage_once ? rows_wave : (size_t)64) * row_bytes;
      A.lds_reals = (int)((per_wave + 15) / 16 * 16 / sizeof(real));
      lds = (size_t)A.lds_reals * sizeof(real) * 4;
// ... 184 lines not shown
```

### rcognita_amd/engine.py

```python
from __future__ import annotations

import ctypes as C
from dataclasses import dataclass
from typing import Optional, Sequence

import numpy as np

from . import _native as N


@dataclass
class EngineConfig:

    sys_id: int
    batch: int = 1
    dtype: str = "f32"
    device: int = 0
    Nactor: int = 5
    mode: str = "MPC"
    stage_obj_struct: str = "quadratic"
    critic_struct: str = "quad-nomix"
    Ncritic: int = 4
    buffer_size: int = 0
    substeps_per_tick: int = 1
# ... 440 lines not shown
        n = state.shape[0]
        keep = []
        ps = self._in(state, keep, lambda a: a.T)
        y = self._tmp((self.dy, n))
        N.check(N.lib().rcg_out(self._h, ps, C.c_void_p(y.ptr), n), self._h)
        return y.to_host().T.copy()

    def stage_obj(self, obs, act):
        obs = np.asarray(obs, dtype=self.real).reshape(-1, self.dy)
        act = np.asarray(act, dtype=self.real).reshape(-1, self.du)
        n = obs.shape[0]
        keep = []
        po, pa = self._in_many([(obs, lambda a: a.T, None, "obs"), (act, lambda a: a.T, None, "act")], keep)
        (pout,), fetch = self._out_many([((n,), None)])
        N.check(N.lib().rcg_stage_obj(self._h, po, pa, pout, n), self._h)
        return fetch()[0]

    def critic(self, obs, act, w):
        obs = np.asarray(obs, dtype=self.real).reshape(-1, self.dy)
        act = np.asarray(act, dtype=self.real).reshape(-1, self.du)
        w = np.asarray(w, dtype=self.real).reshape(-1, self.dc)
        n = obs.shape[0]
        keep = []
        po, pa, pw = self._in_many([(obs, lambda a: a.T, None, "obs"), (act, lambda a: a.T, None, "act"),
                                    (w, lambda a: a.T, None, "w")], keep)
        (pout,), fetch = self._out_many([((n,), None)])
        N.check(N.lib().rcg_critic(self._h, po, pa, pw, pout, n), self._h)
        return fetch()[0]

    def _cand(self, cand, keep, K=None):
        if cand is None:
            return None, (None if K is None else int(K))
        if isinstance(cand, DeviceArray) or _is_torch(cand):
            shape = tuple(int(v) for v in cand.shape)
            if len(shape) != 4:
                raise ValueError(f"candidates on the device must be [B, K, N, du], got shape {shape}")
            Kc = shape[1]
            ptr = self._check_device_input(cand, (self.B, Kc, self.N, self.du), self.real, "candidates")
        else:
            a = np.asarray(cand, dtype=self.real)
            if a.ndim == 3:
                a = np.broadcast_to(a[None], (self.B,) + a.shape)
            a = a.reshape(self.B, -1, self.N, self.du)
            ptr, Kc = self._in(a, keep), a.shape[1]
        if K is not None and int(K) != Kc:
            raise ValueError(f"K = {K} given, but the candidate tensor holds {Kc} sequences per env")
        return ptr, Kc

    def actor_cost(self, cand, obs=None, state_sys=None, w=None):
        keep = []
        pc, K = self._cand(cand, keep)
        J = self._tmp((self.B, K))
        N.check(N.lib().rcg_actor_cost(self._h, pc, K, self._in_soa(obs, keep, self.dy, "obs"),
                                       self._in_soa(state_sys, keep, self.ds, "state_sys"),
                                       self._in_soa(w, keep, self.dc, "w"), C.c_void_p(J.ptr)), self._h)
        return J.to_host()

    def critic_cost(self, w=None):
        keep = []
        Jc = self._tmp((self.B,))
        N.check(N.lib().rcg_critic_cost(self._h, self._in_soa(w, keep, self.dc, "w"), C.c_void_p(Jc.ptr)), self._h)
        return Jc.to_host()

    def set_tick_parts(self, parts):
        N.check(N.lib().rcg_set_tick_parts(self._h, int(parts)), self._h)

    def join(self):
        N.check(N.lib().rcg_join(self._h), self._h)

    def sim_step(self, n_substeps=1, step=None):
        if step is None:
            N.check(N.lib().rcg_sim_step(self._h, int(n_substeps)), self._h)
        else:
            N.check(N.lib().rcg_sim_step_h(self._h, int(n_substeps), float(step)), self._h)

    def loop_step(self, action, step, n_substeps=1, decide=False, push=False, fit=False, iters=10):
        ds, du = self.ds, self.du
        row = ds + du + 2 + (self.dc if self.cfg.mode != "MPC" else 0)
        out = np.empty((self.B, row), dtype=np.float64)
        pa = None
        if action is not None:
            a = np.asarray(action, dtype=np.float64)
            if a.shape != (self.B, du) or not a.flags.c_contiguous:
                a = np.ascontiguousarray(np.broadcast_to(a, (self.B, du)))
            pa = a.ctypes.data
        flags = (N.LOOP_DECIDE if decide else 0) | (N.LOOP_PUSH if push else 0) | (N.LOOP_FIT if fit else 0)
        rc = self._loop_fn(self._h, pa, step, n_substeps, flags, iters, out.ctypes.data)
        if rc:
            N.check(rc, self._h)
        return (out[:, :ds], out[:, ds:ds + du], out[:, ds + du], out[:, ds + du + 1],
                out[:, ds + du + 2:] if row > ds + du + 2 else None)

    def loop_step_begin(self, action, step, n_substeps=1, decide=False, push=False, fit=False, iters=10):
        pa = None
        if action is not None:
            a = np.asarray(action, dtype=np.float64)
            if a.shape != (self.B, self.du) or not a.flags.c_contiguous:
                a = np.ascontiguousarray(np.broadcast_to(a, (self.B, self.du)))
            pa = a.ctypes.data
        flags = (N.LOOP_DECIDE if decide else 0) | (N.LOOP_PUSH if push else 0) | (N.LOOP_FIT if fit else 0)
        rc = self._loop_begin_fn(self._h, pa, step, n_substeps, flags, iters)
        if rc:
            N.check(rc, self._h)

    def loop_step_end(self, drop=False):
        if drop:
            rc = self._loop_end_fn(self._h, None)
            if rc:
                N.check(rc, self._h)
            return None
        ds, du = self.ds, self.du
        row = ds + du + 2 + (self.dc if self.cfg.mode != "MPC" else 0)
        out = np.empty((self.B, row), dtype=np.float64)
        rc = self._loop_end_fn(self._h, out.ctypes.data)
        if rc:
            N.check(rc, self._h)
        return (out[:, :ds], out[:, ds:ds + du], out[:, ds + du], out[:, ds + du + 1],
                out[:, ds + du + 2:] if row > ds + du + 2 else None)

    def actor_argmin(self, cand=None, K=None, obs=None, state_sys=None):
        keep = []
        pc, K = self._cand(cand, keep, K)
        if K is None:
            raise ValueError("actor_argmin: K is required with generated candidates (cand=None)")
        pobs, pxs = self._in_many([self._soa_item(obs, self.dy, "obs"), self._soa_item(state_sys, self.ds, "state_sys")], keep)
        (pact, pbj, pbi), fetch = self._out_many([((self.du, self.B), None), ((self.B,), None), ((self.B,), np.int32)])
        N.check(N.lib().rcg_actor_argmin(self._h, pc, K, pobs, pxs, pact, pbj, pbi), self._h)
        act, bj, bi = fetch()
        return act.T.copy(), bj, bi

    def control_tick(self, cand=None, K=None, T=1):
        keep = []
        pc, K = self._cand(cand, keep, K)
        if K is None:
            raise ValueError("control_tick: K is required with generated candidates (cand=None)")
        if int(T) == 1:
            N.check(N.lib().rcg_control_tick(self._h, pc, K), self._h)
        else:
            N.check(N.lib().rcg_control_tick_n(self._h, pc, K, int(T)), self._h)
        if keep:
            self.synchronize()

    def control_ticks(self, T, K):
        N.check(N.lib().rcg_control_ticks(self._h, int(T), int(K)), self._h)

    def actor_optimize(self, iters=10, obs=None, state_sys=None, u_init=None):
        keep = []
        u0 = None if u_init is None else np.broadcast_to(
            np.asarray(u_init, dtype=self.real).reshape(-1, self.N, self.du), (self.B, self.N, self.du))
        pobs, pxs, pu = self._in_many([self._soa_item(obs, self.dy, "obs"), self._soa_item(state_sys, self.ds, "state_sys"),
                                       (u0, None, None, "u_init")], keep)
        (puo, pact, pbj, pni), fetch = self._out_many([((self.B, self.N, self.du), None), ((self.du, self.B), None),
                                                       ((self.B,), None), ((self.B,), np.int32)])
        N.check(N.lib().rcg_actor_optimize(self._h, int(iters), pobs, pxs, pu, puo, pact, pbj, pni), self._h)
        uo, act, bj, ni = fetch()
        return act.T.copy(), uo, bj, ni

    def control_tick_opt(self, iters=10, warm_start=False):
        N.check(N.lib().rcg_control_tick_opt(self._h, int(iters), 1 if warm_start else 0), self._h)

    def actor_search(self, K=256, rounds=6, obs=None, state_sys=None, centre=None):
        keep = []
        c0 = None if centre is None else np.broadcast_to(
            np.asarray(centre, dtype=self.real).reshape(-1, self.N, self.du), (self.B, self.N, self.du))
        pobs, pxs, pc = self._in_many([self._soa_item(obs, self.dy, "obs"), self._soa_item(state_sys, self.ds, "state_sys"),
                                       (c0, None, None, "centre")], keep)
        (pub, pact, pbj, pbi), fetch = self._out_many([((self.B, self.N, self.du), None), ((self.du, self.B), None),
                                                       ((self.B,), None), ((self.B,), np.int32)])
        N.check(N.lib().rcg_actor_search(self._h, int(K), int(rounds), pobs, pxs, pc, pub, pact, pbj, pbi), self._h)
        ub, act, bj, bi = fetch()
        return act.T.copy(), ub, bj, bi

    def control_tick_search(self, K=256, rounds=6, warm_start=False):
        N.check(N.lib().rcg_control_tick_search(self._h, int(K), int(rounds), 1 if warm_start else 0), self._h)

    def candidates_sample(self, K, round=0, centre=None, out=None):
        keep = []
        c0 = None if centre is None else np.broadcast_to(
            np.asarray(centre, dtype=self.real).reshape(-1, self.N, self.du), (self.B, self.N, self.du))
        (pc,) = self._in_many([(c0, None, (self.B, self.N, self.du), "centre")], keep)
        shape = (self.B, int(K), self.N, self.du)
        if out is not None:
            po = self._check_device_input(out, shape, self.real, "out")
            N.check(N.lib().rcg_candidates_sample(self._h, po, int(K), int(round), pc), self._h)
            if keep:
                self.synchronize()
            return out
        d = self._tmp(shape)
        N.check(N.lib().rcg_candidates_sample(self._h, C.c_void_p(d.ptr), int(K), int(round), pc), self._h)
        return d.to_host()

    def set_optimizer(self, memory=-1, ftol=None):
        N.check(N.lib().rcg_set_optimizer(self._h, int(memory)), self._h)
        if ftol is not None:
            N.check(N.lib().rcg_set_optimizer_tol(self._h, float(ftol)), self._h)

    @staticmethod
    def _ctrl_pars(ctrl_pars):
        if ctrl_pars is None:
            return None
        m, I = (float(v) for v in ctrl_pars)
        return (C.c_double * 2)(m, I)

    def nominal_action(self, obs, ctrl_gain, ctrl_pars=None, clip=False, want_lyap=False):
        obs = np.asarray(obs, dtype=self.real).reshape(-1, self.dy)
        n = obs.shape[0]
        keep = []
        (pact, plyap), fetch = self._out_many([((self.du, n), None), ((n,), None) if want_lyap else None])
        N.check(N.lib().rcg_nominal_action(self._h, self._in(obs, keep, lambda a: a.T), pact, plyap, n, float(ctrl_gain),
                                           self._ctrl_pars(ctrl_pars), 1 if clip else 0), self._h)
        act, lyap = fetch()
        a = act.T.copy()
        return (a, lyap) if want_lyap else a

    def nominal_theta(self, obs):
        obs = np.asarray(obs, dtype=self.real).reshape(-1, self.dy)
        n = obs.shape[0]
        keep = []
        (pth,), fetch = self._out_many([((n,), None)])
        N.check(N.lib().rcg_nominal_theta(self._h, self._in(obs, keep, lambda a: a.T), pth, n), self._h)
        return fetch()[0]

    def control_tick_nominal(self, ctrl_gain, ctrl_pars=None):
        N.check(N.lib().rcg_control_tick_nominal(self._h, float(ctrl_gain), self._ctrl_pars(ctrl_pars)), self._h)

    def critic_update(self, do_fit=True):
        N.check(N.lib().rcg_critic_update(self._h, 1 if do_fit else 0), self._h)

    def critic_fit(self):
        N.check(N.lib().rcg_critic_fit(self._h), self._h)

    def episode_reset(self):
        N.check(N.lib().rcg_episode_reset(self._h), self._h)

    def episode_stats(self, from_accum=False, want_returns=False):
        s = N.RcgSummary()
        out = np.empty((self.B,), dtype=self.real) if want_returns else None
        N.check(N.lib().rcg_episode_stats(self._h, 1 if from_accum else 0, out.ctypes.data if want_returns else None,
                                          C.byref(s)), self._h, allow=(N.ERR_NONFINITE,))
        return {k: getattr(s, k) for k in ("count", "sum", "sumsq", "min", "max", "n_failed")}, out

    def state_dict(self):
        out = {"tick_count": np.int64(N.lib().rcg_tick_count(self._h)), "batch": np.int64(self.B),
               "sys_id": np.int64(self.cfg.sys_id), "dtype": np.str_(self.cfg.dtype)}
        for f in range(N.FIELD_COUNT):
            if N.lib().rcg_field_bytes(self._h, f) > 0:
                out[f"field_{f}"] = self.get_field(f)
        return out

    def load_state_dict(self, sd):
        if int(sd["batch"]) != self.B or int(sd["sys_id"]) != int(self.cfg.sys_id) or str(sd["dtype"]) != self.cfg.dtype:
            raise ValueError("checkpoint was written by a handle with another batch / system / dtype")
        for f in range(N.FIELD_COUNT):
            have = N.lib().rcg_field_bytes(self._h, f) > 0
            if have != (f"field_{f}" in sd):
                raise ValueError(f"checkpoint and handle disagree on field {f} (different mode / flags)")
        order = [N.FIELD_STATE] + [f for f in range(N.FIELD_COUNT) if f != N.FIELD_STATE]
        for f in order:
            if f"field_{f}" in sd:
                self.set_field(f, sd[f"field_{f}"])
        N.check(N.lib().rcg_set_tick_count(self._h, int(sd["tick_count"])), self._h)

    def checkpoint(self, path):
        np.savez(path, **self.state_dict())

    def restore(self, path):
        with np.load(path, allow_pickle=False) as z:
            self.load_state_dict({k: z[k] for k in z.files})

    def profile(self, kernels=(N.KERNEL_ACTOR, N.KERNEL_SIM, N.KERNEL_CRITIC), stride=1, skip=0):
        mask = 0
        if kernels is True:
            mask = 7
        elif kernels:
            for k in kernels:
                mask |= 1 << int(k)
        if mask:
            stride = min(max(int(stride), 1), 0xfff)
            mask |= stride << 8
            mask |= (int(skip) % stride) << 20
        N.check(N.lib().rcg_profile(self._h, mask), self._h)

    def profile_pause(self):
        N.check(N.lib().rcg_profile(self._h, 0x80), self._h)

    def profile_read(self, kernel=N.KERNEL_ACTOR):
        ms, n = C.c_double(), C.c_int64()
        N.check(N.lib().rcg_profile_read(self._h, int(kernel), C.byref(ms), C.byref(n)), self._h)
        return ms.value, n.value

    def profile_samples(self, kernel=N.KERNEL_ACTOR) -> np.ndarray:
        n = C.c_int64()
        N.check(N.lib().rcg_profile_samples(self._h, int(kernel), None, 0, C.byref(n)), self._h)
        out = np.empty(max(n.value, 1), dtype=np.float64)
        N.check(N.lib().rcg_profile_samples(self._h, int(kernel), out.ctypes.data_as(C.POINTER(C.c_double)), n.value,
                                            C.byref(n)), self._h)
        return out[:n.value]

    def last_launch(self, kind=N.KERNEL_ACTOR):
        kid, var, epw = C.c_int32(), C.c_int32(), C.c_int32()
        N.check(N.lib().rcg_last_launch(self._h, int(kind), C.byref(kid), C.byref(var), C.byref(epw)), self._h)
        return {"kernel": N.lib().rcg_kernel_name(kid.value).decode(), "kernel_id": kid.value, "variant": var.value & ~4096,
                "envs_per_wave": epw.value, "split": bool(var.value & 4096)}
```

Baseline: 157.9 million.

## Add zero-weight specialized f64 DMA actor kernel with DPP wave argmin

Adds a templated zero-weight instance of the f64 DMA actor kernel for the MPC G1 variant. Channels whose weights are known to be zero in the policy preset skip the per-step running sums, and their cost comes from the terminal-state and initial terms instead. The instance also replaces the shuffle-based wave argmin with a DPP/readlane min reduction for doubles. This adds a dispatch path in the host launcher and in RTC, plus a query API for the mask used, at the cost of an extra kernel instantiation and more complex probe parsing.

```diff
diff --git a/include/rcg.h b/include/rcg.h
--- a/include/rcg.h
+++ b/include/rcg.h
@@ -7,7 +7,7 @@
 extern "C" {
 #endif
 
-#define RCG_VERSION 122
+#define RCG_VERSION 123
 
 #define RCG_MAX_DS 5
 #define RCG_MAX_DU 2
@@ -214,6 +214,7 @@
   RCG_KID_COUNT_ = 12
 } rcg_kernel_id;
 int rcg_last_launch(const rcg_handle* h, int32_t kind, int32_t* kernel_id, int32_t* variant, int32_t* envs_per_wave);
+int rcg_last_launch_zero_w(const rcg_handle* h, int32_t kind, uint32_t* mask);
 const char* rcg_kernel_name(int32_t kernel_id);
 
 #ifdef __cplusplus
diff --git a/rcognita_amd/_native.py b/rcognita_amd/_native.py
--- a/rcognita_amd/_native.py
+++ b/rcognita_amd/_native.py
@@ -7,7 +7,7 @@
 _HERE = os.path.dirname(os.path.abspath(__file__))
 LIB_PATH = os.path.join(_HERE, "lib", "librcg.so")
 
-RCG_VERSION = 122
+RCG_VERSION = 123
 OK, ERR_BAD_ARG, ERR_HIP, ERR_NO_DEVICE, ERR_UNSUPPORTED, ERR_NONFINITE = 0, -1, -2, -3, -4, -5
 SYS_3WROBOT, SYS_3WROBOT_NI, SYS_2TANK = 0, 1, 2
 MODE_MPC, MODE_RQL, MODE_SQL = 0, 1, 2
@@ -44,7 +44,7 @@
     "rcg_profile_samples", "rcg_last_launch", "rcg_kernel_name", "rcg_wait_stream", "rcg_nominal_theta", "rcg_set_optimizer", "rcg_set_optimizer_tol", "rcg_set_tick_parts", "rcg_join", "rcg_loop_step", "rcg_loop_step_begin", "rcg_loop_step_end",
     "rcg_actor_search", "rcg_control_tick_search", "rcg_candidates_sample", "rcg_release_stream",
     "rcg_register_system", "rcg_rtc_version", "rcg_system_info", "rcg_system_output_info", "rcg_out",
-    "rcg_system_has_critic", "rcg_system_programs", "rcg_critic_fit",
+    "rcg_system_has_critic", "rcg_system_programs", "rcg_critic_fit", "rcg_last_launch_zero_w",
 ]
 KERNEL_ACTOR, KERNEL_SIM, KERNEL_CRITIC = 0, 1, 2
 (KID_NONE, KID_ACTOR, KID_ACTOR_DMA, KID_TICKS, KID_ACTOR_OPT, KID_NOMINAL, KID_SIM, KID_SIM_V, KID_SIM_DIST,
@@ -160,6 +160,7 @@
         "rcg_profile_read": (C.c_int, [vp, i32, C.POINTER(C.c_double), C.POINTER(i64)]),
         "rcg_profile_samples": (C.c_int, [vp, i32, C.POINTER(C.c_double), i64, C.POINTER(i64)]),
         "rcg_last_launch": (C.c_int, [vp, i32, C.POINTER(i32), C.POINTER(i32), C.POINTER(i32)]),
+        "rcg_last_launch_zero_w": (C.c_int, [vp, i32, C.POINTER(C.c_uint32)]),
         "rcg_kernel_name": (C.c_char_p, [i32]),
         "rcg_wait_stream": (C.c_int, [vp, vp]),
         "rcg_release_stream": (C.c_int, [vp, vp]),
diff --git a/rcognita_amd/csrc/rcg_actor_dma.hpp b/rcognita_amd/csrc/rcg_actor_dma.hpp
--- a/rcognita_amd/csrc/rcg_actor_dma.hpp
+++ b/rcognita_amd/csrc/rcg_actor_dma.hpp
@@ -53,6 +53,24 @@
     }
   }
 }
+__device__ __forceinline__ void wave_argmin_reg(float& bestJ, int& bestI) { wave_argmin(bestJ, bestI); }
+__device__ __forceinline__ void wave_argmin_reg(double& bestJ, int& bestI) {
+#ifdef RCG_AB_SHFL_ARGMIN64
+  wave_argmin(bestJ, bestI);
+#else
+  const double Jmin = wave_min_f64(bestJ);
+  bestI = (int)wave_min_u32(bestJ == Jmin ? (unsigned)bestI : 0x7fffffffu);
+  bestJ = Jmin;
+#endif
+}
+
+template <typename Sys, typename real>
+__host__ __device__ constexpr unsigned dma_zw_preset() {
+  if constexpr (sizeof(real) == 8 && !HasOut<Sys>::value)
+    return Sys::ZW_PRESET;
+  else
+    return 0u;
+}
 
 template <typename S, typename = void>
 struct HasPrefix {
@@ -104,7 +122,7 @@
 
 __host__ __device__ constexpr int dma_rpl(int r, int esz) { return r * esz <= 24 ? 4 : (r * esz <= 32 ? 2 : 1); }
 
-template <typename Sys, typename real, int R, bool TGT, int V>
+template <typename Sys, typename real, int R, bool TGT, int V, unsigned ZW = 0u>
 __global__ __launch_bounds__(256) void k_actor_dma(const ActorArgs<real> A, const KParams<real> P) {
   constexpr int DS = Sys::DS, DY = sys_dy<Sys>(), DU = Sys::DU, NCHI = DY + DU, NP = Sys::NP;
   constexpr bool OUT = HasOut<Sys>::value;
@@ -112,6 +130,8 @@
   constexpr bool GEND = V == DMA_MPC_GEND, GENF = V == DMA_MPC_GENF, GEN = GEND || GENF;
   constexpr bool GENR = V >= DMA_RQL_GEN_0;
   static_assert(!(GEN || GENR) || TGT, "the generic-cost instances subtract a target (zeros for a handle without one)");
+  static_assert(ZW == 0u || (G1 && sizeof(real) == 8 && !OUT && ZW == Sys::ZW_PRESET),
+                "the zero-weight instance: DMA_MPC_G1, float64, no output map, the policy's preset mask");
   constexpr int CS = dma_cs(V);
   constexpr int DCMAX = CRIT ? dma_dc(CS, DY, DU) : 1;
   constexpr int ESZ = (int)sizeof(real);
@@ -274,6 +294,7 @@
   const bool env_pars = A.pars_env != nullptr;
   auto pre_env = Sys::template prepare<real>(pn);
   real x1s[DS], trig0[2] = {0, 0}, trig1[2] = {0, 0}, Sini[DY];
+  real zw0 = 0;
 #pragma unroll
   for (int c = 0; c < DS; ++c) x1s[c] = 0;
 #pragma unroll
@@ -340,6 +361,7 @@
       if constexpr (G1) {
 #pragma unroll
         for (int c = 0; c < DY; ++c) {
+          if ((ZW >> c) & 1u) continue;
           const real chi0 = TGT ? y0[c] - P.target[c] : y0[c];
           real a = fma_r(chi0, chi0, (real)0);
           if (N >= 2 && ((FREE >> c) & 1u)) {
@@ -349,6 +371,13 @@
           Sini[c] = uniform_r(a);
         }
       }
+    }
+    if constexpr (ZW != 0u) {
+      real z = 0;
+#pragma unroll
+      for (int i = 0; i < DY; ++i)
+        if ((ZW >> i) & 1u) z = fma_r(P.R1d[i], y0[i] * y0[i], z);
+      zw0 = uniform_r(z);
     }
     bestJ = inf_r<real>();
     bestI = 0x7fffffff;
@@ -449,6 +478,7 @@
 #pragma unroll
             for (int i = 0; i < NCHI; ++i) {
               if (PFX && i < DY && (kk == 0 || (kk == 1 && ((FREE >> i) & 1u)))) continue;
+              if ((ZW >> i) & 1u) continue;
               S[i] = fma_r(chi[i], chi[i], S[i]);
             }
           } else if (SQL) {
@@ -465,7 +495,17 @@
         }
         if (G1) {
 #pragma unroll
-          for (int i = 0; i < NCHI; ++i) J = fma_r(P.R1d[i], S[i], J);
+          for (int i = 0; i < NCHI; ++i)
+            if (!((ZW >> i) & 1u)) J = fma_r(P.R1d[i], S[i], J);
+          if constexpr (ZW != 0u) {
+#pragma unroll
+            for (int i = 0; i < DY; ++i)
+              if ((ZW >> i) & 1u) J = fma_r(P.R1d[i], y[i] * y[i], J);
+#pragma unroll
+            for (int c = 0; c < DU; ++c)
+              if ((ZW >> (DY + c)) & 1u) J = fma_r(P.R1d[DY + c], cur[(N - 1) * DU + c] * cur[(N - 1) * DU + c], J);
+            J += zw0;
+          }
         }
         if (SQL) {
 #pragma unroll
@@ -508,7 +548,10 @@
         ++b;
         continue;
       }
-      wave_argmin(bestJ, bestI);
+      if constexpr (ZW != 0u)
+        wave_argmin_reg(bestJ, bestI);
+      else
+        wave_argmin(bestJ, bestI);
       const int wl = __builtin_amdgcn_readfirstlane(bestI & 63);
 #pragma unroll
       for (int c = 0; c < DU; ++c) bu[c] = readlane_r(bu[c], wl);
@@ -546,6 +589,14 @@
 }
 
 #if !defined(__HIPCC_RTC__)
+template <typename real>
+static inline unsigned dma_zero_w(unsigned preset, int variant, const ActorArgs<real>& A, const KParams<real>& P) {
+#ifdef RCG_AB_NO_DMA_ZW
+  return 0u;
+#else
+  return (preset != 0u && variant == DMA_MPC_G1 && !A.J && (P.zero_w & preset) == preset) ? preset : 0u;
+#endif
+}
 template <typename Sys, typename real, int GROUP>
 bool launch_dma(int r, int variant, dim3 grid, dim3 block, size_t lds, hipStream_t s, const ActorArgs<real>& A,
                 const KParams<real>& P, hipEvent_t ev_a, hipEvent_t ev_b);
diff --git a/rcognita_amd/csrc/rcg_api.hip b/rcognita_amd/csrc/rcg_api.hip
--- a/rcognita_amd/csrc/rcg_api.hip
+++ b/rcognita_amd/csrc/rcg_api.hip
@@ -1263,6 +1263,12 @@
   return RCG_OK;
 }
 
+int rcg_last_launch_zero_w(const rcg_handle* h, int32_t kind, uint32_t* mask) {
+  if (!h || !mask || kind < 0 || kind >= RCG_KERNEL_COUNT_) return RCG_ERR_BAD_ARG;
+  *mask = h->last[kind].zero_w;
+  return RCG_OK;
+}
+
 const char* rcg_kernel_name(int32_t kernel_id) {
   static const char* const names[RCG_KID_COUNT_] = {"none",        "k_actor",   "k_actor_dma", "k_ticks",    "k_actor_opt",
                                                     "k_nominal",   "k_sim",     "k_sim_v",     "k_sim_dist", "k_critic_fit",
diff --git a/rcognita_amd/csrc/rcg_dma_launch.hpp b/rcognita_amd/csrc/rcg_dma_launch.hpp
--- a/rcognita_amd/csrc/rcg_dma_launch.hpp
+++ b/rcognita_amd/csrc/rcg_dma_launch.hpp
@@ -15,9 +15,9 @@
     if constexpr (R % Sys::DU != 0) {
       return false;
     } else {
-#define RCG_DMA_CASE(V)                                                                                              \
-  case V: {                                                                                                          \
-    auto fn = k_actor_dma<Sys, real, R, ((V) >= DMA_MPC_GEND ? true : Sys::TGT), V>;                                 \
+#define RCG_DMA_LAUNCH(FN)                                                                                           \
+  {                                                                                                                  \
+    auto fn = FN;                                                                                                    \
     if (lds > 64 * 1024)      \
       (void)hipFuncSetAttribute(reinterpret_cast<const void*>(fn), hipFuncAttributeMaxDynamicSharedMemorySize,       \
                                 (int)lds);                                                                           \
@@ -27,7 +27,14 @@
       hipLaunchKernelGGL(fn, grid, block, lds, s, A, P);                                                             \
     return true;                                                                                                     \
   }
+#define RCG_DMA_CASE(V) \
+  case V:               \
+    RCG_DMA_LAUNCH((k_actor_dma<Sys, real, R, ((V) >= DMA_MPC_GEND ? true : Sys::TGT), V>))
       if constexpr (GROUP == 0) {
+        constexpr unsigned ZWP = dma_zw_preset<Sys, real>();
+        if constexpr (ZWP != 0u) {
+          if (dma_zero_w<real>(ZWP, variant, A, P) != 0u) RCG_DMA_LAUNCH((k_actor_dma<Sys, real, R, Sys::TGT, DMA_MPC_G1, ZWP>))
+        }
         switch (variant) {
           RCG_DMA_CASE(DMA_MPC_G1)
           RCG_DMA_CASE(DMA_MPC)
@@ -60,6 +67,7 @@
         }
       }
 #undef RCG_DMA_CASE
+#undef RCG_DMA_LAUNCH
       return false;
     }
   }
diff --git a/rcognita_amd/csrc/rcg_handle.hpp b/rcognita_amd/csrc/rcg_handle.hpp
--- a/rcognita_amd/csrc/rcg_handle.hpp
+++ b/rcognita_amd/csrc/rcg_handle.hpp
@@ -72,6 +72,7 @@
   int probe;
   struct LastLaunch {
     int32_t kernel_id, variant, envs_per_wave;
+    uint32_t zero_w;
   } last[RCG_KERNEL_COUNT_];
 };
 static constexpr size_t kProfMaxSamples = 65536;
@@ -83,6 +84,7 @@
   h->last[kind].kernel_id = kernel_id;
   h->last[kind].variant = variant | (h->sub_hi > 0 ? kVariantSplitBit : 0);
   h->last[kind].envs_per_wave = envs_per_wave;
+  h->last[kind].zero_w = 0u;
 }
 
 static constexpr size_t kConstR64 = 512, kConstW = 1296, kConstBytes = 2256;
diff --git a/rcognita_amd/csrc/rcg_math.hpp b/rcognita_amd/csrc/rcg_math.hpp
--- a/rcognita_amd/csrc/rcg_math.hpp
+++ b/rcognita_amd/csrc/rcg_math.hpp
@@ -133,6 +133,49 @@
   return b < a ? b : a;
 }
 
+__device__ __forceinline__ double wave_min_f64(double v) {
+#define RCG_DPP_MIN(CTRL)                                                                                          \
+  {                                                                                                                \
+    const unsigned long long k = (unsigned long long)__double_as_longlong(v);                                      \
+    const unsigned lo = (unsigned)__builtin_amdgcn_update_dpp(0, (int)(unsigned)k, CTRL, 0xF, 0xF, false);         \
+    const unsigned hi = (unsigned)__builtin_amdgcn_update_dpp(0, (int)(unsigned)(k >> 32), CTRL, 0xF, 0xF, false); \
+    const double o = __longlong_as_double((long long)(((unsigned long long)hi << 32) | lo));                       \
+    v = o < v ? o : v;                                                                                             \
+  }
+  RCG_DPP_MIN(0xB1)
+  RCG_DPP_MIN(0x4E)
+  RCG_DPP_MIN(0x141)
+  RCG_DPP_MIN(0x140)
+#undef RCG_DPP_MIN
+  double r[4];
+#pragma unroll
+  for (int i = 0; i < 4; ++i) {
+    const unsigned long long k = (unsigned long long)__double_as_longlong(v);
+    const unsigned lo = (unsigned)__builtin_amdgcn_readlane((int)(unsigned)k, 16 * i);
+    const unsigned hi = (unsigned)__builtin_amdgcn_readlane((int)(unsigned)(k >> 32), 16 * i);
+    r[i] = __longlong_as_double((long long)(((unsigned long long)hi << 32) | lo));
+  }
+  const double a = r[1] < r[0] ? r[1] : r[0], b = r[3] < r[2] ? r[3] : r[2];
+  return b < a ? b : a;
+}
+__device__ __forceinline__ unsigned wave_min_u32(unsigned k) {
+#define RCG_DPP_MIN(CTRL)                                                                        \
+  {                                                                                              \
+    const unsigned o = (unsigned)__builtin_amdgcn_update_dpp(0, (int)k, CTRL, 0xF, 0xF, false); \
+    k = o < k ? o : k;                                                                           \
+  }
+  RCG_DPP_MIN(0xB1)
+  RCG_DPP_MIN(0x4E)
+  RCG_DPP_MIN(0x141)
+  RCG_DPP_MIN(0x140)
+#undef RCG_DPP_MIN
+  unsigned r[4];
+#pragma unroll
+  for (int i = 0; i < 4; ++i) r[i] = (unsigned)__builtin_amdgcn_readlane((int)k, 16 * i);
+  const unsigned a = r[1] < r[0] ? r[1] : r[0], b = r[3] < r[2] ? r[3] : r[2];
+  return b < a ? b : a;
+}
+
 __device__ __forceinline__ float readlane_r(float v, int l) {
   return __uint_as_float((unsigned)__builtin_amdgcn_readlane((int)__float_as_uint(v), l));
 }
diff --git a/rcognita_amd/csrc/rcg_rtc.hip b/rcognita_amd/csrc/rcg_rtc.hip
--- a/rcognita_amd/csrc/rcg_rtc.hip
+++ b/rcognita_amd/csrc/rcg_rtc.hip
@@ -27,6 +27,7 @@
   std::string name, src;
   RtcDims dims;
   bool tgt;
+  unsigned zw;
   RtcProgram core[2];
   std::map<std::tuple<int, int, int, int>, std::unique_ptr<RtcProgram>> dma;
   std::map<std::tuple<int, int, int>, std::unique_ptr<RtcProgram>> critic;
@@ -85,7 +86,7 @@
          "template <class S> struct dy<S, void_t<decltype(S::DY)>> { static constexpr int v = S::DY; };\n"
          "template <class S, class = void> struct crit { static constexpr bool v = false; };\n"
          "template <class S> struct crit<S, void_t<decltype(S::CRITIC)>> { static constexpr bool v = S::CRITIC; };\n"
-         "template <bool TGT, bool JAC, int DY, bool OUT, bool OJAC, bool CRIT> __global__ void k_rtc_probe() {}\n"
+         "template <bool TGT, bool JAC, int DY, bool OUT, bool OJAC, bool CRIT, unsigned ZW> __global__ void k_rtc_probe() {}\n"
          "}  // namespace rtc\n"
          "struct RcgRtcSys : " + N + " {\n"
          "  static constexpr bool TGT = rtc::tgt<" + N + ">::v;\n"
@@ -171,10 +172,10 @@
          ">";
 }
 template <typename real>
-std::string expr_dma(bool packed, int R, int variant, bool sys_tgt) {
+std::string expr_dma(bool packed, int R, int variant, bool sys_tgt, unsigned zw) {
   const bool tgt = (!packed && variant >= DMA_MPC_GEND) ? true : sys_tgt;
   return std::string(packed ? "rcg::k_actor_dma_packed<" : "rcg::k_actor_dma<") + kSysExpr + ", " + real_name<real>() + ", " +
-         std::to_string(R) + ", " + tf(tgt) + ", " + std::to_string(variant) + ">";
+         std::to_string(R) + ", " + tf(tgt) + ", " + std::to_string(variant) + (zw ? ", " + std::to_string(zw) + "u>" : ">");
 }
 
 template <typename real>
@@ -244,15 +245,15 @@
 }
 
 template <typename real>
-int dma_function(rcg_handle* h, bool packed, int R, int variant, hipFunction_t* fn) {
+int dma_function(rcg_handle* h, bool packed, int R, int variant, unsigned zw, hipFunction_t* fn) {
   RtcSystem& S = *const_cast<RtcSystem*>(h->rtc);
-  const std::string expr = expr_dma<real>(packed, R, variant, S.tgt);
+  const std::string expr = expr_dma<real>(packed, R, variant, S.tgt, zw);
   auto hit = h->rtc_fn.find(expr);
   if (hit != h->rtc_fn.end()) {
     *fn = hit->second;
     return RCG_OK;
   }
-  const auto key = std::make_tuple(sizeof(real) == 8 ? 1 : 0, packed ? 1 : 0, R, variant);
+  const auto key = std::make_tuple(sizeof(real) == 8 ? 1 : 0, packed ? 1 : 0, R, variant | (zw ? 256 : 0));
   bool have;
   {
     std::lock_guard<std::mutex> lock(g_mu);
@@ -405,13 +406,16 @@
 
 struct ActorPick {
   bool packed, dma;
+  unsigned zero_w;
   hipFunction_t f;
 };
 template <typename real>
-int resolve_actor_instance(rcg_handle* h, const ActorPlan& L, bool streamed, ActorPick* p) {
+int resolve_actor_instance(rcg_handle* h, const ActorArgs<real>& A, const ActorPlan& L, bool streamed, ActorPick* p) {
   p->packed = L.pack_ok && !(L.variant >= DMA_RQL_0 && !packed_critic_ok(h->dc, (int)sizeof(real)));
   p->dma = !p->packed && L.dma_ok;
-  if (p->packed || p->dma) return dma_function<real>(h, p->packed, L.R, L.variant, &p->f);
+  const RtcSystem& S = *h->rtc;
+  p->zero_w = (p->dma && sizeof(real) == 8 && !S.dims.has_out) ? dma_zero_w<real>(S.zw, L.variant, A, params<real>(h)) : 0u;
+  if (p->packed || p->dma) return dma_function<real>(h, p->packed, L.R, L.variant, p->zero_w, &p->f);
   return core_function<real>(h, expr_actor<real>(L.long_row || L.generic, L.tgt, streamed, L.long_row), &p->f);
 }
 
@@ -431,7 +435,7 @@
   if (h->sub_hi > 0 && !(L.dma_ok && !L.pack_ok))
     return rcg_fail(h, RCG_ERR_UNSUPPORTED, "%s: a split tick needs the k_actor_dma shape", who);
   ActorPick pick;
-  rc = resolve_actor_instance<real>(h, L, cand != nullptr, &pick);
+  rc = resolve_actor_instance<real>(h, A, L, cand != nullptr, &pick);
   if (rc) return rc;
   const bool packed = pick.packed, dma = pick.dma;
   hipFunction_t const f = pick.f;
@@ -453,7 +457,10 @@
     ActorArgs<real> Ad = dma_args(h, A, L);
     void* args[] = {&Ad, &P};
     rc = launch(h, f, L.dma_grid, dim3(256), L.dma_lds, args);
-    if (rc == RCG_OK) note_launch(h, RCG_KERNEL_ACTOR, RCG_KID_ACTOR_DMA, L.variant, (int)L.dma_gpw);
+    if (rc == RCG_OK) {
+      note_launch(h, RCG_KERNEL_ACTOR, RCG_KID_ACTOR_DMA, L.variant, (int)L.dma_gpw);
+      h->last[RCG_KERNEL_ACTOR].zero_w = pick.zero_w;
+    }
     return rc;
   }
   void* args[] = {&A, &P};
@@ -584,26 +591,26 @@
 int probe(RtcSystem& S, std::string* log) {
   const std::string pol = "rcg::" + S.name;
   const std::string e = std::string("rcg::rtc::k_rtc_probe<") + kSysExpr + "::TGT, rcg::rtc::jac<" + pol + ">::v, " + kSysExpr +
-                        "::DY, " + kSysExpr + "::HAS_OUT, rcg::rtc::ojac<" + pol + ">::v, rcg::rtc::crit<" + pol + ">::v>";
+                        "::DY, " + kSysExpr + "::HAS_OUT, rcg::rtc::ojac<" + pol + ">::v, rcg::rtc::crit<" + pol + ">::v, " + kSysExpr + "::ZW_PRESET>";
   RtcProgram P;
   const int rc = compile(unit_source(S), S.name + "_probe.hip", {e}, &P, log);
   if (rc) return rc;
   const std::string& low = P.lowered[e];
-  long v[6];
+  long v[7];
   size_t p = low.find("IL");
   int n = 0;
-  for (p = p == std::string::npos ? p : p + 1; p != std::string::npos && n < 6 && p + 2 < low.size() && low[p] == 'L'; ++n) {
+  for (p = p == std::string::npos ? p : p + 1; p != std::string::npos && n < 7 && p + 2 < low.size() && low[p] == 'L'; ++n) {
     const char t = low[p + 1];
     size_t q = p + 2;
     const bool neg = t == 'i' && low[q] == 'n';
     if (neg) ++q;
     long x = 0;
     while (q < low.size() && isdigit((unsigned char)low[q])) x = 10 * x + (low[q++] - '0');
-    if ((t != 'b' && t != 'i') || q >= low.size() || low[q] != 'E') break;
+    if ((t != 'b' && t != 'i' && t != 'j') || q >= low.size() || low[q] != 'E') break;
     v[n] = neg ? -x : x;
     p = q + 1;
   }
-  if (n != 6) {
+  if (n != 7) {
     *log = "cannot read the probe instance " + low;
     return RCG_ERR_HIP;
   }
@@ -613,6 +620,7 @@
   S.dims.has_out = v[3] != 0;
   S.dims.has_out_jac = S.dims.has_out && v[4] != 0;
   S.dims.has_critic = v[5] != 0;
+  S.zw = (unsigned)v[6];
   return RCG_OK;
 }
 
@@ -656,7 +664,7 @@
                                h->f[RCG_FIELD_ACTION], h->f[RCG_FIELD_BEST_J], (int32_t*)h->f[RCG_FIELD_BEST_IDX], true, false, A, L);
     if (rc2) return rc2;
     ActorPick pick;
-    return resolve_actor_instance<real>(h, L, cand != nullptr, &pick);
+    return resolve_actor_instance<real>(h, A, L, cand != nullptr, &pick);
   });
 }
 
diff --git a/rcognita_amd/csrc/rcg_sysops.hpp b/rcognita_amd/csrc/rcg_sysops.hpp
--- a/rcognita_amd/csrc/rcg_sysops.hpp
+++ b/rcognita_amd/csrc/rcg_sysops.hpp
@@ -625,6 +625,7 @@
     if (!ok) prof_give_back(h, pp);
     if (ok) {
       note_launch(h, RCG_KERNEL_ACTOR, RCG_KID_ACTOR_DMA, variant, (int)L.dma_gpw);
+      h->last[RCG_KERNEL_ACTOR].zero_w = dma_zero_w<real>(dma_zw_preset<Sys, real>(), variant, Ad, P);
       HIPCHK(h, hipGetLastError());
       return RCG_OK;
     }
diff --git a/rcognita_amd/engine.py b/rcognita_amd/engine.py
--- a/rcognita_amd/engine.py
+++ b/rcognita_amd/engine.py
@@ -766,3 +766,8 @@
         N.check(N.lib().rcg_last_launch(self._h, int(kind), C.byref(kid), C.byref(var), C.byref(epw)), self._h)
         return {"kernel": N.lib().rcg_kernel_name(kid.value).decode(), "kernel_id": kid.value, "variant": var.value & ~4096,
                 "envs_per_wave": epw.value, "split": bool(var.value & 4096)}
+
+    def last_launch_zero_w(self, kind=N.KERNEL_ACTOR):
+        m = C.c_uint32()
+        N.check(N.lib().rcg_last_launch_zero_w(self._h, int(kind), C.byref(m)), self._h)
+        return int(m.value)
```

Result: faster. 160.8 million, median of 6 (+1.8%).
